# rlog58/dags-vae-search

Hardware: AMD Instinct MI355X
Metric: DAGs/sec VAE+predictor train step, n=12 batch 4096 per GPU, at 1 MI355X (higher is better)
Workload: dtype f32 (fwd bf16x6, bwd bf16x3 split products, fp32 accumulate); 1 GPU; synthetic_v12 DAGs (n=12, card=12, N=15 tokens), PACE-VAE train step: pack + fwd + bwd + clip_grad_norm_(1.0) + Adam(1e-4), train mode dropout 0.15; per_gpu_batch=4096, global_batch=4096, waves_per_workgroup=8, parallelism=single

## Files before the change

### dags_vae_search_amd/csrc/dvs_api.hip

```cpp
#include <math.h>
#include <stdarg.h>
#include <stdio.h>
#include <stdlib.h>
#include <string.h>

#include "dvs_kernels.h"
#include "dvs_backward.h"
#include "dvs_wide.h"
#include "dvs_wimg.h"
#include "dvs_decode.h"
#include "dvs_search_args.h"

static thread_local char g_err[256] = "";

#include <map>
#include <mutex>
#include <string>
#include <utility>
#include <vector>
namespace {
struct ProfRec {
    const char* name;
#ifndef DVS_EMU
    hipEvent_t a, b;
// ... 114 lines not shown
struct LayoutBuilder {
    int64_t off = 0;
    dvs_param_entry* table;
    int cap, count = 0;
    int64_t add(int rows, int cols, const char* fmt, ...) {
        const int64_t o = off;
        if (table && count < cap) {
            dvs_param_entry& e = table[count];
            memset(&e, 0, sizeof(e));
            va_list ap;
            va_start(ap, fmt);
            vsnprintf(e.name, sizeof(e.name), fmt, ap);
            va_end(ap);
            e.offset = o;
            e.rows = rows;
            e.cols = cols;
        }
        ++count;
        const int64_t n = (int64_t)rows * (cols ? cols : 1);
        off += (n + 3) & ~(int64_t)3;
        return o;
    }
};
}

DvsLayout dvs_make_layout(int N, int C, dvs_param_entry* table, int cap, int* count) {
    LayoutBuilder b;
    b.table = table;
    b.cap = cap;
    DvsLayout l;
    auto attn = [&](const char* stack, int i, const char* which, DvsAttnP& p) {
        p.in_w = b.add(192, 64, "%s.layers.%d.%s.in_proj_weight", stack, i, which);
        p.in_b = b.add(192, 0, "%s.layers.%d.%s.in_proj_bias", stack, i, which);
        p.out_w = b.add(64, 64, "%s.layers.%d.%s.out_proj.weight", stack, i, which);
        p.out_b = b.add(64, 0, "%s.layers.%d.%s.out_proj.bias", stack, i, which);
    };
    auto ffn = [&](const char* stack, int i, DvsFfnP& p) {
        p.l1_w = b.add(64, 64, "%s.layers.%d.linear1.weight", stack, i);
        p.l1_b = b.add(64, 0, "%s.layers.%d.linear1.bias", stack, i);
        p.l2_w = b.add(64, 64, "%s.layers.%d.linear2.weight", stack, i);
        p.l2_b = b.add(64, 0, "%s.layers.%d.linear2.bias", stack, i);
    };
    auto norm = [&](const char* stack, int i, int k, DvsNormP& p) {
        p.w = b.add(64, 0, "%s.layers.%d.norm%d.weight", stack, i, k);
        p.b = b.add(64, 0, "%s.layers.%d.norm%d.bias", stack, i, k);
    };
    l.W1 = b.add(2 * N, 64, "vertex_position_embed.W1");
    l.W2 = b.add(64, 32, "vertex_position_embed.W2");
    l.lab_w = b.add(32, C, "vertex_label_embed.0.weight");
    l.lab_b = b.add(32, 0, "vertex_label_embed.0.bias");
    for (int i = 0; i < DVS_LAYERS; ++i) {
        attn("encoder", i, "self_attn", l.enc[i].sa);
        ffn("encoder", i, l.enc[i].ff);
        norm("encoder", i, 1, l.enc[i].n1);
        norm("encoder", i, 2, l.enc[i].n2);
    }
    l.fc1_w = b.add(32, N * 64, "fc1.weight");
    l.fc1_b = b.add(32, 0, "fc1.bias");
    l.fc2_w = b.add(32, N * 64, "fc2.weight");
    l.fc2_b = b.add(32, 0, "fc2.bias");
    for (int i = 0; i < DVS_LAYERS; ++i) {
        attn("decoder", i, "self_attn", l.dec[i].sa);
        attn("decoder", i, "multihead_attn", l.dec[i].ca);
        ffn("decoder", i, l.dec[i].ff);
        norm("decoder", i, 1, l.dec[i].n1);
        norm("decoder", i, 2, l.dec[i].n2);
        norm("decoder", i, 3, l.dec[i].n3);
    }
    l.node0_w = b.add(32, 64, "add_node.0.weight");
    l.node0_b = b.add(32, 0, "add_node.0.bias");
    l.node2_w = b.add(C, 32, "add_node.2.weight");
    l.node2_b = b.add(C, 0, "add_node.2.bias");
    l.edge0_w = b.add(64, 128, "add_edge.0.weight");
    l.edge0_b = b.add(64, 0, "add_edge.0.bias");
    l.edge2_w = b.add(1, 64, "add_edge.2.weight");
    l.edge2_b = b.add(1, 0, "add_edge.2.bias");
    l.fc3_w = b.add(N * 64, 32, "fc3.weight");
    l.fc3_b = b.add(N * 64, 0, "fc3.bias");
    l.total = b.off;
    if (count) *count = b.count;
    return l;
}

DvsWorkspace dvs_make_workspace(int B, int NT, int64_t P, int nslab, bool wide) {
    DvsWorkspace w;
    size_t off = 0;
    auto take = [&](size_t n) {
        const size_t o = off;
        off += (n + 63) & ~(size_t)63;
        return o;
    };
    const size_t tile = (size_t)B * NT * 1024;
    for (int s = 0; s < DVS_NSLOTS; ++s) {
        w.act[s] = take(tile);
        w.stats[s] = take((size_t)B * NT * 32);
    }
    w.enc_out = take(tile);
    w.mu = take((size_t)B * 32);
    w.logvar = take((size_t)B * 32);
    w.z = take((size_t)B * 32);
    w.epsv = take((size_t)B * 32);
    w.mem = take(tile);
    w.dag_loss = take((size_t)B * 2);
    w.gA = take(tile);
    w.gB = take(tile);
    w.gq = take(tile);
    w.gk = take(tile);
    w.gv = take(tile);
    w.gmem = take(tile);
    w.genc = take(tile);
    w.gz = take((size_t)B * 64);
    w.nslab = nslab;
    w.slabs = take((size_t)nslab * (size_t)P);
    w.fcpart = take((size_t)DVS_FC_PARTS * (size_t)P);
    w.wimg = take((DVS_WIMG_BF16 + 1) / 2);
    w.limg = take(DvsLatImg::floats(NT));
    for (int blk = 0; blk < 9; ++blk) w.qkv[blk] = take(wide ? (size_t)B * NT * 12 * 256 : 0);
    w.total_floats = off;
    return w;
}

static int check_shape(const dvs_shape* s) {
    if (!s) return fail(1, "dvs: null shape");
    if (s->batch <= 0) return fail(2, "dvs: batch must be > 0");
    if (s->n_tokens < 4 || s->n_tokens > DVS_WTOK)
        return fail(3, "dvs: n_tokens (= max_num_vertices + 3) must be in [4, 48] in this build");
    if (s->n_classes < 4 || s->n_classes > DVS_WTOK)
        return fail(4, "dvs: n_classes (= vertex_label_cardinality + 3) must be in [4, 48] in this build");
    if (!(s->dropout >= 0.f && s->dropout < 1.f)) return fail(5, "dvs: dropout must be in [0, 1)");
    return 0;
}

static bool is_wide(const dvs_shape* s) { return s->n_tokens > DVS_MAXTOK || s->n_classes > 16; }
static int tiles_of(const dvs_shape* s) { return (s->n_tokens + 15) / 16; }
static size_t record_size(bool wide) { return wide ? sizeof(DvsRecordW) : sizeof(DvsRecord); }

static DvsDims make_dims(const dvs_shape* s) {
    DvsDims d;
    d.NT = tiles_of(s);
    d.B = s->batch;
    d.N = s->n_tokens;
    d.C = s->n_classes;
    d.training = s->training ? 1 : 0;
    d.drop.thr16 = (uint32_t)lrintf(s->dropout * 65536.0f);
    d.drop.on = (d.training && d.drop.thr16 > 0) ? 1 : 0;
    d.drop.scale = 1.0f / (1.0f - (float)d.drop.thr16 / 65536.0f);
    d.seed_lo = (uint32_t)(s->seed & 0xFFFFFFFFull);
    d.seed_hi = (uint32_t)(s->seed >> 32);
    d.dag_offset = s->dag_offset;
    d.beta = s->beta;
    d.eps_scale = s->eps_scale;
    d.debug = 0;
    return d;
}

static int num_slabs() {
    const int cus = dvs_device_cus();
    return cus > 0 ? cus : 256;
}
static int grid_for(int units, int per_wg, int cap) {
    const int want = (units + per_wg - 1) / per_wg;
    return want < cap ? want : cap;
}

static int waves_per_wg(const DvsDims& d, bool wide, int nslab) {
    const char* env = getenv("DVS_WAVES_PER_WG");
    const int force = env ? atoi(env) : 0;
    if (wide) return 8;
    if (force == 4 || force == 8) return force;
    return d.B <= 4 * nslab ? 4 : 8;
}
static int active_slabs(const DvsDims& d, bool wide, int nslab) {
    if (wide) return nslab;
    const int want = (d.B + 3) / 4;
    return want < nslab ? want : nslab;
}

static bool env_on(const char* name) {
    const char* v = getenv(name);
    return v && atoi(v) != 0;
}
static bool split_stack() {
    static const bool on = env_on("DVS_SPLIT_STACK");
    return on;
}
static bool latent_kernels_off() {
    static const bool on = env_on("DVS_LATENT_KERNELS");
    return on;
}
static bool latent_in_chain(bool chain, int nw) { return chain && !latent_kernels_off() && nw == 8; }

struct FwdGrids {
    int chain;
    int tiles16;
    int tiles8;
    int tiles4;
    int dags;
    int dags2;
    int dec4;
};

struct Step {
    DvsDims d;
    DvsLayout L;
    DvsWorkspace W;
    bool wide;
    const float* P;
    float* ws;
    const DvsRecord* rec;
    dvs_stream_t st;
    int nw;
    FwdGrids g;
    int slabs;
};
static Step make_step(const dvs_shape* s, const void* records, const float* params, void* workspace, void* stream) {
    Step c;
    c.d = make_dims(s);
    c.L = dvs_make_layout(c.d.N, c.d.C, nullptr, 0, nullptr);
    c.wide = is_wide(s);
    const int nslab = num_slabs();
    c.W = dvs_make_workspace(c.d.B, c.d.NT, c.L.total, nslab, c.wide);
    c.P = params;
    c.ws = (float*)workspace;
    c.rec = (const DvsRecord*)records;
    c.st = (dvs_stream_t)stream;
    c.nw = waves_per_wg(c.d, c.wide, nslab);
    const int tiles = c.d.B * c.d.NT;
    c.g.chain = grid_for(tiles, c.nw, nslab);
    c.g.tiles16 = grid_for(tiles, 16, nslab);
    c.g.tiles8 = grid_for(tiles, 8, nslab);
    c.g.tiles4 = grid_for(tiles, 4, nslab);
    c.g.dags = grid_for(c.d.B, 1, nslab);
    c.g.dags2 = c.d.B < 2 * c.g.dags ? c.d.B : 2 * c.g.dags;
    c.g.dec4 = grid_for(c.d.B, 4, nslab);
    c.slabs = active_slabs(c.d, c.wide, nslab);
    return c;
}

static int check_records(const char* fn, size_t records_bytes, int batch, bool wide) {
    const size_t need = (size_t)batch * record_size(wide);
    if (records_bytes >= need) return 0;
    char msg[240];
    snprintf(msg, sizeof(msg), "%s: records_bytes %zu < batch * dvs_record_bytes = %zu", fn, records_bytes, need);
    return fail(14, msg);
}
static int check_buffers(const Step& c, const char* fn, size_t records_bytes, int64_t n_params, size_t workspace_bytes) {
    if (int e = check_records(fn, records_bytes, c.d.B, c.wide)) return e;
    char msg[240];
    if (n_params < c.L.total) {
        snprintf(msg, sizeof(msg), "%s: n_params %lld < dvs_param_count = %lld", fn, (long long)n_params, (long long)c.L.total);
        return fail(14, msg);
    }
    const size_t need = c.W.total_floats * sizeof(float);
    if (workspace_bytes < need) {
        snprintf(msg, sizeof(msg), "%s: workspace_bytes %zu < dvs_workspace_bytes = %zu", fn, workspace_bytes, need);
        return fail(14, msg);
    }
    return 0;
}

extern "C" int64_t dvs_param_count(const dvs_shape* s) {
    if (check_shape(s)) return -1;
    return dvs_make_layout(s->n_tokens, s->n_classes, nullptr, 0, nullptr).total;
}

extern "C" int dvs_param_table(const dvs_shape* s, dvs_param_entry* out, int cap) {
    if (check_shape(s)) return -1;
    int count = 0;
    dvs_make_layout(s->n_tokens, s->n_classes, out, cap, &count);
    return count;
}

extern "C" size_t dvs_workspace_bytes(const dvs_shape* s) {
    if (check_shape(s)) return 0;
    return make_step(s, nullptr, nullptr, nullptr, nullptr).W.total_floats * sizeof(float);
}

extern "C" size_t dvs_record_bytes(const dvs_shape* s) {
    if (check_shape(s)) return 0;
    return record_size(is_wide(s));
}

extern "C" int dvs_pack_features(const dvs_shape* s, const float* label_onehot, const float* pos_onehot,
                                 const float* adjacency, const uint8_t* target_masks, void* records, size_t records_bytes,
                                 int32_t* status, void* stream) {
    if (int e = check_shape(s)) return e;
    if (!label_onehot || !pos_onehot || !adjacency || !target_masks || !records || !status)
        return fail(10, "dvs_pack_features: null pointer");
    if (int e = check_records("dvs_pack_features", records_bytes, s->batch, is_wide(s))) return e;
    call_begin();
    PackArgs a;
    a.B = s->batch;
    a.N = s->n_tokens;
    a.C = s->n_classes;
    a.lab1h = label_onehot;
    a.pos1h = pos_onehot;
    a.adj = adjacency;
    a.tmask = target_masks;
    a.rec = (DvsRecord*)records;
    a.status = status;
    if (is_wide(s)) dvs_launch_pack_w(a, (dvs_stream_t)stream);
    else dvs_launch_pack(a, (dvs_stream_t)stream);
    return call_end("dvs_pack_features");
}

extern "C" int dvs_build_records(const dvs_shape* s, const uint8_t* labels, const void* preds, void* records,
                                 size_t records_bytes, int32_t* status, void* stream) {
    if (int e = check_shape(s)) return e;
    if (!labels || !preds || !records || !status) return fail(10, "dvs_build_records: null pointer");
    if (int e = check_records("dvs_build_records", records_bytes, s->batch, is_wide(s))) return e;
    call_begin();
    if (is_wide(s)) {
        BuildWArgs a;
        a.B = s->batch;
        a.N = s->n_tokens;
        a.C = s->n_classes;
        a.labels = labels;
        a.preds = (const uint64_t*)preds;
        a.rec = (DvsRecordW*)records;
        a.status = status;
        dvs_launch_build_records_w(a, (dvs_stream_t)stream);
        return call_end("dvs_build_records");
    }
    BuildArgs a;
    a.B = s->batch;
    a.N = s->n_tokens;
    a.C = s->n_classes;
    a.labels = labels;
    a.preds = (const uint16_t*)preds;
    a.rec = (DvsRecord*)records;
    a.status = status;
    dvs_launch_build_records(a, (dvs_stream_t)stream);
    return call_end("dvs_build_records");
}

static inline int slot_enc(int layer, int sub) { return 1 + 2 * layer + sub; }
static inline int slot_dec(int layer, int sub) { return 8 + 3 * layer + sub; }
static inline int site_enc(int layer, int k) { return 4 + 4 * layer + k; }
static inline int site_dec(int layer, int k) { return 16 + 6 * layer + k; }

static inline size_t img_attn(int block) { return (size_t)block * DvsAttnImg::SIZE; }
static inline size_t img_ffn(int block) { return DVS_N_ATTN_BLOCKS * DvsAttnImg::SIZE + (size_t)block * DvsFfnImg::SIZE; }
static inline int blk_enc_attn(int layer) { return layer; }
static inline int blk_dec_self(int layer) { return 3 + 2 * layer; }
static inline int blk_dec_cross(int layer) { return 4 + 2 * layer; }
static inline int blk_enc_ffn(int layer) { return layer; }
static inline int blk_dec_ffn(int layer) { return 3 + layer; }

static inline const void* wimg_attn(const Step& c, int block) { return (const dvs_bf16*)(c.ws + c.W.wimg) + img_attn(block); }
static inline const void* wimg_ffn(const Step& c, int block) { return (const dvs_bf16*)(c.ws + c.W.wimg) + img_ffn(block); }

static DvsLN ln_of(const Step& c, int slot, const DvsNormP* n) {
    if (!n) return DvsLN{nullptr, nullptr, nullptr};
    return DvsLN{c.ws + c.W.stats[slot], c.P + n->w, c.P + n->b};
}

static EmbedArgs embed_args(const Step& c, int site) {
    EmbedArgs e;
    memset(&e, 0, sizeof(e));
    e.dims = c.d;
    e.rec = c.rec;
    e.W1 = c.P + c.L.W1;
    e.W2 = c.P + c.L.W2;
    e.lab_w = c.P + c.L.lab_w;
    e.lab_b = c.P + c.L.lab_b;
    e.embimg = (const float*)((const dvs_bf16*)(c.ws + c.W.wimg) + DVS_WIMG_EMB);
    e.site = site;
    return e;
}

static AttnArgs attn_args(const Step& c, const DvsAttnP& p, int block, int in, const DvsNormP* norm, const float* kv, int out,
                          int site0) {
    AttnArgs a;
    memset(&a, 0, sizeof(a));
    a.dims = c.d;
    a.rec = c.rec;
    a.xin = c.ws + c.W.act[in];
    a.ln = ln_of(c, in, norm);
    a.kv = kv;
    a.in_w = c.P + p.in_w;
    a.in_b = c.P + p.in_b;
    a.out_w = c.P + p.out_w;
    a.out_b = c.P + p.out_b;
    a.wimg = wimg_attn(c, block);
    a.qkv = c.wide ? c.ws + c.W.qkv[block] : nullptr;
    a.out_pre = c.ws + c.W.act[out];
    a.out_stats = c.ws + c.W.stats[out];
    a.site_prob = site0;
    a.site_post = site0 + 1;
    return a;
}

static FfnArgs ffn_args(const Step& c, const DvsFfnP& p, int block, int in, const DvsNormP& norm, int out, int site0) {
    FfnArgs f;
    memset(&f, 0, sizeof(f));
    f.dims = c.d;
    f.xin = c.ws + c.W.act[in];
    f.ln = ln_of(c, in, &norm);
    f.l1_w = c.P + p.l1_w;
    f.l1_b = c.P + p.l1_b;
    f.l2_w = c.P + p.l2_w;
    f.l2_b = c.P + p.l2_b;
    f.wimg = wimg_ffn(c, block);
    f.out_pre = c.ws + c.W.act[out];
    f.out_stats = c.ws + c.W.stats[out];
    f.site_hidden = site0;
    f.site_post = site0 + 1;
    return f;
}

static LatentArgs latent_args(const Step& c, const float* eps, bool with_mem) {
    LatentArgs a;
    memset(&a, 0, sizeof(a));
    a.dims = c.d;
    a.xenc = c.ws + c.W.enc_out;
    a.fc1_w = c.P + c.L.fc1_w;
    a.fc1_b = c.P + c.L.fc1_b;
    a.fc2_w = c.P + c.L.fc2_w;
    a.fc2_b = c.P + c.L.fc2_b;
    a.fc3_w = c.P + c.L.fc3_w;
    a.fc3_b = c.P + c.L.fc3_b;
    a.limg = c.ws + c.W.limg;
    a.eps_in = eps;
    a.mu = c.ws + c.W.mu;
    a.logvar = c.ws + c.W.logvar;
    a.z = c.ws + c.W.z;
    a.epsv = c.ws + c.W.epsv;
    a.mem = with_mem ? c.ws + c.W.mem : nullptr;
    a.dag_loss = c.ws + c.W.dag_loss;
    return a;
}

template <class A>
static void head_params(const Step& c, A& a) {
    a.node0_w = c.P + c.L.node0_w;
    a.node0_b = c.P + c.L.node0_b;
    a.node2_w = c.P + c.L.node2_w;
    a.node2_b = c.P + c.L.node2_b;
    a.edge0_b = c.P + c.L.edge0_b;
    a.edge2_w = c.P + c.L.edge2_w;
    a.edge2_b = c.P + c.L.edge2_b;
}
template <class A>
static void head_input(const Step& c, A& a) {
    const int last = slot_dec(DVS_LAYERS - 1, 2);
    a.xin = c.ws + c.W.act[last];
    a.ln = ln_of(c, last, &c.L.dec[DVS_LAYERS - 1].n3);
    a.edge0_w = c.P + c.L.edge0_w;
    head_params(c, a);
}

static LossArgs loss_args(const Step& c) {
    LossArgs a;
    memset(&a, 0, sizeof(a));
    a.dims = c.d;
    a.rec = c.rec;
    head_input(c, a);
    a.wimg = (const dvs_bf16*)(c.ws + c.W.wimg) + DVS_WIMG_LOSS;
    a.dag_loss = c.ws + c.W.dag_loss;
    return a;
}

static void prepare_images(const Step& c) {
    const DvsLayout& L = c.L;
    const bool wide = c.wide;
    DvsImgJobs J;
    J.count = 0;
    auto add = [&](int64_t src, size_t dst, int rows, int flags) {
        DvsImgJob& j = J.job[J.count++];
        j.src = src;
        j.dst = (int64_t)dst;
        j.rows = rows;
        j.flags = flags;
    };
    auto attn = [&](const DvsAttnP& p, int block) {
        const size_t b = img_attn(block);
        add(p.in_w, b + DvsAttnImg::Win, 192, wide ? 0 : 2);
        add(p.out_w, b + DvsAttnImg::Wout, 64, wide ? 0 : 4);
        add(p.out_w, b + DvsAttnImg::WoutT, 64, 1 | (wide ? 0 : 4));
        add(p.in_w, b + DvsAttnImg::WinB, 192, 16 | (wide ? 0 : 2));
        for (int q = 0; q < 3; ++q)
            add(p.in_w + 4096 * q, b + DvsAttnImg::WinT + (size_t)q * 2 * DVS_IMG64, 64, 1 | (wide ? 0 : 2));
    };
    auto ffn = [&](const DvsFfnP& p, int block) {
        const size_t b = img_ffn(block);
        add(p.l1_w, b + DvsFfnImg::W1, 64, 0);
        add(p.l2_w, b + DvsFfnImg::W2, 64, 0);
        add(p.l2_w, b + DvsFfnImg::W2T, 64, 1);
        add(p.l1_w, b + DvsFfnImg::W1T, 64, 1);
    };
// ... 10 lines not shown
        add(L.edge0_w, DVS_WIMG_LOSS + DvsLossImg::WaT, 64, 8 | 1);
        add(L.edge0_w + 64, DVS_WIMG_LOSS + DvsLossImg::WbT, 64, 8 | 1);
    }
    dvs_bf16* wimg = (dvs_bf16*)(c.ws + c.W.wimg);
    DvsLatImgArgs lat;
    lat.fc1_w = c.P + L.fc1_w;
    lat.fc2_w = c.P + L.fc2_w;
    lat.fc3_w = c.P + L.fc3_w;
    lat.fc3_b = c.P + L.fc3_b;
    lat.img = c.ws + c.W.limg;
    lat.N = c.d.N;
    lat.NT = c.d.NT;
    DvsLossHeadArgs head;
    memset(&head, 0, sizeof(head));
    if (!wide) {
        head_params(c, head);
        head.ln_g = c.P + L.dec[DVS_LAYERS - 1].n3.w;
        head.ln_b = c.P + L.dec[DVS_LAYERS - 1].n3.b;
        head.dst = (float*)(wimg + DVS_WIMG_LOSS + DvsLossImg::Head);
        head.C = c.d.C;
        head.W1 = c.P + L.W1;
        head.W2 = c.P + L.W2;
        head.lab_w = c.P + L.lab_w;
        head.lab_b = c.P + L.lab_b;
        head.dst_emb = (float*)(wimg + DVS_WIMG_EMB);
        head.N = c.d.N;
    }
    dvs_launch_prepare_images(J, c.P, wimg, lat, head, c.st);
}

static void launch_embed_fwd(const Step& c, const EmbedArgs& e) {
    if (c.wide) dvs_launch_embed_fwd_w(e, c.g.tiles4, c.st);
    else if (c.nw == 4) dvs_launch_embed_fwd(e, c.g.chain, 4, c.st);
    else dvs_launch_embed_fwd(e, c.g.tiles16, 16, c.st);
}
static void launch_attn_fwd(const Step& c, const AttnArgs& a) {
    if (c.wide) dvs_launch_attn_fwd_w(a, c.g.dags, c.st);
    else if (c.nw == 4) dvs_launch_attn_fwd(a, c.g.chain, 4, c.st);
    else dvs_launch_attn_fwd(a, c.g.tiles8, 8, c.st);
}
static void launch_ffn_fwd(const Step& c, const FfnArgs& f) {
    if (c.nw == 4) dvs_launch_ffn_fwd(f, c.g.chain, 4, c.st);
    else dvs_launch_ffn_fwd(f, c.g.tiles16, 16, c.st);
}
static void launch_loss_fwd(const Step& c, const LossArgs& a) {
    if (c.wide) dvs_launch_loss_fwd_w(a, c.g.dags2, c.st);
    else if (c.nw == 4) dvs_launch_loss_fwd(a, c.g.chain, 4, c.st);
    else dvs_launch_loss_fwd(a, c.g.tiles8, 8, c.st);
}
struct FwdChain {
    FwdStackArgs stack;
    const Step& c;
    int tag;
    bool chain;
    FwdChain(const Step& step, int tag_) : c(step), tag(tag_), chain(!step.wide && !split_stack()) { memset(&stack, 0, sizeof(stack)); }
    FwdPhase& next(int kind) {
        if (stack.nphase == DVS_FWD_STACK_PHASES) flush();
        FwdPhase& ph = stack.ph[stack.nphase++];
        ph.kind = kind;
        return ph;
    }
    void attn(const AttnArgs& a) {
        if (chain) next(DVS_FPH_ATTN).u.a = a;
        else launch_attn_fwd(c, a);
    }
    void ffn(const FfnArgs& f) {
        if (chain) next(DVS_FPH_FFN).u.f = f;
        else launch_ffn_fwd(c, f);
    }
    bool latent(const LatentArgs& l) {
        if (!latent_in_chain(chain, c.nw) || stack.nphase == 0 || stack.nphase == DVS_FWD_STACK_PHASES) return false;
        next(DVS_FPH_LATENT).u.l = l;
        return true;
    }
    void flush() {
        if (stack.nphase > 0) dvs_launch_fwd_stack(stack, tag, c.g.chain, c.nw, c.st);
        stack.nphase = 0;
    }
};

static void encoder_forward(const Step& c, const LatentArgs& lat, bool dec_embed = false, bool save_qkv = false) {
    EmbedArgs e = embed_args(c, 0);
    e.out = c.ws + c.W.act[0];
    if (dec_embed) {
        e.out2 = c.ws + c.W.act[7];
        e.site2 = 2;
    }
    launch_embed_fwd(c, e);
    FwdChain chain(c, 0);
    const DvsNormP* norm = nullptr;
    int prev = 0;
    for (int i = 0; i < DVS_LAYERS; ++i) {
        const auto& pl = c.L.enc[i];
        const int sa = slot_enc(i, 0), sf = slot_enc(i, 1);
        AttnArgs a = attn_args(c, pl.sa, blk_enc_attn(i), prev, norm, nullptr, sa, site_enc(i, 0));
        if (!save_qkv) a.qkv = nullptr;
        chain.attn(a);
        FfnArgs f = ffn_args(c, pl.ff, blk_enc_ffn(i), sa, pl.n1, sf, site_enc(i, 2));
        if (i == DVS_LAYERS - 1) {
            f.out_norm = c.ws + c.W.enc_out;
            f.ng = c.P + pl.n2.w;
            f.nb = c.P + pl.n2.b;
        }
        chain.ffn(f);
        norm = &pl.n2;
        prev = sf;
    }
    const bool fused = chain.latent(lat);
    chain.flush();
    if (!fused) dvs_launch_latent_fwd(lat, c.st);
}

static void decoder_forward(const Step& c, int dec_in) {
    FwdChain chain(c, 1);
    const DvsNormP* norm = nullptr;
    int prev = dec_in;
    for (int i = 0; i < DVS_LAYERS; ++i) {
        const auto& pl = c.L.dec[i];
        const int s0 = slot_dec(i, 0), s1 = slot_dec(i, 1), s2 = slot_dec(i, 2);
        chain.attn(attn_args(c, pl.sa, blk_dec_self(i), prev, norm, nullptr, s0, site_dec(i, 0)));
        chain.attn(attn_args(c, pl.ca, blk_dec_cross(i), s0, &pl.n1, c.ws + c.W.mem, s1, site_dec(i, 2)));
        chain.ffn(ffn_args(c, pl.ff, blk_dec_ffn(i), s1, pl.n2, s2, site_dec(i, 4)));
        norm = &pl.n3;
        prev = s2;
    }
    chain.flush();
}

extern "C" int dvs_loss_forward(const dvs_shape* s, const void* records, size_t records_bytes, const float* params,
                                int64_t n_params, void* workspace, size_t workspace_bytes, const float* eps,
                                const int32_t* status, float* losses, float* mu, float* logvar, void* stream) {
    return dvs_loss_forward_notify(s, records, records_bytes, params, n_params, workspace, workspace_bytes, eps,
                                   (int32_t*)status, losses, mu, logvar, nullptr, 0u, stream);
}

extern "C" int dvs_loss_forward_notify(const dvs_shape* s, const void* records, size_t records_bytes, const float* params,
                                       int64_t n_params, void* workspace, size_t workspace_bytes, const float* eps,
                                       int32_t* status, float* losses, float* mu, float* logvar, void* host_tail,
                                       uint32_t host_seq, void* stream) {
    if (int e = check_shape(s)) return e;
    if (!records || !params || !workspace || !losses) return fail(10, "dvs_loss_forward: null pointer");
    const Step c = make_step(s, records, params, workspace, stream);
    if (int e = check_buffers(c, "dvs_loss_forward", records_bytes, n_params, workspace_bytes)) return e;
    call_begin();
    prepare_images(c);
    encoder_forward(c, latent_args(c, eps, true), c.d.drop.on, true);
    decoder_forward(c, c.d.drop.on ? 7 : 0);
    launch_loss_fwd(c, loss_args(c));
    FinalizeArgs fa;
    fa.B = c.d.B;
    fa.beta = c.d.beta;
    fa.dag_loss = c.ws + c.W.dag_loss;
    fa.status = status;
    fa.losses = losses;
    fa.host_tail = (float*)host_tail;
    fa.host_seq = host_seq;
    dvs_launch_finalize(fa, c.st);
    const size_t nb = (size_t)c.d.B * 32 * sizeof(float);
    if (mu) copy_out(mu, c.ws + c.W.mu, nb, c.st);
    if (logvar) copy_out(logvar, c.ws + c.W.logvar, nb, c.st);
    return call_end("dvs_loss_forward");
}

extern "C" int dvs_encode(const dvs_shape* s, const void* records, size_t records_bytes, const float* params,
                          int64_t n_params, void* workspace, size_t workspace_bytes, float* mu, float* logvar,
                          void* stream) {
    if (int e = check_shape(s)) return e;
    if (!records || !params || !workspace || !mu || !logvar) return fail(10, "dvs_encode: null pointer");
    const Step c = make_step(s, records, params, workspace, stream);
// ... 77 lines not shown
```

### dags_vae_search_amd/csrc/dvs_api_backward.inc

```

static AttnBwdArgs attn_bwd_args(const Step& c, const DvsAttnP& ap, int block, int in, const DvsNormP* norm, const float* kv,
                                 const float* gpre, int site0) {
    AttnBwdArgs a;
    memset(&a, 0, sizeof(a));
    a.wimg = wimg_attn(c, block);
    a.dims = c.d;
    a.rec = c.rec;
    a.xin = c.ws + c.W.act[in];
    a.ln = ln_of(c, in, norm);
    a.kv = kv;
    a.in_w = c.P + ap.in_w;
    a.in_b = c.P + ap.in_b;
    a.out_w = c.P + ap.out_w;
    a.out_b = c.P + ap.out_b;
    a.gpre = gpre;
    a.gq = c.ws + c.W.gq;
    a.gk = c.ws + c.W.gk;
    a.gv = c.ws + c.W.gv;
    a.site_prob = site0;
    a.site_post = site0 + 1;
    a.slab = c.ws + c.W.slabs;
    a.P = c.L.total;
    a.o_out_w = ap.out_w;
    a.o_out_b = ap.out_b;
    a.qkv = c.wide ? c.ws + c.W.qkv[block] : nullptr;
    return a;
}

static ProjBwdArgs proj_bwd_args(const Step& c, const DvsAttnP& ap, int block, int in, const DvsNormP* norm, const float* gres,
                                 float* gout) {
    ProjBwdArgs a;
    memset(&a, 0, sizeof(a));
    a.dims = c.d;
    a.xin = c.ws + c.W.act[in];
    a.ln = ln_of(c, in, norm);
    a.w = c.P + ap.in_w;
    a.wimg = (const dvs_bf16*)wimg_attn(c, block) + DvsAttnImg::WinT;
    a.gy[0] = c.ws + c.W.gq;
    a.gy[1] = c.ws + c.W.gk;
    a.gy[2] = c.ws + c.W.gv;
    a.gres = gres;
    a.gout = gout;
    a.slot_order = c.wide ? 0 : 1;
    a.slab = c.ws + c.W.slabs;
    a.P = c.L.total;
    a.o_w = ap.in_w;
    a.o_b = ap.in_b;
    a.o_ln_g = norm ? norm->w : -1;
    a.o_ln_b = norm ? norm->b : -1;
    return a;
}

static FfnBwdArgs ffn_bwd_args(const Step& c, const DvsFfnP& fp, int block, int in, const DvsNormP& norm, const float* gpre,
                               float* gout, int site0) {
    FfnBwdArgs a;
    memset(&a, 0, sizeof(a));
    a.dims = c.d;
    a.xin = c.ws + c.W.act[in];
    a.ln = ln_of(c, in, &norm);
    a.l1_w = c.P + fp.l1_w;
    a.l1_b = c.P + fp.l1_b;
    a.l2_w = c.P + fp.l2_w;
    a.l2_b = c.P + fp.l2_b;
    a.wimg = wimg_ffn(c, block);
    a.gpre = gpre;
    a.gout = gout;
    a.site_hidden = site0;
    a.site_post = site0 + 1;
    a.slab = c.ws + c.W.slabs;
    a.P = c.L.total;
    a.o_l1_w = fp.l1_w;
    a.o_l1_b = fp.l1_b;
    a.o_l2_w = fp.l2_w;
    a.o_l2_b = fp.l2_b;
    a.o_ln_g = norm.w;
    a.o_ln_b = norm.b;
    a.o_own_g = -1;
    a.o_own_b = -1;
    return a;
}

extern "C" int dvs_loss_backward(const dvs_shape* s, const void* records, size_t records_bytes, const float* params,
                                 int64_t n_params, void* workspace, size_t workspace_bytes, const float* gcoef,
                                 float* grads, void* stream) {
    return dvs_loss_backward_sq(s, records, records_bytes, params, n_params, workspace, workspace_bytes, gcoef, grads, nullptr,
                                stream);
}

extern "C" int dvs_loss_backward_sq(const dvs_shape* s, const void* records, size_t records_bytes, const float* params,
                                    int64_t n_params, void* workspace, size_t workspace_bytes, const float* gcoef,
                                    float* grads, float* clip_scratch, void* stream) {
    if (int e = check_shape(s)) return e;
    if (!records || !params || !workspace || !gcoef || !grads) return fail(10, "dvs_loss_backward: null pointer");
    const Step c = make_step(s, records, params, workspace, stream);
    if (int e = check_buffers(c, "dvs_loss_backward", records_bytes, n_params, workspace_bytes)) return e;
    if (clip_scratch && 2 + dvs_sq_parts(c.L.total) > DVS_CLIP_SCRATCH_FLOATS)
        return fail(14, "dvs_loss_backward_sq: clip_scratch (DVS_CLIP_SCRATCH_FLOATS) is too small for this parameter count");
    call_begin();
    const DvsLayout& L = c.L;
    const DvsWorkspace& W = c.W;
    float* ws = c.ws;
    dvs_stream_t st = c.st;
    const bool wide = c.wide;
    const int grid = c.slabs;
    const int nw = c.nw;
    const bool chain = !wide && !split_stack();
    const bool chain_local = wide && !split_stack();
    BwdStackArgs stack;
    memset(&stack, 0, sizeof(stack));
    int stack_tag = 0;
    auto flush_stack = [&]() {
        if (stack.nphase > 0) dvs_launch_bwd_stack(stack, stack_tag, grid, nw, st);
        stack.nphase = 0;
        stack.has_latent = 0;
    };
    auto next_phase = [&](int kind) -> BwdPhase& {
        if (stack.nphase == DVS_STACK_PHASES) flush_stack();
        BwdPhase& ph = stack.ph[stack.nphase++];
        ph.kind = kind;
        return ph;
    };
    auto launch_ffn_bwd = [&](const FfnBwdArgs& f) {
        if (chain || chain_local) next_phase(DVS_PH_FFN).u.f = f;
        else dvs_launch_ffn_bwd(f, grid, nw, st);
    };
    auto launch_attn_bwd = [&](const AttnBwdArgs& a) {
        if (chain) {
            next_phase(DVS_PH_ATTN).u.a = a;
        } else if (wide) {
            flush_stack();
            dvs_launch_attn_bwd_w(a, grid, st);
        } else {
            dvs_launch_attn_bwd(a, grid, nw, st);
        }
    };
    auto launch_proj_bwd = [&](const ProjBwdArgs& a) {
        if (chain || chain_local) next_phase(DVS_PH_PROJ1 + 2).u.p = a;
        else dvs_launch_proj_bwd(a, 3, grid, nw, st);
    };

    float* cur = ws + W.gA;
    float* oth = ws + W.gB;
    {
        LossArgs la = loss_args(c);
        la.gcoef = gcoef;
        la.gout = cur;
        la.slab = ws + W.slabs;
        la.P = L.total;
        la.o_node0_w = L.node0_w;
        la.o_node0_b = L.node0_b;
        la.o_node2_w = L.node2_w;
        la.o_node2_b = L.node2_b;
        la.o_edge0_w = L.edge0_w;
        la.o_edge0_b = L.edge0_b;
        la.o_edge2_w = L.edge2_w;
        la.o_edge2_b = L.edge2_b;
        la.o_ln_g = L.dec[DVS_LAYERS - 1].n3.w;
        la.o_ln_b = L.dec[DVS_LAYERS - 1].n3.b;
        if (wide) dvs_launch_loss_bwd_w(la, grid, st);
        else dvs_launch_loss_bwd(la, grid, st);
    }
// ... 9 lines not shown
        pq.gout2 = ws + W.gmem;
        pq.accumulate_out2 = i != DVS_LAYERS - 1;
        launch_proj_bwd(pq);
        std::swap(cur, oth);
        const int sp = i > 0 ? slot_dec(i - 1, 2) : dec_in;
        const DvsNormP* np = i > 0 ? &L.dec[i - 1].n3 : nullptr;
        launch_attn_bwd(attn_bwd_args(c, pl.sa, blk_dec_self(i), sp, np, nullptr, cur, site_dec(i, 0)));
        launch_proj_bwd(proj_bwd_args(c, pl.sa, blk_dec_self(i), sp, np, cur, oth));
        std::swap(cur, oth);
    }
    flush_stack();
    stack_tag = 1;
    float* gdec_emb = cur;
    float* freebuf = oth;

    const bool fc_deferred = latent_in_chain(chain, nw);
    FcDwArgs fcdw;
    {
        LatentBwdArgs a;
        memset(&a, 0, sizeof(a));
        a.dims = c.d;
        a.gmem = ws + W.gmem;
        a.mu = ws + W.mu;
        a.logvar = ws + W.logvar;
        a.epsv = ws + W.epsv;
        a.limg = ws + W.limg;
        a.gcoef = gcoef;
        a.gz = ws + W.gz;
        a.genc = ws + W.genc;
        if (fc_deferred) {
            stack.has_latent = 1;
            stack.lat = a;
        } else {
            dvs_launch_latent_bwd(a, st);
        }
        FcDwArgs& f = fcdw;
        memset(&f, 0, sizeof(f));
        f.dims = c.d;
        f.gz = ws + W.gz;
        f.xenc = ws + W.enc_out;
        f.gmem = ws + W.gmem;
        f.z = ws + W.z;
        f.fcpart = ws + W.fcpart;
        f.P = L.total;
        f.o_fc1_w = L.fc1_w;
        f.o_fc1_b = L.fc1_b;
        f.o_fc2_w = L.fc2_w;
        f.o_fc2_b = L.fc2_b;
        f.o_fc3_w = L.fc3_w;
        f.o_fc3_b = L.fc3_b;
        if (!fc_deferred) dvs_launch_fc_dw(f, st);
    }
    cur = ws + W.genc;
    oth = freebuf;
    for (int i = DVS_LAYERS - 1; i >= 0; --i) {
        const auto& pl = L.enc[i];
        const int s0 = slot_enc(i, 0), s1 = slot_enc(i, 1);
        FfnBwdArgs f = ffn_bwd_args(c, pl.ff, blk_enc_ffn(i), s0, pl.n1, cur, oth, site_enc(i, 2));
        if (i == DVS_LAYERS - 1) {
            f.own_pre = ws + W.act[s1];
            f.own = ln_of(c, s1, &pl.n2);
            f.o_own_g = pl.n2.w;
            f.o_own_b = pl.n2.b;
        }
        launch_ffn_bwd(f);
        std::swap(cur, oth);
        const int sp = i > 0 ? slot_enc(i - 1, 1) : 0;
        const DvsNormP* np = i > 0 ? &L.enc[i - 1].n2 : nullptr;
        launch_attn_bwd(attn_bwd_args(c, pl.sa, blk_enc_attn(i), sp, np, nullptr, cur, site_enc(i, 0)));
        launch_proj_bwd(proj_bwd_args(c, pl.sa, blk_enc_attn(i), sp, np, cur, oth));
        std::swap(cur, oth);
    }
    flush_stack();
    if (fc_deferred) dvs_launch_fc_dw(fcdw, st);
    {
        EmbedArgs e = embed_args(c, 0);
        e.gout = cur;
        e.slab = ws + W.slabs;
        e.P = L.total;
        e.oW1 = L.W1;
        e.oW2 = L.W2;
        e.olab_w = L.lab_w;
        e.olab_b = L.lab_b;
        if (wide) dvs_launch_embed_bwd_w(e, gdec_emb, 2, grid, st);
        else dvs_launch_embed_bwd(e, gdec_emb, 2, grid, nw, st);
    }
    ReduceArgs r;
    r.slab = ws + W.slabs;
    r.fcpart = ws + W.fcpart;
    r.grads = grads;
    r.P = L.total;
    r.nslab = grid;
    r.fc_lo1 = L.fc1_w;
    r.fc_hi1 = L.dec[0].sa.in_w;
    r.fc_lo2 = L.fc3_w;
    r.fc_hi2 = L.total;
    r.sqpart = clip_scratch ? clip_scratch + 2 : nullptr;
    dvs_launch_reduce_slabs(r, st);
    return call_end("dvs_loss_backward");
}

extern "C" int dvs_clip_adam(int64_t n, float* params, float* grads, float* exp_avg, float* exp_avg_sq, float lr,
                             float beta1, float beta2, float adam_eps, int64_t step, float max_norm, float* scratch,
                             const float* guard, void* stream) {
    if (n <= 0 || !params || !grads || !exp_avg || !exp_avg_sq || !scratch) return fail(10, "dvs_clip_adam: bad argument");
    if (step < 1) return fail(12, "dvs_clip_adam: step is 1-based");
    call_begin();
    dvs_launch_clip_adam(n, params, grads, exp_avg, exp_avg_sq, lr, beta1, beta2, adam_eps, step, max_norm, scratch, guard, false,
                         (dvs_stream_t)stream);
    return call_end("dvs_clip_adam");
}

extern "C" int dvs_clip_adam_from_partials(int64_t n, float* params, float* grads, float* exp_avg, float* exp_avg_sq, float lr,
                                           float beta1, float beta2, float adam_eps, int64_t step, float max_norm,
                                           float* scratch, const float* guard, void* stream) {
    if (n <= 0 || !params || !grads || !exp_avg || !exp_avg_sq || !scratch) return fail(10, "dvs_clip_adam_from_partials: bad argument");
    if (step < 1) return fail(12, "dvs_clip_adam_from_partials: step is 1-based");
    if (2 + dvs_sq_parts(n) > DVS_CLIP_SCRATCH_FLOATS) return fail(14, "dvs_clip_adam_from_partials: more partials than the scratch holds");
    call_begin();
    dvs_launch_clip_adam(n, params, grads, exp_avg, exp_avg_sq, lr, beta1, beta2, adam_eps, step, max_norm, scratch, guard, true,
                         (dvs_stream_t)stream);
    return call_end("dvs_clip_adam_from_partials");
}
```

### dags_vae_search_amd/csrc/dvs_backward.h

```cpp
#pragma once
#include "dvs_kernels.h"
#include "dvs_stage.h"

struct FfnBwdArgs {
    DvsDims dims;
    const float* xin;
    DvsLN ln;
    const float *l1_w, *l1_b, *l2_w, *l2_b;
    const void* wimg;
    const float* gpre;
    const float* own_pre;
    DvsLN own;
    float* gout;
    int site_hidden, site_post;
    float* slab;
    int64_t P;
    int64_t o_l1_w, o_l1_b, o_l2_w, o_l2_b, o_ln_g, o_ln_b, o_own_g, o_own_b;
};

struct ProjBwdArgs {
    DvsDims dims;
    const float* xin;
    DvsLN ln;
    const float* w;
    const void* wimg;
    const float* gy[3];
    const float* gres;
    float* gout;
    int accumulate_out;
    int slot_order;
    const float* xin2;
    float* gout2;
    int accumulate_out2;
    float* slab;
    int64_t P;
    int64_t o_w, o_b, o_ln_g, o_ln_b;
};

struct AttnBwdArgs {
    DvsDims dims;
    const DvsRecord* rec;
    const float* xin;
    DvsLN ln;
    const float* kv;
    const float *in_w, *in_b, *out_w, *out_b;
    const void* wimg;
    const float* gpre;
    float *gq, *gk, *gv;
    int site_prob, site_post;
    float* slab;
    int64_t P;
    int64_t o_out_w, o_out_b;
    const float* qkv;
};

struct LatentBwdArgs {
    DvsDims dims;
    const float* gmem;
    const float *mu, *logvar, *epsv;
    const float* limg;
    const float* gcoef;
    float* gz;
    float* genc;
};

struct FcDwArgs {
    DvsDims dims;
    const float* gz;
    const float* xenc;
    const float* gmem;
    const float* z;
    float* fcpart;
    int64_t P;
    int64_t o_fc1_w, o_fc1_b, o_fc2_w, o_fc2_b, o_fc3_w, o_fc3_b;
};

struct ReduceArgs {
    const float* slab;
    const float* fcpart;
    float* grads;
    int64_t P;
    int nslab;
    int64_t fc_lo1, fc_hi1, fc_lo2, fc_hi2;
    float* sqpart;
};

enum { DVS_PH_FFN = 0, DVS_PH_ATTN = 1, DVS_PH_PROJ1 = 2, DVS_PH_PROJ2 = 3, DVS_PH_PROJ3 = 4 };
#define DVS_STACK_PHASES 9
struct BwdPhase {
    int kind, pad;
    union {
        FfnBwdArgs f;
        AttnBwdArgs a;
        ProjBwdArgs p;
    } u;
};
struct BwdStackArgs {
    int nphase;
    int has_latent;
    BwdPhase ph[DVS_STACK_PHASES];
    DvsStagePlan plan[DVS_STACK_PHASES];
    LatentBwdArgs lat;
};
static_assert(sizeof(BwdStackArgs) <= 4096, "kernel argument block limit");
void dvs_launch_bwd_stack(const BwdStackArgs& s, int tag, int grid, int nw, dvs_stream_t st);
void dvs_launch_ffn_bwd(const FfnBwdArgs& a, int grid, int nw, dvs_stream_t st);
void dvs_launch_proj_bwd(const ProjBwdArgs& a, int nproj, int grid, int nw, dvs_stream_t st);
void dvs_launch_attn_bwd(const AttnBwdArgs& a, int grid, int nw, dvs_stream_t st);
void dvs_launch_loss_bwd(const LossArgs& a, int grid, dvs_stream_t st);
void dvs_launch_embed_bwd(const EmbedArgs& a, const float* gout2, int site2, int grid, int nw, dvs_stream_t st);
void dvs_launch_latent_bwd(const LatentBwdArgs& a, dvs_stream_t st);
void dvs_launch_fc_dw(const FcDwArgs& a, dvs_stream_t st);
void dvs_launch_reduce_slabs(const ReduceArgs& a, dvs_stream_t st);
void dvs_launch_clip_adam(int64_t n, float* params, float* grads, float* m, float* v, float lr, float b1, float b2,
                          float eps, int64_t step, float max_norm, float* scratch, const float* guard, bool have_partials,
                          dvs_stream_t st);
inline int dvs_sq_parts(int64_t n) { return (int)(((n + 3) / 4 + 63) / 64); }

template <int OT, int IT>
__device__ __forceinline__ void dvs_stage_dw(float* region, const f4 (&dw)[OT][IT], const Lane& L) {
    constexpr int COLS = 16 * IT;
    float* mine = region + L.wave * (256 * OT * IT);
#pragma unroll
    for (int ot = 0; ot < OT; ++ot)
#pragma unroll
        for (int it = 0; it < IT; ++it)
#pragma unroll
            for (int reg = 0; reg < 4; ++reg) mine[(16 * ot + 4 * L.g + reg) * COLS + 16 * it + L.r] = dw[ot][it][reg];
}
template <int OT, int IT>
__device__ __forceinline__ void dvs_flush_dw(const float* region, float* dst, const Lane& L, int rows = 16 * OT,
                                             int ld_dst = 16 * IT, int cols_used = 16 * IT, bool rperm = false,
                                             bool cperm = false) {
    constexpr int COLS = 16 * IT, SZ = 256 * OT * IT;
    if (cperm) {
        for (int i = dvs_tid(); i < rows * COLS; i += blockDim.x) {
// ... 153 lines not shown
```

### dags_vae_search_amd/csrc/dvs_bwd_phases.h

```cpp
#pragma once
#include "dvs_backward.h"
#include "dvs_wimg.h"

constexpr int DVS_PROJB_SLOT = 6 * DVS_PKB;
static size_t projb_lds_bytes(int nproj) {
    return (size_t)2 * nproj * 64 * DVS_LDB * sizeof(dvs_bf16) + 128 * 4 + (size_t)8 * DVS_PROJB_SLOT * sizeof(dvs_bf16) + 64;
}


#include "dvs_stage.h"

constexpr size_t DVS_BWD_EPI_FLOOR = 80 * 1024;
static_assert(8 * DVS_IMG64 * sizeof(dvs_bf16) + (192 + 64 + 128) * 4 + 16 <= DVS_BWD_EPI_FLOOR, "attention-core plan");
static_assert(7 * DVS_IMG64 * sizeof(dvs_bf16) + 6 * 64 * 4 + 16 <= DVS_BWD_EPI_FLOOR, "FFN plan");
static_assert(6 * DVS_IMG64 * sizeof(dvs_bf16) + 128 * 4 + 16 <= DVS_BWD_EPI_FLOOR, "projection plan");
static_assert(DVS_BWD_EPI_FLOOR + (2 * 4096 + 8 * 6 * 64) * 4 <= 7 * DVS_IMG64 * sizeof(dvs_bf16) + (6 * 64 + 8 * 2 * DVS_SCR) * 4, "FFN");
static_assert(DVS_BWD_EPI_FLOOR + (4096 + 8 * 64) * 4 <= 8 * DVS_IMG64 * sizeof(dvs_bf16) + (384 + 8 * 2 * DVS_SCR) * 4, "attention core");
static_assert(DVS_BWD_EPI_FLOOR + (1 * 4096 + 8 * 3 * 64) * 4 <= 2 * DVS_IMG64 * sizeof(dvs_bf16) + 8 * DVS_PROJB_SLOT * sizeof(dvs_bf16), "1 projection");
static_assert(DVS_BWD_EPI_FLOOR + (3 * 4096 + 8 * 5 * 64) * 4 <= 6 * DVS_IMG64 * sizeof(dvs_bf16) + 8 * DVS_PROJB_SLOT * sizeof(dvs_bf16), "3 projections");
__device__ __forceinline__ float* dvs_bwd_epi(char* smem) { return (float*)(smem + DVS_BWD_EPI_FLOOR); }

#ifdef DVS_STAMPS
DVS_STAMP_DECL(dvs_stamps_bwd);
#endif

struct FfnBLds {
    dvs_bf16 *W2Th, *W2Tl, *W1Th, *W1Tl, *W1x6;
    float *b1, *b2, *lg, *lb, *og, *ob, *slots;
    int* gcount;
};
DVS_HD inline FfnBLds ffnb_lds(char* smem) {
    FfnBLds l;
    l.W2Th = (dvs_bf16*)smem;
    l.W2Tl = l.W2Th + 64 * DVS_LDB;
    l.W1Th = l.W2Tl + 64 * DVS_LDB;
    l.W1Tl = l.W1Th + 64 * DVS_LDB;
    l.W1x6 = l.W1Tl + 64 * DVS_LDB;
    l.b1 = (float*)(l.W1x6 + 3 * 64 * DVS_LDB);
    l.b2 = l.b1 + 64;
    l.lg = l.b2 + 64;
    l.lb = l.lg + 64;
    l.og = l.lb + 64;
    l.ob = l.og + 64;
    l.gcount = (int*)(l.ob + 64);
    l.slots = (float*)(l.gcount + 4);
    return l;
}
static size_t ffnb_lds_bytes() {
    return 7 * 64 * DVS_LDB * sizeof(dvs_bf16) + (6 * 64 + (size_t)8 * 2 * DVS_SCR + 16) * sizeof(float);
}

constexpr int DVS_ATTNB_TLD = 20;
constexpr int DVS_ATTNB_TSCR = 16 * DVS_ATTNB_TLD;
struct AttnBLds {
    float *inb, *outb, *lg, *lb, *slots, *stats;
    dvs_bf16 *Winh, *Winl, *WoTh, *WoTl;
    int* gcount;
};
DVS_HD inline AttnBLds attnb_lds(char* smem) {
    AttnBLds l;
    l.WoTh = (dvs_bf16*)smem;
    l.WoTl = l.WoTh + 64 * DVS_LDB;
    l.Winh = l.WoTl + 64 * DVS_LDB;
    l.Winl = l.Winh + 192 * DVS_LDB;
    l.inb = (float*)(l.Winl + 192 * DVS_LDB);
    l.outb = l.inb + 192;
    l.lg = l.outb + 64;
    l.lb = l.lg + 64;
    l.gcount = (int*)(l.lb + 64);
    l.slots = (float*)(l.gcount + 4);
    l.stats = l.slots + 8 * 2 * DVS_SCR;
    return l;
}
static size_t attnb_lds_floats() {
    return 512 * DVS_LDB / 2 + 192 + 64 + 128 + (size_t)8 * 2 * DVS_SCR + 8 * DVS_ATTNB_TSCR + 16;
}


struct ProjBLds {
    dvs_bf16* WT;
    float *lg, *lb;
    dvs_bf16* slots;
    int* gcount;
};
DVS_HD inline ProjBLds projb_lds(char* smem, int nproj) {
    ProjBLds l;
    l.WT = (dvs_bf16*)smem;
    l.lg = (float*)(l.WT + nproj * 2 * DVS_IMG64);
    l.lb = l.lg + 64;
    l.gcount = (int*)(l.lb + 64);
    l.slots = (dvs_bf16*)(l.gcount + 4);
    return l;
}

inline void ffnb_plan(DvsStagePlan& p, const FfnBwdArgs& a, char* smem) {
    const FfnBLds l = ffnb_lds(smem);
    dvs_plan_clear(p);
    dvs_plan_seg(p, smem, l.W2Th, (const dvs_bf16*)a.wimg + DvsFfnImg::W2T, (int)(7 * DVS_IMG64));
    dvs_plan_vec(p, smem, l.b1, a.l1_b, 64);
    dvs_plan_vec(p, smem, l.b2, a.l2_b, 64);
    dvs_plan_vec(p, smem, l.lg, a.ln.g, a.ln.stats ? 64 : 0);
    dvs_plan_vec(p, smem, l.lb, a.ln.b, a.ln.stats ? 64 : 0);
    dvs_plan_vec(p, smem, l.og, a.own.g, a.own_pre ? 64 : 0);
    dvs_plan_vec(p, smem, l.ob, a.own.b, a.own_pre ? 64 : 0);
    p.zero_int = (int)(((const char*)l.gcount - smem) >> 2);
    dvs_plan_cold(p, a.xin, a.own_pre, a.dims.B * a.dims.NT);
    dvs_plan_seal(p);
}
inline void attnb_plan(DvsStagePlan& p, const AttnBwdArgs& a, char* smem) {
    const AttnBLds l = attnb_lds(smem);
    dvs_plan_clear(p);
    dvs_plan_seg(p, smem, l.WoTh, (const dvs_bf16*)a.wimg + DvsAttnImg::WoutT, (int)(8 * DVS_IMG64));
    dvs_plan_vec(p, smem, l.inb, a.in_b, 192, true);
    dvs_plan_vec(p, smem, l.outb, a.out_b, 64);
    dvs_plan_vec(p, smem, l.lg, a.ln.g, a.ln.stats ? 64 : 0);
    dvs_plan_vec(p, smem, l.lb, a.ln.b, a.ln.stats ? 64 : 0);
    p.zero_int = (int)(((const char*)l.gcount - smem) >> 2);
    dvs_plan_cold(p, a.xin, a.kv, a.dims.B * a.dims.NT);
    dvs_plan_seal(p);
}
inline void projb_plan(DvsStagePlan& p, const ProjBwdArgs& a, int nproj, char* smem) {
    const ProjBLds l = projb_lds(smem, nproj);
    dvs_plan_clear(p);
    dvs_plan_seg(p, smem, l.WT, a.wimg, (int)(nproj * 2 * DVS_IMG64));
    dvs_plan_vec(p, smem, l.lg, a.ln.g, a.ln.stats ? 64 : 0);
    dvs_plan_vec(p, smem, l.lb, a.ln.b, a.ln.stats ? 64 : 0);
    p.zero_int = (int)(((const char*)l.gcount - smem) >> 2);
    dvs_plan_cold(p, a.xin, a.xin2, a.dims.B * a.dims.NT);
    dvs_plan_seal(p);
}
inline void dvs_bwd_plan(DvsStagePlan& p, const BwdPhase& ph, char* smem) {
    switch (ph.kind) {
        case DVS_PH_FFN: ffnb_plan(p, ph.u.f, smem); break;
        case DVS_PH_ATTN: attnb_plan(p, ph.u.a, smem); break;
        case DVS_PH_PROJ1: projb_plan(p, ph.u.p, 1, smem); break;
        case DVS_PH_PROJ2: projb_plan(p, ph.u.p, 2, smem); break;
        default: projb_plan(p, ph.u.p, 3, smem); break;
    }
}
struct DvsBwdTail {
    DvsPrefetch<DVS_PF_BWD_TAIL> pf;
};
template <class PP>
__device__ __forceinline__ void dvs_tail_issue(DvsBwdTail& t, PP next, bool has_next) {
    if (has_next && dvs_tid() < DVS_PF_THREADS) dvs_prefetch_issue<false>(t.pf, next, dvs_tid(), DVS_PF_THREADS);
}
template <class PP>
__device__ __forceinline__ void dvs_tail_commit(const DvsBwdTail& t, PP next, bool has_next, char* smem) {
    if (has_next && dvs_tid() < DVS_PF_THREADS) dvs_prefetch_commit<false>(t.pf, next, smem, dvs_tid(), DVS_PF_THREADS);
}
template <class PP>
__device__ __forceinline__ void dvs_bwd_tail_end(const DvsBwdTail& tail, const DvsTouch& touch, PP mine, PP next, bool has_next,
                                                 char* smem) {
    DVS_STAMP(dvs_stamps_bwd, mine, 5);
    dvs_tail_commit(tail, next, has_next, smem);
    DVS_STAMP(dvs_stamps_bwd, mine, 6);
    dvs_touch_done(touch);
}

template <int NW, class PP>
__device__ __forceinline__ void dvs_ffn_bwd_phase(const FfnBwdArgs& a, char* smem, PP mine, bool stage_mine, PP next,
                                                  bool has_next) {
    const FfnBLds l = ffnb_lds(smem);
    DVS_STAMP(dvs_stamps_bwd, mine, 0);
    if (stage_mine) {
        dvs_stage_now<(NW == 8 ? DVS_PF_BWD : DVS_PF_BWD_TAIL)>(mine, smem);
        __syncthreads();
    }
    DVS_STAMP(dvs_stamps_bwd, mine, 1);
    int* gcount = l.gcount;
    const Lane L = dvs_lane();
    const DvsDrop D = dvs_drop_of(a.dims);
    const int B = a.dims.B * a.dims.NT;
    float* sA = l.slots + L.wave * 2 * DVS_SCR;
    float* sB = sA + DVS_SCR;
    DvsGroup G = {gcount + (L.wave >> 2), 0};
    f4 aW1[4] = {f4_zero(), f4_zero(), f4_zero(), f4_zero()}, aW2[4] = {f4_zero(), f4_zero(), f4_zero(), f4_zero()};
    f4 ab1 = f4_zero(), ab2 = f4_zero();
    float vgam = 0.f, vbet = 0.f, vog = 0.f, vob = 0.f;
    dvs_bf16* const bslots = (dvs_bf16*)l.slots;
    constexpr int BSTRIDE = 2 * 2 * DVS_SCR;
    bool gate = !stage_mine;
    for (int base = dvs_bid() * NW; base < B; base += gridDim.x * NW) {
        const int dag = base + L.wave;
        const bool live = dag < B;
        const size_t dg = live ? dag : 0;
        const DvsTile T = dvs_tile_of((int)dg, a.dims);
        const int N = T.Nl;
        const int Nl = live ? N : 0;
        f4 x[4], xhat[4], gp[4];
        float rstd;
        {
            DvsRawX rx;
            dvs_load_x_issue(rx, a.xin, a.ln, dg, L);
            DVS_PHASE_GATE(gate);
            dvs_load_tile(gp, a.gpre, dg, L);
            dvs_load_x_finish<true>(x, xhat, rstd, rx, a.ln, l.lg, l.lb, Nl, L);
            dvs_zero_rows(gp, Nl, L);
        }
        if (a.own_pre) {
            f4 po[4], pxh[4], t0[4];
            float prstd;
            dvs_load_x<true>(po, pxh, prstd, a.own_pre, a.own, l.og, l.ob, dg, Nl, L);
#pragma unroll
            for (int t = 0; t < 4; ++t) t0[t] = gp[t] * pxh[t];
            dvs_park_T(sA, t0, L);
            dvs_park_T(sB, gp, L);
            dvs_wave_sync();
            vog += dvs_colsum(sA, L);
            vob += dvs_colsum(sB, L);
            dvs_wave_sync();
            dvs_ln_bwd_core(gp, pxh, prstd, l.og, L);
        }
        const uint32_t gdag = a.dims.dag_offset + (uint32_t)T.dag;
        const uint32_t khid = dvs_site_key(a.dims.seed_lo, a.dims.seed_hi, a.site_hidden, gdag);
        const uint32_t kpost = dvs_site_key(a.dims.seed_lo, a.dims.seed_hi, a.site_post, gdag);
        f4 hpre[4], hd[4];
#pragma unroll
        for (int t = 0; t < 4; ++t) hpre[t] = dvs_vecT(l.b1, t, L);
        dvs_matb3<4>(hpre, dvs_split3_T(x), l.W1x6, 64, 0, L);
#pragma unroll
        for (int t = 0; t < 4; ++t)
#pragma unroll
            for (int kk = 0; kk < 4; ++kk) hd[t][kk] = (live && L.r < N) ? fmaxf(hpre[t][kk], 0.f) : 0.f;
        const uint32_t hid_bits = dvs_dropout_bits(khid, D, L, T.tok0);
        dvs_dropout_apply(hd, hid_bits, D);
        f4 dy[4];
#pragma unroll
        for (int t = 0; t < 4; ++t) dy[t] = gp[t];
        dvs_dropout_tile(dy, kpost, D, L, T.tok0);
        dvs_park_bf((dvs_bf16*)sA, dy, L);
        dvs_park_bf((dvs_bf16*)sB, hd, L);
        dvs_group_barrier(G, L);
        dvs_coop_dw_bf(aW2, ab2, bslots, bslots + 2 * DVS_SCR, BSTRIDE, L);
        f4 dh[4] = {f4_zero(), f4_zero(), f4_zero(), f4_zero()};
        dvs_matb_T<4>(dh, dvs_split_T(dy), l.W2Th, l.W2Tl, 0, L);
        dvs_dropout_apply(dh, hid_bits, D);
#pragma unroll
        for (int t = 0; t < 4; ++t)
#pragma unroll
            for (int kk = 0; kk < 4; ++kk) dh[t][kk] = hpre[t][kk] > 0.f ? dh[t][kk] : 0.f;
        dvs_group_barrier(G, L);
        dvs_park_bf((dvs_bf16*)sA, dh, L);
        dvs_park_bf((dvs_bf16*)sB, x, L);
        dvs_group_barrier(G, L);
        dvs_coop_dw_bf(aW1, ab1, bslots, bslots + 2 * DVS_SCR, BSTRIDE, L);
        f4 dx[4];
#pragma unroll
        for (int t = 0; t < 4; ++t) dx[t] = gp[t];
        dvs_matb_T<4>(dx, dvs_split_T(dh), l.W1Th, l.W1Tl, 0, L);
        dvs_group_barrier(G, L);
        if (a.ln.stats) {
            f4 t0[4];
#pragma unroll
            for (int t = 0; t < 4; ++t) t0[t] = dx[t] * xhat[t];
            dvs_park_T(sA, t0, L);
            dvs_park_T(sB, dx, L);
            dvs_wave_sync();
            vgam += dvs_colsum(sA, L);
            vbet += dvs_colsum(sB, L);
            dvs_wave_sync();
            dvs_ln_bwd_core(dx, xhat, rstd, l.lg, L);
        }
        if (live) dvs_store_tile(a.gout, dag, dx, L);
        if (base == dvs_bid() * NW) DVS_STAMP(dvs_stamps_bwd, mine, 7);
    }
    DVS_PHASE_GATE(gate);
    DvsBwdTail tail;
    DVS_STAMP(dvs_stamps_bwd, mine, 2);
    dvs_tail_issue(tail, next, has_next);
    const DvsTouch touch = dvs_touch_first(next, has_next, NW, L.wave, L.lane);
    DVS_STAMP(dvs_stamps_bwd, mine, 3);
    dvs_lds_barrier();
    DVS_STAMP(dvs_stamps_bwd, mine, 4);
    float* slab = a.slab + (size_t)dvs_bid() * a.P;
    float* const buf1 = dvs_bwd_epi(smem);
    float* const buf2 = buf1 + 4096;
    float* red = buf2 + 4096;
    dvs_coop_stage<NW>(buf1, aW1, L);
    dvs_coop_stage<NW>(buf2, aW2, L);
    red[(L.wave * 6 + 0) * 64 + L.lane] = 0.f;
    red[(L.wave * 6 + 1) * 64 + L.lane] = 0.f;
    red[(L.wave * 6 + 2) * 64 + L.lane] = vgam;
    red[(L.wave * 6 + 3) * 64 + L.lane] = vbet;
    red[(L.wave * 6 + 4) * 64 + L.lane] = vog;
    red[(L.wave * 6 + 5) * 64 + L.lane] = vob;
    dvs_wave_sync();
    if (L.r == 0) {
#pragma unroll
        for (int reg = 0; reg < 4; ++reg) {
            red[(L.wave * 6 + 0) * 64 + 16 * (L.wave & 3) + 4 * L.g + reg] = ab1[reg];
            red[(L.wave * 6 + 1) * 64 + 16 * (L.wave & 3) + 4 * L.g + reg] = ab2[reg];
        }
    }
    dvs_lds_barrier();
    dvs_coop_flush<NW>(buf1, slab + a.o_l1_w, aW1, L);
    dvs_coop_flush<NW>(buf2, slab + a.o_l2_w, aW2, L);
    for (int k = dvs_tid() >> 6; k < 6; k += NW) {
        const int f = dvs_tid() & 63;
        float s = 0.f;
        for (int w = 0; w < NW; ++w) s += red[(w * 6 + k) * 64 + f];
        const int64_t off = k == 0 ? a.o_l1_b : k == 1 ? a.o_l2_b : k == 2 ? a.o_ln_g : k == 3 ? a.o_ln_b : k == 4 ? a.o_own_g : a.o_own_b;
        if (off >= 0) slab[off + f] = s;
    }
    dvs_bwd_tail_end(tail, touch, mine, next, has_next, smem);
}

template <int NPROJ, int NW, class PP>
__device__ __forceinline__ void dvs_proj_bwd_phase(const ProjBwdArgs& a, char* smem, PP mine, bool stage_mine, PP next,
                                                   bool has_next) {
    const ProjBLds pl = projb_lds(smem, NPROJ);
    dvs_bf16* WT = pl.WT;
    float* lg = pl.lg;
    float* lb = pl.lb;
    dvs_bf16* slots = pl.slots;
    int* gcount = pl.gcount;
    DVS_STAMP(dvs_stamps_bwd, mine, 0);
    if (stage_mine) {
        dvs_stage_now<(NW == 8 ? DVS_PF_BWD : DVS_PF_BWD_TAIL)>(mine, smem);
        __syncthreads();
    }
    DVS_STAMP(dvs_stamps_bwd, mine, 1);
    const Lane L = dvs_lane();
    const int B = a.dims.B * a.dims.NT;
    dvs_bf16* myA0 = slots + L.wave * DVS_PROJB_SLOT;
    dvs_bf16* myA1 = myA0 + 2 * DVS_PKB;
    dvs_bf16* myB = myA0 + 4 * DVS_PKB;
    DvsGroup G = {gcount + (L.wave >> 2), 0};
    bool gate = !stage_mine;
    f4 aW[NPROJ][4], ab[NPROJ];
    float vgam = 0.f, vbet = 0.f;
#pragma unroll
    for (int p = 0; p < NPROJ; ++p) {
        ab[p] = f4_zero();
#pragma unroll
        for (int i = 0; i < 4; ++i) aW[p][i] = f4_zero();
    }
    for (int base = dvs_bid() * NW; base < B; base += gridDim.x * NW) {
        const int dag = base + L.wave;
        const bool live = dag < B;
        const size_t dg = live ? dag : 0;
        const int Nl = live ? dvs_tile_of((int)dg, a.dims).Nl : 0;
        f4 x[4], xhat[4], dx[4];
        float rstd;
        {
            DvsRawX rx;
            dvs_load_x_issue(rx, a.xin, a.ln, dg, L);
            DVS_PHASE_GATE(gate);
            if (a.gres) {
                dvs_load_tile(dx, a.gres, dg, L);
            } else {
#pragma unroll
                for (int t = 0; t < 4; ++t) dx[t] = f4_zero();
            }
            dvs_load_x_finish<true>(x, xhat, rstd, rx, a.ln, lg, lb, Nl, L);
            dvs_zero_rows(dx, Nl, L);
        }
        dvs_park_bf(myB, x, L);
        const bool split = NPROJ == 3 && a.xin2 != nullptr;
        auto run = [&](int p0, int p1, f4 (&acc_dx)[4]) {
#pragma unroll
            for (int p = 0; p < NPROJ; ++p) {
                if (p < p0 || p >= p1) continue;
                dvs_bf16* mine = (p & 1) ? myA1 : myA0;
                f4 dy[4];
                dvs_load_grad(dy, a.gy[p], dg, Nl, L);
                dvs_park_bf(mine, dy, L);
                dvs_group_barrier(G, L);
                dvs_coop_dw_bf(aW[p], ab[p], slots + (p & 1) * 2 * DVS_PKB, slots + 4 * DVS_PKB, DVS_PROJB_SLOT, L);
                dvs_matb_T<4>(acc_dx, dvs_split_T(dy), WT + p * 2 * DVS_IMG64, WT + p * 2 * DVS_IMG64 + DVS_IMG64, 0, L);
            }
        };
        run(0, split ? 1 : NPROJ, dx);
        dvs_group_barrier(G, L);
        if (a.ln.stats) {
            float* fA = (float*)myA0;
            float* fB = (float*)myB;
            f4 t0[4];
#pragma unroll
            for (int t = 0; t < 4; ++t) t0[t] = dx[t] * xhat[t];
            dvs_park_T(fA, t0, L);
            dvs_park_T(fB, dx, L);
            dvs_wave_sync();
            vgam += dvs_colsum(fA, L);
            vbet += dvs_colsum(fB, L);
            dvs_wave_sync();
            dvs_ln_bwd_core(dx, xhat, rstd, lg, L);
        }
        if (live) {
            if (a.accumulate_out) {
                f4 old[4];
                dvs_load_tile(old, a.gout, dag, L);
#pragma unroll
                for (int t = 0; t < 4; ++t) dx[t] += old[t];
            }
            dvs_store_tile(a.gout, dag, dx, L);
        }
        if (split) {
            f4 x2[4], dx2[4] = {f4_zero(), f4_zero(), f4_zero(), f4_zero()};
            dvs_load_grad(x2, a.xin2, dg, Nl, L);
            dvs_park_bf(myB, x2, L);
            run(1, 3, dx2);
            dvs_group_barrier(G, L);
            if (live) {
                if (a.accumulate_out2) {
                    f4 old[4];
                    dvs_load_tile(old, a.gout2, dag, L);
#pragma unroll
                    for (int t = 0; t < 4; ++t) dx2[t] += old[t];
                }
                dvs_store_tile(a.gout2, dag, dx2, L);
            }
        }
        if (base == dvs_bid() * NW) DVS_STAMP(dvs_stamps_bwd, mine, 7);
    }
    DVS_PHASE_GATE(gate);
    DvsBwdTail tail;
    DVS_STAMP(dvs_stamps_bwd, mine, 2);
    dvs_tail_issue(tail, next, has_next);
    const DvsTouch touch = dvs_touch_first(next, has_next, NW, L.wave, L.lane);
    DVS_STAMP(dvs_stamps_bwd, mine, 3);
    dvs_lds_barrier();
    DVS_STAMP(dvs_stamps_bwd, mine, 4);
    float* slab = a.slab + (size_t)dvs_bid() * a.P;
    const bool so = a.slot_order != 0;
    float* const bufs = dvs_bwd_epi(smem);
#pragma unroll
    for (int p = 0; p < NPROJ; ++p) dvs_coop_stage<NW>(bufs + 4096 * p, aW[p], L);
    float* red = bufs + 4096 * NPROJ;
#pragma unroll
    for (int p = 0; p < NPROJ; ++p) red[(L.wave * (NPROJ + 2) + p) * 64 + L.lane] = 0.f;
    red[(L.wave * (NPROJ + 2) + NPROJ) * 64 + L.lane] = vgam;
    red[(L.wave * (NPROJ + 2) + NPROJ + 1) * 64 + L.lane] = vbet;
    dvs_wave_sync();
    if (L.r == 0) {
#pragma unroll
        for (int p = 0; p < NPROJ; ++p)
#pragma unroll
            for (int reg = 0; reg < 4; ++reg) red[(L.wave * (NPROJ + 2) + p) * 64 + 16 * (L.wave & 3) + 4 * L.g + reg] = ab[p][reg];
    }
    dvs_lds_barrier();
#pragma unroll
    for (int p = 0; p < NPROJ; ++p) dvs_coop_flush<NW>(bufs + 4096 * p, slab + a.o_w + 4096 * p, aW[p], L, so, false);
    for (int k = dvs_tid() >> 6; k < NPROJ + 2; k += NW) {
        const int f = dvs_tid() & 63;
        float s = 0.f;
        for (int w = 0; w < NW; ++w) s += red[(w * (NPROJ + 2) + k) * 64 + f];
        if (k < NPROJ) slab[a.o_b + 64 * k + (so ? dvs_pi(f) : f)] = s;
        else if (a.o_ln_g >= 0) slab[(k == NPROJ ? a.o_ln_g : a.o_ln_b) + f] = s;
    }
    dvs_bwd_tail_end(tail, touch, mine, next, has_next, smem);
}


__device__ __forceinline__ float dvs_bit_select(uint32_t bits, int pos, float v) {
#ifndef DVS_EMU
    const uint32_t m = (uint32_t)__builtin_amdgcn_sbfe((int)bits, pos, 1);
#else
    const uint32_t m = ((bits >> pos) & 1u) ? 0xFFFFFFFFu : 0u;
#endif
    return __uint_as_float(__float_as_uint(v) & m);
}
struct ProbMask {
    uint32_t T;
    uint32_t S[4];
};
__device__ __forceinline__ ProbMask dvs_prob_mask(uint32_t key, const DvsDrop& D, const Lane& L) {
    ProbMask m;
    m.T = 0xFFFFFFFFu;
    if (D.on) {
        uint32_t bits = 0;
#pragma unroll
        for (int h = 0; h < 8; ++h) {
            const uint32_t p0 = (uint32_t)((h * 16 + L.r) * 8 + 2 * L.g);
            const uint32_t h0 = dvs_draw(key, p0), h1 = dvs_draw(key, p0 + 1);
            bits |= ((h0 & 0xFFFFu) >= D.thr16 ? 1u : 0u) << (4 * h);
            bits |= ((h0 >> 16) >= D.thr16 ? 1u : 0u) << (4 * h + 1);
            bits |= ((h1 & 0xFFFFu) >= D.thr16 ? 1u : 0u) << (4 * h + 2);
            bits |= ((h1 >> 16) >= D.thr16 ? 1u : 0u) << (4 * h + 3);
        }
        m.T = bits;
    }
#pragma unroll
    for (int reg = 0; reg < 4; ++reg)
        m.S[reg] = D.on ? ((uint32_t)__shfl((int)m.T, 4 * L.g + reg + 16 * (L.r >> 2)) >> (L.r & 3)) : 0xFFFFFFFFu;
    return m;
}
__device__ __forceinline__ f4 mask_T(const ProbMask& m, int h, const DvsDrop& D) {
    if (!D.on) return f4_splat(1.f);
    f4 r;
#pragma unroll
    for (int reg = 0; reg < 4; ++reg) r[reg] = dvs_bit_select(m.T, 4 * h + reg, D.scale);
    return r;
}
__device__ __forceinline__ f4 mask_S(const ProbMask& m, int h, const DvsDrop& D) {
    if (!D.on) return f4_splat(1.f);
    f4 r;
#pragma unroll
    for (int reg = 0; reg < 4; ++reg) r[reg] = dvs_bit_select(m.S[reg], 4 * h, D.scale);
    return r;
}

template <int NW, class PP>
__device__ __forceinline__ void dvs_attn_bwd_phase(const AttnBwdArgs& a, char* smem, PP mine, bool stage_mine, PP next,
                                                   bool has_next) {
    const AttnBLds l = attnb_lds(smem);
    DVS_STAMP(dvs_stamps_bwd, mine, 0);
    if (stage_mine) {
        dvs_stage_now<(NW == 8 ? DVS_PF_BWD : DVS_PF_BWD_TAIL)>(mine, smem);
        __syncthreads();
    }
    DVS_STAMP(dvs_stamps_bwd, mine, 1);
    const Lane L = dvs_lane();
    const DvsDrop D = dvs_drop_of(a.dims);
    const int N = a.dims.N, B = a.dims.B;
    float* sA = l.slots + L.wave * 2 * DVS_SCR;
    float* sB = sA + DVS_SCR;
    float* st = l.stats + L.wave * DVS_ATTNB_TSCR;
    DvsGroup G = {l.gcount + (L.wave >> 2), 0};
    const float scale = 0.35355339059327373f;
    f4 aWo[4] = {f4_zero(), f4_zero(), f4_zero(), f4_zero()};
    f4 abo = f4_zero();
    bool gate = !stage_mine;
    DVS_PHASE_GATE(gate);
    for (int base = dvs_bid() * NW; base < B; base += gridDim.x * NW) {
        const int dag = base + L.wave;
        const bool live = dag < B;
        const size_t dg = live ? dag : 0;
        const int Nl = live ? N : 0;
        const uint32_t gdag = a.dims.dag_offset + (uint32_t)dg;
        const uint32_t kprob = dvs_site_key(a.dims.seed_lo, a.dims.seed_hi, a.site_prob, gdag);
        const unsigned allowed_r = live ? a.rec[dg].allowed[L.r] : (1u << L.r);
        f4 q[4], k[4], v[4];
        {
            f4 x[4], kv[4], dummy[4];
            float rstd;
            {
                dvs_load_x<false>(x, dummy, rstd, a.xin, a.ln, l.lg, l.lb, dg, Nl, L);
                if (a.kv) dvs_load_tile(kv, a.kv, dg, L);
            }
            if (!a.kv) {
#pragma unroll
                for (int t = 0; t < 4; ++t) kv[t] = x[t];
            }
#pragma unroll
            for (int t = 0; t < 4; ++t) {
                q[t] = dvs_vecT(l.inb, t, L);
                k[t] = dvs_vecT(l.inb + 64, t, L);
                v[t] = f4_splat(l.inb[128 + 16 * t + L.r]);
            }
            {
                const SplitT xs = dvs_split_T(x);
                dvs_matb_T<4>(q, xs, l.Winh, l.Winl, 0, L);
                if (a.kv) {
                    const SplitT ks = dvs_split_T(kv);
                    dvs_matb_T<4>(k, ks, l.Winh, l.Winl, 64, L);
                    dvs_matb_N<4>(v, ks, l.Winh, l.Winl, 128, L);
                } else {
                    dvs_matb_T<4>(k, xs, l.Winh, l.Winl, 64, L);
                    dvs_matb_N<4>(v, xs, l.Winh, l.Winl, 128, L);
                }
            }
#pragma unroll
            for (int t = 0; t < 4; ++t) q[t] *= scale;
        }
        f4 qN[4], kN[4], vT[4], dOT[4], dON[4];
        {
            f4 dy[4];
            dvs_load_grad(dy, a.gpre, dg, Nl, L);
            dvs_dropout_tile(dy, dvs_site_key(a.dims.seed_lo, a.dims.seed_hi, a.site_post, gdag), D, L);
            dvs_park_bf((dvs_bf16*)sA, dy, L);
#pragma unroll
            for (int t = 0; t < 4; ++t) dOT[t] = f4_zero();
            dvs_matb_T<4>(dOT, dvs_split_T(dy), l.WoTh, l.WoTl, 0, L);
        }
        dvs_t2n<4>(qN, q, sB, L);
        dvs_t2n<4>(kN, k, sB, L);
        dvs_n2t<4>(vT, v, sB, L);
        dvs_t2n<4>(dON, dOT, sB, L);

        const ProbMask pm = dvs_prob_mask(kprob, D, L);
        const bool hsel = ((L.r & 3) >> 1) != 0;
        bool ok[4];
        unsigned al4[4];
#pragma unroll
        for (int reg = 0; reg < 4; ++reg) {
            ok[reg] = (allowed_r >> (4 * L.g + reg)) & 1u;
            al4[reg] = (unsigned)__shfl((int)allowed_r, 4 * L.g + reg);
        }
#pragma unroll
        for (int t = 0; t < 4; ++t) {
            f4 pT[2], dsT[2], ds[2], pd[2];
            float delta[2];
            {
                f4 sT[2] = {f4_zero(), f4_zero()};
#pragma unroll
                for (int kk = 0; kk < 2; ++kk) {
                    sT[0] = dvs_mfma(k[t][kk], q[t][kk], sT[0]);
                    sT[1] = dvs_mfma(k[t][kk + 2], q[t][kk + 2], sT[1]);
                }
                float m[2], den[2];
#pragma unroll
                for (int u = 0; u < 2; ++u) {
                    float mx = -3.0e38f;
#pragma unroll
                    for (int reg = 0; reg < 4; ++reg) mx = ok[reg] ? fmaxf(mx, sT[u][reg]) : mx;
                    m[u] = mx;
                }
#pragma unroll
                for (int u = 0; u < 2; ++u) m[u] = dvs_max_x16(m[u]);
#pragma unroll
                for (int u = 0; u < 2; ++u) m[u] = dvs_max_x32(m[u]);
#pragma unroll
                for (int u = 0; u < 2; ++u) {
                    float sum = 0.f;
#pragma unroll
                    for (int reg = 0; reg < 4; ++reg) {
                        pT[u][reg] = ok[reg] ? __expf(sT[u][reg] - m[u]) : 0.f;
                        sum += pT[u][reg];
                    }
                    den[u] = sum;
                }
#pragma unroll
                for (int u = 0; u < 2; ++u) den[u] = dvs_add_x16(den[u]);
#pragma unroll
                for (int u = 0; u < 2; ++u) den[u] = dvs_add_x32(den[u]);
#pragma unroll
                for (int u = 0; u < 2; ++u) pT[u] *= dvs_rcp(den[u]);
            }
            {
                f4 mk[2], dpT[2];
#pragma unroll
                for (int u = 0; u < 2; ++u) {
                    mk[u] = mask_T(pm, 2 * t + u, D);
                    dpT[u] = f4_zero();
                }
                {
                    f4 oa = f4_zero(), ob = f4_zero();
#pragma unroll
                    for (int kk = 0; kk < 4; ++kk) {
                        oa = dvs_mfma(pT[0][kk] * mk[0][kk], v[t][kk], oa);
                        ob = dvs_mfma(pT[1][kk] * mk[1][kk], v[t][kk], ob);
                    }
                    dvs_bf16* po = (dvs_bf16*)sB + (4 * L.g) * DVS_PLD + 16 * t + L.r;
#pragma unroll
                    for (int reg = 0; reg < 4; ++reg) {
                        dvs_bf16 oh, ol;
                        dvs_split1(hsel ? ob[reg] : oa[reg], oh, ol);
                        po[reg * DVS_PLD] = oh;
                        po[DVS_PKB + reg * DVS_PLD] = ol;
                    }
                }
#pragma unroll
                for (int kk = 0; kk < 2; ++kk) {
                    dpT[0] = dvs_mfma(vT[t][kk], dOT[t][kk], dpT[0]);
                    dpT[1] = dvs_mfma(vT[t][kk + 2], dOT[t][kk + 2], dpT[1]);
                }
#pragma unroll
                for (int u = 0; u < 2; ++u) {
                    dpT[u] *= mk[u];
                    float dl = 0.f;
#pragma unroll
                    for (int reg = 0; reg < 4; ++reg) dl += pT[u][reg] * dpT[u][reg];
                    delta[u] = dl;
                }
#pragma unroll
                for (int u = 0; u < 2; ++u) delta[u] = dvs_add_x16(delta[u]);
#pragma unroll
                for (int u = 0; u < 2; ++u) delta[u] = dvs_add_x32(delta[u]);
#pragma unroll
                for (int u = 0; u < 2; ++u)
#pragma unroll
                    for (int reg = 0; reg < 4; ++reg) dsT[u][reg] = pT[u][reg] * (dpT[u][reg] - delta[u]);
#pragma unroll
                for (int u = 0; u < 2; ++u) {
                    *(f4*)(st + L.r * DVS_ATTNB_TLD + 4 * L.g) = dsT[u];
                    dvs_wave_sync();
#pragma unroll
                    for (int reg = 0; reg < 4; ++reg) ds[u][reg] = st[(4 * L.g + reg) * DVS_ATTNB_TLD + L.r];
                    dvs_wave_sync();
                    *(f4*)(st + L.r * DVS_ATTNB_TLD + 4 * L.g) = pT[u] * mk[u];
                    dvs_wave_sync();
#pragma unroll
                    for (int reg = 0; reg < 4; ++reg) pd[u][reg] = st[(4 * L.g + reg) * DVS_ATTNB_TLD + L.r];
                    dvs_wave_sync();
                }
            }
            {
                f4 qa = f4_zero(), qb = f4_zero();
#pragma unroll
                for (int kk = 0; kk < 4; ++kk) {
                    qa = dvs_mfma(kN[t][kk], dsT[0][kk], qa);
                    qb = dvs_mfma(kN[t][kk], dsT[1][kk], qb);
                }
                const f4 dq = f4{qa[0], qa[1], qb[2], qb[3]} * scale;
                if (live) ((f4*)(a.gq + dg * DVS_TILE))[t * 64 + L.lane] = dq;
            }
            {
                f4 ka = f4_zero(), kb = f4_zero(), va = f4_zero(), vb = f4_zero();
#pragma unroll
                for (int kk = 0; kk < 4; ++kk) {
                    ka = dvs_mfma(qN[t][kk], ds[0][kk], ka);
                    kb = dvs_mfma(qN[t][kk], ds[1][kk], kb);
                    va = dvs_mfma(dON[t][kk], pd[0][kk], va);
                    vb = dvs_mfma(dON[t][kk], pd[1][kk], vb);
                }
                if (live) {
                    ((f4*)(a.gk + dg * DVS_TILE))[t * 64 + L.lane] = f4{ka[0], ka[1], kb[2], kb[3]};
                    ((f4*)(a.gv + dg * DVS_TILE))[t * 64 + L.lane] = f4{va[0], va[1], vb[2], vb[3]};
                }
            }
            DVS_SCHED_FENCE();
        }
        dvs_group_barrier(G, L);
        dvs_coop_dw_bf(aWo, abo, (const dvs_bf16*)l.slots, (const dvs_bf16*)l.slots + 2 * DVS_SCR, 2 * 2 * DVS_SCR, L);
        dvs_group_barrier(G, L);
        if (base == dvs_bid() * NW) DVS_STAMP(dvs_stamps_bwd, mine, 7);
    }
    DvsBwdTail tail;
    DVS_STAMP(dvs_stamps_bwd, mine, 2);
    dvs_tail_issue(tail, next, has_next);
    const DvsTouch touch = dvs_touch_first(next, has_next, NW, L.wave, L.lane);
    DVS_STAMP(dvs_stamps_bwd, mine, 3);
    dvs_lds_barrier();
    DVS_STAMP(dvs_stamps_bwd, mine, 4);
    float* slab = a.slab + (size_t)dvs_bid() * a.P;
    float* const bufo = dvs_bwd_epi(smem);
    float* red = bufo + 4096;
    dvs_coop_stage<NW>(bufo, aWo, L);
    red[L.wave * 64 + L.lane] = 0.f;
    dvs_wave_sync();
    if (L.r == 0) {
#pragma unroll
        for (int reg = 0; reg < 4; ++reg) red[L.wave * 64 + 16 * (L.wave & 3) + 4 * L.g + reg] = abo[reg];
    }
    dvs_lds_barrier();
    dvs_coop_flush<NW>(bufo, slab + a.o_out_w, aWo, L, false, true);
    if (dvs_tid() < 64) {
        float s = 0.f;
        for (int w = 0; w < NW; ++w) s += red[w * 64 + dvs_tid()];
        slab[a.o_out_b + dvs_tid()] = s;
    }
    dvs_bwd_tail_end(tail, touch, mine, next, has_next, smem);
}
```

### dags_vae_search_amd/csrc/dvs_device.h

```cpp
#pragma once

#ifndef DVS_EMU
#include <hip/hip_runtime.h>
typedef float dvs_f32x4 __attribute__((ext_vector_type(4)));
#define DVS_DYN_LDS(name) extern __shared__ __attribute__((aligned(16))) char name[]
#else
#define DVS_DYN_LDS(name) char* name = emu::g_block->dyn_smem
#endif

#include <stdint.h>

typedef dvs_f32x4 f4;

constexpr int DVS_D = 64;
constexpr int DVS_LD = 68;
constexpr int DVS_TOK = 16;
constexpr int DVS_TILE = DVS_TOK * DVS_D;
constexpr int DVS_SCR = DVS_TOK * DVS_LD;

struct DvsRecord {
    uint8_t label[16];
    uint8_t pos[16];
    uint16_t parents[16];
    uint16_t allowed[16];
// ... 209 lines not shown
#ifndef DVS_EMU
__device__ __forceinline__ void dvs_swap16(float& a, float& b) {
    asm volatile("s_nop 1\n\tv_permlane16_swap_b32 %0, %1" : "+v"(a), "+v"(b));
}
__device__ __forceinline__ void dvs_swap32(float& a, float& b) {
    asm volatile("s_nop 1\n\tv_permlane32_swap_b32 %0, %1" : "+v"(a), "+v"(b));
}
__device__ __forceinline__ float dvs_add_x16(float v) { float a = v, b = v; dvs_swap16(a, b); return a + b; }
__device__ __forceinline__ float dvs_add_x32(float v) { float a = v, b = v; dvs_swap32(a, b); return a + b; }
__device__ __forceinline__ float dvs_max_x16(float v) { float a = v, b = v; dvs_swap16(a, b); return fmaxf(a, b); }
__device__ __forceinline__ float dvs_max_x32(float v) { float a = v, b = v; dvs_swap32(a, b); return fmaxf(a, b); }
#else
__device__ __forceinline__ float dvs_add_x16(float v) { return v + __shfl_xor(v, 16); }
__device__ __forceinline__ float dvs_add_x32(float v) { return v + __shfl_xor(v, 32); }
__device__ __forceinline__ float dvs_max_x16(float v) { return fmaxf(v, __shfl_xor(v, 16)); }
__device__ __forceinline__ float dvs_max_x32(float v) { return fmaxf(v, __shfl_xor(v, 32)); }
#endif
__device__ __forceinline__ float dvs_sum_g(float v) { return dvs_add_x32(dvs_add_x16(v)); }
__device__ __forceinline__ float dvs_max_g(float v) { return dvs_max_x32(dvs_max_x16(v)); }
__device__ __forceinline__ float dvs_sum_r(float v) {
    v += __shfl_xor(v, 1);
    v += __shfl_xor(v, 2);
    v += __shfl_xor(v, 4);
    v += __shfl_xor(v, 8);
    return v;
}
__device__ __forceinline__ float dvs_sum_wave(float v) { return dvs_sum_g(dvs_sum_r(v)); }
__device__ __forceinline__ float dvs_tile_sum(const f4 (&x)[4]) {
    float s = 0.f;
#pragma unroll
    for (int t = 0; t < 4; ++t) s += (x[t][0] + x[t][1]) + (x[t][2] + x[t][3]);
    return dvs_sum_g(s);
}

__device__ __forceinline__ void dvs_ln_stats(const f4 (&x)[4], float& mean, float& rstd) {
    mean = dvs_tile_sum(x) * (1.f / 64.f);
    float s = 0.f;
#pragma unroll
    for (int t = 0; t < 4; ++t)
#pragma unroll
        for (int kk = 0; kk < 4; ++kk) {
            const float d = x[t][kk] - mean;
            s += d * d;
        }
    rstd = 1.0f / sqrtf(dvs_sum_g(s) * (1.f / 64.f) + 1e-5f);
}

constexpr uint32_t DVS_SITE_GEN_EDGES = 300u, DVS_SITE_GEN_LABELS = 301u, DVS_SITE_GEN_COUNTS = 302u;
constexpr uint32_t DVS_SITE_HC_PERTURB = 400u;
__device__ __forceinline__ uint32_t dvs_fmix32(uint32_t x) {
    x ^= x >> 16;
    x *= 0x85EBCA6Bu;
    x ^= x >> 13;
    x *= 0xC2B2AE35u;
    x ^= x >> 16;
    return x;
}
__device__ __forceinline__ uint32_t dvs_site_key(uint32_t seed_lo, uint32_t seed_hi, uint32_t site, uint32_t dag) {
    uint32_t k = dvs_fmix32(seed_lo ^ ((site + 1u) * 0x632BE5ABu));
    k = dvs_fmix32(k ^ seed_hi ^ (dag * 0x9E3779B1u));
    return k;
}
__device__ __forceinline__ uint32_t dvs_draw(uint32_t key, uint32_t pair) { return dvs_fmix32(key ^ (pair * 0x9E3779B1u)); }

struct DvsDrop {
    uint32_t thr16;
    float scale;
    int on;
};
template <int NTILE = 4>
__device__ __forceinline__ void dvs_dropout_tile(f4 (&x)[NTILE], uint32_t key, const DvsDrop& D, const Lane& L, int tok0 = 0) {
    if (!D.on) return;
#pragma unroll
    for (int t = 0; t < NTILE; ++t) {
        const uint32_t p0 = (uint32_t)((tok0 + L.r) * 64 + 16 * t + 4 * L.g) >> 1;
        const uint32_t h0 = dvs_draw(key, p0), h1 = dvs_draw(key, p0 + 1);
        x[t][0] = ((h0 & 0xFFFFu) >= D.thr16) ? x[t][0] * D.scale : 0.f;
        x[t][1] = ((h0 >> 16) >= D.thr16) ? x[t][1] * D.scale : 0.f;
        x[t][2] = ((h1 & 0xFFFFu) >= D.thr16) ? x[t][2] * D.scale : 0.f;
        x[t][3] = ((h1 >> 16) >= D.thr16) ? x[t][3] * D.scale : 0.f;
    }
}
template <int NTILE = 4>
__device__ __forceinline__ uint32_t dvs_dropout_bits(uint32_t key, const DvsDrop& D, const Lane& L, int tok0 = 0) {
    uint32_t bits = 0xFFFFFFFFu;
    if (D.on) {
        bits = 0;
#pragma unroll
        for (int t = 0; t < NTILE; ++t) {
            const uint32_t p0 = (uint32_t)((tok0 + L.r) * 64 + 16 * t + 4 * L.g) >> 1;
            const uint32_t h0 = dvs_draw(key, p0), h1 = dvs_draw(key, p0 + 1);
            bits |= ((h0 & 0xFFFFu) >= D.thr16 ? 1u : 0u) << (4 * t);
            bits |= ((h0 >> 16) >= D.thr16 ? 1u : 0u) << (4 * t + 1);
            bits |= ((h1 & 0xFFFFu) >= D.thr16 ? 1u : 0u) << (4 * t + 2);
            bits |= ((h1 >> 16) >= D.thr16 ? 1u : 0u) << (4 * t + 3);
        }
    }
    return bits;
}
template <int NTILE = 4>
__device__ __forceinline__ void dvs_dropout_apply(f4 (&x)[NTILE], uint32_t bits, const DvsDrop& D) {
    if (!D.on) return;
#pragma unroll
    for (int t = 0; t < NTILE; ++t)
#pragma unroll
        for (int kk = 0; kk < 4; ++kk) x[t][kk] = ((bits >> (4 * t + kk)) & 1u) ? x[t][kk] * D.scale : 0.f;
}
__device__ __forceinline__ float dvs_dropout_elem(float v, uint32_t key, uint32_t e, const DvsDrop& D) {
    const uint32_t h = dvs_draw(key, e >> 1);
    const uint32_t half = (e & 1u) ? (h >> 16) : (h & 0xFFFFu);
    return (half >= D.thr16) ? v * D.scale : 0.f;
}
```

### dags_vae_search_amd/csrc/dvs_host.h

```cpp
#pragma once
#include <stddef.h>
#include <stdint.h>

#include "../../include/dvs.h"

constexpr int DVS_LAYERS = 3;
constexpr int DVS_HEADS = 8;
constexpr int DVS_LATENT = 32;
constexpr int DVS_FCH = 32;
constexpr int DVS_EMB = 32;
constexpr int DVS_MAXTOK = 16;
constexpr int DVS_WTOK = 48;
constexpr int DVS_FC_PARTS = 16;
constexpr int DVS_NSLOTS = 17;

struct DvsAttnP { int64_t in_w, in_b, out_w, out_b; };
struct DvsFfnP { int64_t l1_w, l1_b, l2_w, l2_b; };
struct DvsNormP { int64_t w, b; };

struct DvsLayout {
    int64_t W1, W2, lab_w, lab_b;
    struct { DvsAttnP sa; DvsFfnP ff; DvsNormP n1, n2; } enc[DVS_LAYERS];
    int64_t fc1_w, fc1_b, fc2_w, fc2_b;
    struct { DvsAttnP sa, ca; DvsFfnP ff; DvsNormP n1, n2, n3; } dec[DVS_LAYERS];
    int64_t node0_w, node0_b, node2_w, node2_b, edge0_w, edge0_b, edge2_w, edge2_b, fc3_w, fc3_b;
    int64_t total;
};

DvsLayout dvs_make_layout(int N, int C, dvs_param_entry* table , int cap, int* count);

struct DvsDropH {
    uint32_t thr16;
    float scale;
    int on;
};

struct DvsDims {
    int B, N, C, training;
    int NT;
    DvsDropH drop;
    uint32_t seed_lo, seed_hi, dag_offset;
    float beta, eps_scale;
    int debug;
};

struct DvsWorkspace {
    size_t act[DVS_NSLOTS];
    size_t stats[DVS_NSLOTS];
    size_t enc_out;
    size_t mu, logvar, z, epsv;
    size_t mem;
    size_t dag_loss;
    size_t gA, gB;
    size_t gq, gk, gv;
    size_t gmem;
    size_t genc;
    size_t gz;
    size_t slabs;
    size_t fcpart;
    size_t wimg;
    size_t limg;
    size_t qkv[9];
    size_t total_floats;
    int nslab;
};

DvsWorkspace dvs_make_workspace(int B, int NT, int64_t P, int nslab, bool wide);
```

### dags_vae_search_amd/csrc/dvs_kernels.h

```cpp
#pragma once
#include "dvs_device.h"
#include "dvs_host.h"
#include "dvs_stage.h"

#ifndef DVS_EMU
typedef hipStream_t dvs_stream_t;
#else
typedef void* dvs_stream_t;
#endif

struct DvsLN {
    const float* stats;
    const float* g;
    const float* b;
};

struct PackArgs {
    int B, N, C;
    const float* lab1h;
    const float* pos1h;
    const float* adj;
    const uint8_t* tmask;
    DvsRecord* rec;
    int* status;
};

struct EmbedArgs {
    DvsDims dims;
    const DvsRecord* rec;
    const float *W1, *W2, *lab_w, *lab_b;
    const float* embimg;
    float* out;
    int site;
    float* out2;
    int site2;
    const float* gout;
    float* slab;
    int64_t P;
    int64_t oW1, oW2, olab_w, olab_b;
};

struct AttnArgs {
    DvsDims dims;
    const DvsRecord* rec;
    const float* xin;
    DvsLN ln;
    const float* kv;
    const float *in_w, *in_b, *out_w, *out_b;
    const void* wimg;
    float* out_pre;
    float* out_stats;
    int site_prob, site_post;
    float* qkv;
};

struct FfnArgs {
    DvsDims dims;
    const float* xin;
    DvsLN ln;
    const float *l1_w, *l1_b, *l2_w, *l2_b;
    const void* wimg;
    float* out_pre;
    float* out_stats;
    float* out_norm;
    const float *ng, *nb;
    int site_hidden, site_post;
};

struct LatentArgs {
    DvsDims dims;
    const float* xenc;
    const float *fc1_w, *fc1_b, *fc2_w, *fc2_b, *fc3_w, *fc3_b;
    const float* limg;
    const float* eps_in;
    float *mu, *logvar, *z, *epsv;
    float* mem;
    float* dag_loss;
};

struct LossArgs {
    DvsDims dims;
    const DvsRecord* rec;
    const float* xin;
    DvsLN ln;
    const float *node0_w, *node0_b, *node2_w, *node2_b, *edge0_w, *edge0_b, *edge2_w, *edge2_b;
    const void* wimg;
    float* dag_loss;
    const float* gcoef;
    float* gout;
    float* slab;
    int64_t P;
    int64_t o_node0_w, o_node0_b, o_node2_w, o_node2_b, o_edge0_w, o_edge0_b, o_edge2_w, o_edge2_b, o_ln_g, o_ln_b;
};

struct FinalizeArgs {
    int B;
    float beta;
    const float* dag_loss;
    int* status;
    float* losses;
    float* host_tail;
    uint32_t host_seq;
};

struct BuildArgs {
    int B, N, C;
    const uint8_t* labels;
    const uint16_t* preds;
    DvsRecord* rec;
    int* status;
};
void dvs_launch_build_records(const BuildArgs& a, dvs_stream_t st);
void dvs_launch_pack(const PackArgs& a, dvs_stream_t st);
void dvs_launch_embed_fwd(const EmbedArgs& a, int grid, int nw, dvs_stream_t st);
enum { DVS_FPH_ATTN = 0, DVS_FPH_FFN = 1, DVS_FPH_LATENT = 2 };
#define DVS_FWD_STACK_PHASES 9
struct FwdPhase {
    int kind, pad;
    union {
        AttnArgs a;
        FfnArgs f;
        LatentArgs l;
    } u;
};
struct FwdStackArgs {
    int nphase, pad;
    FwdPhase ph[DVS_FWD_STACK_PHASES];
    DvsStagePlan plan[DVS_FWD_STACK_PHASES];
};
static_assert(sizeof(FwdStackArgs) <= 4096, "kernel argument block limit");
void dvs_launch_fwd_stack(const FwdStackArgs& s, int tag, int grid, int nw, dvs_stream_t st);
void dvs_launch_attn_fwd(const AttnArgs& a, int grid, int nw, dvs_stream_t st);
void dvs_launch_ffn_fwd(const FfnArgs& a, int grid, int nw, dvs_stream_t st);
void dvs_launch_latent_fwd(const LatentArgs& a, dvs_stream_t st);
void dvs_launch_loss_fwd(const LossArgs& a, int grid, int nw, dvs_stream_t st);
void dvs_launch_finalize(const FinalizeArgs& a, dvs_stream_t st);
void dvs_launch_unfrag(const float* frag, float* out, int B, dvs_stream_t st);

void dvs_prof_begin(const char* name, dvs_stream_t st);
void dvs_prof_end(dvs_stream_t st);
void dvs_note_hip_error(const char* what, int hip_error, const char* hip_message);
#define DVS_LAUNCH_AS(name, kernel, grid, block, lds, st, ...)                                 \
    do {                                                                                       \
        dvs_prof_begin(name, st);                                                              \
        hipLaunchKernelGGL(kernel, grid, block, lds, st, __VA_ARGS__);                         \
        const hipError_t dvs_le_ = hipGetLastError();                                          \
        if (dvs_le_ != hipSuccess) dvs_note_hip_error(name, (int)dvs_le_, hipGetErrorString(dvs_le_)); \
        dvs_prof_end(st);                                                                      \
    } while (0)
// ... 151 lines not shown
```

### dags_vae_search_amd/csrc/dvs_stage.h

```cpp
#pragma once
#include "dvs_device.h"

constexpr int DVS_PLAN_VECS = 6;
struct DvsStagePlan {
    const f4* src;
    int dst16;
    int n16;
    const float* vsrc[DVS_PLAN_VECS];
    unsigned short vdst[DVS_PLAN_VECS];
    unsigned short vbase[DVS_PLAN_VECS];
    unsigned short vlen[DVS_PLAN_VECS];
    int vperm;
    int nvec;
    int zero_int;
    int phase;
    const float* cold[2];
    int cold_tiles;
};

#ifdef DVS_STAMPS
constexpr int DVS_STAMP_IDS = 8, DVS_STAMP_PHASES = 32, DVS_STAMP_WAVES = 8, DVS_STAMP_WGS = 256;
#define DVS_STAMP_DECL(name) __device__ unsigned long long name[DVS_STAMP_WGS * DVS_STAMP_WAVES * DVS_STAMP_PHASES * DVS_STAMP_IDS]
#define DVS_STAMP(buf, pp, id)                                                                                              \
    do {                                                                                                                    \
        if ((dvs_tid() & 63) == 0 && dvs_bid() < DVS_STAMP_WGS && (dvs_tid() >> 6) < DVS_STAMP_WAVES)                        \
            buf[(((size_t)dvs_bid() * DVS_STAMP_WAVES + (dvs_tid() >> 6)) * DVS_STAMP_PHASES + ((pp)->phase & 31)) *          \
                    DVS_STAMP_IDS + (id)] = __builtin_amdgcn_s_memtime();                                                    \
    } while (0)
#define DVS_ACC_STAMP_DECL(name) __device__ unsigned long long name[256 * 8 * 8]
#define DVS_ACC_STAMP_AT(buf, last, nw, ids, k)                                                                             \
    do {                                                                                                                    \
        const unsigned long long now_ = __builtin_amdgcn_s_memtime();                                                       \
        if ((dvs_tid() & 63) == 0 && dvs_bid() < 256) buf[(dvs_bid() * (nw) + (dvs_tid() >> 6)) * (ids) + (k)] += now_ - last; \
        last = now_;                                                                                                        \
    } while (0)
#define DVS_ACC_STAMP(buf, last, k) DVS_ACC_STAMP_AT(buf, last, 8, 8, k)
#define DVS_STAMP_READER(name)                                                                                              \
    extern "C" int dvs_debug_read_stamps_##name(void* out, size_t bytes, int clear) {                                       \
        if (bytes > sizeof(dvs_stamps_##name)) bytes = sizeof(dvs_stamps_##name);                                           \
        if (hipMemcpyFromSymbol(out, HIP_SYMBOL(dvs_stamps_##name), bytes) != hipSuccess) return 1;                         \
        void* p = nullptr;                                                                                                  \
        if (clear && (hipGetSymbolAddress(&p, HIP_SYMBOL(dvs_stamps_##name)) != hipSuccess ||                               \
                      hipMemset(p, 0, sizeof(dvs_stamps_##name)) != hipSuccess))                                            \
            return 2;                                                                                                       \
        return 0;                                                                                                           \
    }
#else
#define DVS_STAMP(buf, pp, id) ((void)0)
#define DVS_ACC_STAMP(buf, last, k) ((void)0)
#define DVS_ACC_STAMP_AT(buf, last, nw, ids, k) ((void)0)
#endif

#ifndef DVS_EMU
#define DVS_HD __host__ __device__
#else
#define DVS_HD
#endif
#define DVS_FAKE_LDS ((char*)(uintptr_t)(1u << 20))
DVS_HD inline void dvs_plan_clear(DvsStagePlan& p) {
    p.src = nullptr;
    p.dst16 = 0;
    p.n16 = 0;
    for (int i = 0; i < DVS_PLAN_VECS; ++i) {
        p.vsrc[i] = nullptr;
        p.vdst[i] = 0;
        p.vbase[i] = 0;
        p.vlen[i] = 0;
    }
    p.phase = 0;
    p.nvec = 0;
    p.vperm = 0;
    p.zero_int = -1;
    p.cold[0] = p.cold[1] = nullptr;
    p.cold_tiles = 0;
}
DVS_HD inline void dvs_plan_cold(DvsStagePlan& p, const float* a, const float* b, int tiles) {
    p.cold[0] = a ? a : b;
    p.cold[1] = b ? b : a;
    p.cold_tiles = (a || b) ? tiles : 0;
}
DVS_HD inline void dvs_plan_seg(DvsStagePlan& p, const char* smem, const void* lds_dst, const void* src, int n_bf16) {
    p.src = (const f4*)src;
    p.dst16 = (int)(((const char*)lds_dst - smem) >> 4);
    p.n16 = n_bf16 >> 3;
}
DVS_HD inline void dvs_plan_vec(DvsStagePlan& p, const char* smem, const float* lds_dst, const float* src, int n,
                                bool perm = false) {
    for (int base = 0; base < n; base += 64) {
        if (p.nvec >= DVS_PLAN_VECS) {
            p.nvec = DVS_PLAN_VECS + 1;
            return;
        }
        p.vsrc[p.nvec] = src;
        p.vdst[p.nvec] = (unsigned short)(((const char*)lds_dst - smem) >> 2);
        p.vbase[p.nvec] = (unsigned short)base;
        p.vlen[p.nvec] = (unsigned short)n;
        if (perm) p.vperm |= 1 << p.nvec;
        ++p.nvec;
    }
}

constexpr int DVS_PF_THREADS = 256;
constexpr int DVS_PF_BWD = 9, DVS_PF_FWD = 14, DVS_PF_BWD_TAIL = 18, DVS_PF_FWD_TAIL = 27;
template <int NCH>
struct DvsPrefetch {
    f4 v[NCH];
    float s[2];
};

#ifndef DVS_EMU
typedef const __attribute__((address_space(4))) DvsStagePlan* DvsPlanK;
#else
typedef const DvsStagePlan* DvsPlanK;
#endif

DVS_HD inline bool dvs_plan_ok(const DvsStagePlan& p) { return p.nvec <= DVS_PLAN_VECS; }
void dvs_note_hip_error(const char* what, int hip_error, const char* hip_message);
DVS_HD inline void dvs_plan_seal(DvsStagePlan& p) {
#if !defined(__HIP_DEVICE_COMPILE__)
    if (!dvs_plan_ok(p)) {
        dvs_note_hip_error("staging plan", -1, "more than DVS_PLAN_VECS vector units (launcher bug)");
        p.nvec = DVS_PLAN_VECS;
    }
#endif
    for (int i = 0; i < DVS_PLAN_VECS; ++i)
        if (i >= p.nvec || !p.vsrc[i] || p.vlen[i] <= 0) {
            p.vsrc[i] = (const float*)p.src;
            p.vbase[i] = 0;
            p.vlen[i] = 0;
        }
}

__device__ __forceinline__ int dvs_uniform(int v) {
#ifndef DVS_EMU
    return __builtin_amdgcn_readfirstlane(v);
#else
    return v;
#endif
}
struct DvsPlanHead {
    const char* src;
    int dst, nwc, rot, wave, nw, lane16;
};
template <bool ROT, class PP>
__device__ __forceinline__ DvsPlanHead dvs_plan_head(PP p, int tid, int step) {
    DvsPlanHead h;
    h.src = (const char*)p->src;
    h.dst = p->dst16 * 16;
    h.nwc = p->n16 >> 6;
    h.rot = ROT ? (int)(((unsigned)dvs_bid() * 2654435761u) % (unsigned)(h.nwc > 0 ? h.nwc : 1)) : 0;
    h.wave = dvs_uniform(tid >> 6);
    h.nw = step >> 6;
    h.lane16 = (tid & 63) * 16;
    return h;
}
template <bool ROT>
__device__ __forceinline__ bool dvs_plan_slot(const DvsPlanHead& h, int u, int& byte) {
    int c = u * h.nw + h.wave;
    const bool live = c < h.nwc;
    if (ROT) {
        c += h.rot;
        c = c >= h.nwc ? c - h.nwc : c;
    }
    byte = ((live ? c : 0) << 10) + h.lane16;
    return live;
}

template <bool ROT, int NCH, class PP>
__device__ __forceinline__ void dvs_prefetch_issue(DvsPrefetch<NCH>& pf, PP p, int tid, int step) {
    const DvsPlanHead h = dvs_plan_head<ROT>(p, tid, step);
#pragma unroll
    for (int u = 0; u < NCH; ++u) {
        int byte;
        dvs_plan_slot<ROT>(h, u, byte);
        pf.v[u] = *(const f4*)(h.src + (unsigned)byte);
    }
#pragma unroll
    for (int q = 0; q < 2; ++q) {
        const int j = h.wave + q * h.nw, jc = j < DVS_PLAN_VECS ? j : 0;
        const int idx = p->vbase[jc] + (tid & 63);
        const int ic = (j < DVS_PLAN_VECS && idx < p->vlen[jc]) ? idx : 0;
        pf.s[q] = p->vsrc[jc][((p->vperm >> jc) & 1) ? dvs_pi(ic) : ic];
    }
}
template <bool ROT, int NCH, class PP>
__device__ __forceinline__ void dvs_prefetch_commit(const DvsPrefetch<NCH>& pf, PP p, char* smem, int tid, int step) {
    const DvsPlanHead h = dvs_plan_head<ROT>(p, tid, step);
#pragma unroll
    for (int u = 0; u < NCH; ++u) {
        int byte;
        if (dvs_plan_slot<ROT>(h, u, byte)) *(f4*)(smem + h.dst + byte) = pf.v[u];
    }
    float* ldsf = (float*)smem;
#pragma unroll
    for (int q = 0; q < 2; ++q) {
        const int j = h.wave + q * h.nw, jc = j < DVS_PLAN_VECS ? j : 0;
        const int idx = p->vbase[jc] + (tid & 63);
        if (j < DVS_PLAN_VECS && idx < p->vlen[jc]) ldsf[p->vdst[jc] + idx] = pf.s[q];
    }
    if (p->zero_int >= 0 && tid < 2) ((int*)smem)[p->zero_int + tid] = 0;
}
struct DvsTouch {
    float v[2];
};
template <class PP>
__device__ __forceinline__ DvsTouch dvs_touch_first(PP next, bool has_next, int nw, int wave, int lane) {
    DvsTouch t;
    t.v[0] = t.v[1] = 0.f;
    if (has_next && next->cold_tiles > 0) {
        int tile = dvs_bid() * nw + wave;
        tile = tile < next->cold_tiles ? tile : 0;
        const size_t off = (size_t)tile * 1024 + (size_t)lane * 16;
        t.v[0] = next->cold[0][off];
        t.v[1] = next->cold[1][off];
    }
    return t;
}
__device__ __forceinline__ void dvs_touch_done(const DvsTouch& t) {
#ifndef DVS_EMU
    asm volatile("" ::"v"(t.v[0]), "v"(t.v[1]));
#else
    (void)t;
#endif
}

template <int NCH, class PP>
__device__ __forceinline__ void dvs_stage_now(PP p, char* smem) {
    DvsPrefetch<NCH> pf;
    dvs_prefetch_issue<true>(pf, p, dvs_tid(), (int)blockDim.x);
    dvs_prefetch_commit<true>(pf, p, smem, dvs_tid(), (int)blockDim.x);
}
```

### dags_vae_search_amd/csrc/k_backward.hip

```cpp
#include "dvs_bwd_phases.h"
#include "dvs_latent_bwd.h"

template <int NW>
__global__ __launch_bounds__(64 * NW) void k_ffn_bwd(FfnBwdArgs a, DvsStagePlan plan) {
    DVS_DYN_LDS(smem);
    dvs_ffn_bwd_phase<NW>(a, smem, &plan, true, &plan, false);
}
void dvs_launch_ffn_bwd(const FfnBwdArgs& a, int grid, int nw, dvs_stream_t st) {
    const size_t lds = ffnb_lds_bytes();
    DvsStagePlan plan;
    ffnb_plan(plan, a, DVS_FAKE_LDS);
    if (nw == 4) {
        DVS_SET_LDS(k_ffn_bwd<4>, lds);
        DVS_LAUNCH_AS("k_ffn_bwd", k_ffn_bwd<4>, dim3(grid), dim3(256), lds, st, a, plan);
    } else {
        DVS_SET_LDS(k_ffn_bwd<8>, lds);
        DVS_LAUNCH_AS("k_ffn_bwd", k_ffn_bwd<8>, dim3(grid), dim3(512), lds, st, a, plan);
    }
}

template <int NPROJ, int NW>
__global__ __launch_bounds__(64 * NW) void k_proj_bwd(ProjBwdArgs a, DvsStagePlan plan) {
    DVS_DYN_LDS(smem);
    dvs_proj_bwd_phase<NPROJ, NW>(a, smem, &plan, true, &plan, false);
}

#define DVS_PROJ_LAUNCH(NP, NWV)                                                               \
    do {                                                                                       \
        DVS_SET_LDS((k_proj_bwd<NP, NWV>), bytes);                                             \
        DVS_LAUNCH_AS("k_proj_bwd<" #NP ">", (k_proj_bwd<NP, NWV>), dim3(grid), dim3(64 * NWV), bytes, st, a, plan); \
    } while (0)
void dvs_launch_proj_bwd(const ProjBwdArgs& a, int nproj, int grid, int nw, dvs_stream_t st) {
    const size_t bytes = projb_lds_bytes(nproj);
    DvsStagePlan plan;
    projb_plan(plan, a, nproj, DVS_FAKE_LDS);
    if (nw == 4) {
        if (nproj == 3) DVS_PROJ_LAUNCH(3, 4);
        else if (nproj == 2) DVS_PROJ_LAUNCH(2, 4);
        else DVS_PROJ_LAUNCH(1, 4);
    } else {
        if (nproj == 3) DVS_PROJ_LAUNCH(3, 8);
        else if (nproj == 2) DVS_PROJ_LAUNCH(2, 8);
        else DVS_PROJ_LAUNCH(1, 8);
    }
}

template <int NW>
__global__ __launch_bounds__(64 * NW) void k_attn_bwd(AttnBwdArgs a, DvsStagePlan plan) {
    DVS_DYN_LDS(smem);
    dvs_attn_bwd_phase<NW>(a, smem, &plan, true, &plan, false);
}

void dvs_launch_attn_bwd(const AttnBwdArgs& a, int grid, int nw, dvs_stream_t st) {
    const size_t lds = attnb_lds_floats() * 4;
    DvsStagePlan plan;
    attnb_plan(plan, a, DVS_FAKE_LDS);
    if (nw == 4) {
        DVS_SET_LDS(k_attn_bwd<4>, lds);
        DVS_LAUNCH_AS("k_attn_bwd", k_attn_bwd<4>, dim3(grid), dim3(256), lds, st, a, plan);
    } else {
        DVS_SET_LDS(k_attn_bwd<8>, lds);
        DVS_LAUNCH_AS("k_attn_bwd", k_attn_bwd<8>, dim3(grid), dim3(512), lds, st, a, plan);
    }
}

template <int TAG, int NW>
__global__ __launch_bounds__(64 * NW) void k_bwd_stack(BwdStackArgs s) {
    DVS_DYN_LDS(smem);
#ifndef DVS_EMU
    const DvsPlanK plans =
        ((const __attribute__((address_space(4))) BwdStackArgs*)__builtin_amdgcn_kernarg_segment_ptr())->plan;
#else
    const DvsPlanK plans = s.plan;
#endif
    if (TAG == 1 && NW == 8 && s.has_latent) {
        const int step = (int)gridDim.x * 8, B = s.lat.dims.B;
        for (int base = dvs_bid() * 8; base < B; base += 2 * step) {
            dvs_latent_bwd_group<8>(s.lat, (f4 (*)[2][64])smem, base, base + step);
            __syncthreads();
        }
    }
    for (int i = 0; i < s.nphase; ++i) {
        const BwdPhase& ph = s.ph[i];
        const bool first = i == 0;
        const bool more = i + 1 < s.nphase;
        const DvsPlanK mine = plans + i;
        const DvsPlanK next = plans + (more ? i + 1 : i);
        switch (ph.kind) {
            case DVS_PH_FFN: dvs_ffn_bwd_phase<NW>(ph.u.f, smem, mine, first, next, more); break;
            case DVS_PH_ATTN: dvs_attn_bwd_phase<NW>(ph.u.a, smem, mine, first, next, more); break;
            case DVS_PH_PROJ1: dvs_proj_bwd_phase<1, NW>(ph.u.p, smem, mine, first, next, more); break;
            case DVS_PH_PROJ2: dvs_proj_bwd_phase<2, NW>(ph.u.p, smem, mine, first, next, more); break;
            default: dvs_proj_bwd_phase<3, NW>(ph.u.p, smem, mine, first, next, more); break;
        }
    }
}

void dvs_launch_bwd_stack(const BwdStackArgs& s_in, int tag, int grid, int nw, dvs_stream_t st) {
    BwdStackArgs s = s_in;
    for (int i = 0; i < s.nphase; ++i) {
        dvs_bwd_plan(s.plan[i], s.ph[i], DVS_FAKE_LDS);
        s.plan[i].phase = i;
    }
#ifdef DVS_STAMPS
    static int stamp_seq = 0;
    for (int i = 0; i < s.nphase; ++i) s.plan[i].phase = (stamp_seq % 3) * DVS_STACK_PHASES + i;
    ++stamp_seq;
#endif
    size_t lds = 0;
    for (int i = 0; i < s.nphase; ++i) {
        const int k = s.ph[i].kind;
        const size_t b = k == DVS_PH_FFN ? ffnb_lds_bytes() : k == DVS_PH_ATTN ? attnb_lds_floats() * 4 : projb_lds_bytes(k - DVS_PH_PROJ1 + 1);
        lds = b > lds ? b : lds;
    }
#define DVS_BSTACK_LAUNCH(TG, NWV)                                                             \
    do {                                                                                       \
        DVS_SET_LDS((k_bwd_stack<TG, NWV>), lds);                                              \
        DVS_LAUNCH_AS("k_bwd_stack<" #TG ">", (k_bwd_stack<TG, NWV>), dim3(grid), dim3(64 * NWV), lds, st, s); \
    } while (0)
    if (nw == 4) {
        if (tag == 0) DVS_BSTACK_LAUNCH(0, 4);
        else DVS_BSTACK_LAUNCH(1, 4);
    } else {
        if (tag == 0) DVS_BSTACK_LAUNCH(0, 8);
        else DVS_BSTACK_LAUNCH(1, 8);
    }
}

__global__ __launch_bounds__(256) void k_reduce_slabs(ReduceArgs a) {
    __shared__ f4 part[4][64];
    const int q = threadIdx.x >> 6, c = threadIdx.x & 63;
    const int64_t i4 = ((int64_t)blockIdx.x * 64 + c) * 4;
    const bool in = i4 < a.P;
    f4 s = f4_zero();
    if (in) {
        const bool fc = (i4 >= a.fc_lo1 && i4 < a.fc_hi1) || (i4 >= a.fc_lo2 && i4 < a.fc_hi2);
        const float* src = fc ? a.fcpart : a.slab;
        const int n = fc ? DVS_FC_PARTS : a.nslab;
        const int per = (n + 3) / 4;
        const int k1 = (q + 1) * per < n ? (q + 1) * per : n;
        int k = q * per;
        for (; k + 8 <= k1; k += 8) {
            f4 v[8];
#pragma unroll
            for (int u = 0; u < 8; ++u) v[u] = *(const f4*)(src + (size_t)(k + u) * a.P + i4);
#pragma unroll
            for (int u = 0; u < 8; ++u) s += v[u];
        }
        for (; k < k1; ++k) s += *(const f4*)(src + (size_t)k * a.P + i4);
    }
    part[q][c] = s;
    __syncthreads();
    if (q == 0) {
        const f4 tot = (part[0][c] + part[1][c]) + (part[2][c] + part[3][c]);
        if (in) *(f4*)(a.grads + i4) = tot;
        if (a.sqpart) {
            float ss = 0.f;
#pragma unroll
            for (int e = 0; e < 4; ++e) ss += (in && i4 + e < a.P) ? tot[e] * tot[e] : 0.f;
            ss = dvs_sum_wave(ss);
            if (c == 0) a.sqpart[blockIdx.x] = ss;
        }
    }
}

void dvs_launch_reduce_slabs(const ReduceArgs& a, dvs_stream_t st) {
    const int64_t n4 = (a.P + 3) / 4;
    DVS_LAUNCH(k_reduce_slabs, dim3((unsigned)((n4 + 63) / 64)), dim3(256), 0, st, a);
}

#ifdef DVS_STAMPS
DVS_STAMP_READER(bwd)
#endif
```

### dags_vae_search_amd/csrc/k_backward_heads.hip

```cpp
#include "dvs_backward.h"
#include "dvs_wimg.h"
#include "dvs_latent_bwd.h"
#include "dvs_loss.h"

#ifdef DVS_STAMPS
__device__ unsigned long long dvs_stamps_lossb[256 * 4 * 12];
DVS_STAMP_READER(lossb)
#endif
#define LBSTAMP(k) DVS_ACC_STAMP_AT(dvs_stamps_lossb, lst_, 4, 12, k)
__global__ __launch_bounds__(256) void k_loss_bwd(LossArgs a, DvsStagePlan plan) {
#ifdef DVS_STAMPS
    unsigned long long lst_ = __builtin_amdgcn_s_memtime();
#endif
    DVS_DYN_LDS(smem);
    const LossLds l = loss_lds(smem);
    const int N = a.dims.N, C = a.dims.C;
    dvs_stage_now<(LOSS_CHUNKS + 3) / 4>(&plan, smem);
    __syncthreads();
    const Lane L = dvs_lane();
    float* scrV = l.scr + L.wave * 3 * DVS_SCR;
    float* scrU = scrV + DVS_SCR;
    float* dlm = scrU + DVS_SCR;
    const float b2 = l.b2[0];
    const float gr = a.gcoef[0];
// ... 185 lines not shown
        (void)touch;
#endif
        LBSTAMP(7);
    }
    __syncthreads();
    LBSTAMP(8);
    float* slab = a.slab + (size_t)blockIdx.x * a.P;
    {
        dvs_coop_flush<4>(nullptr, slab + a.o_edge0_w, aWa, L, false, false, 128);
        dvs_coop_flush<4>(nullptr, slab + a.o_edge0_w + 64, aWb, L, false, false, 128);
        if (L.r == 0) {
#pragma unroll
            for (int reg = 0; reg < 4; ++reg) slab[a.o_edge0_b + 16 * L.wave + 4 * L.g + reg] = abV[reg];
        }
        float* rN1 = (float*)smem;
        float* rN2 = rN1 + 4 * 2048;
        float* rv = rN2 + 4 * 512;
        dvs_stage_dw<2, 4>(rN1, dWn1, L);
        dvs_stage_dw<1, 2>(rN2, dWn2, L);
        float* es = rv + 192 + 4 * DVS_RED_VEC + 16 + L.wave * DVS_SCR;
        dvs_stage_vec<2>(rv, dbn1, es, L);
        dvs_stage_vec<1>(rv + 128, dbn2, es, L);
        dvs_stage_vec<4>(rv + 192 + DVS_RED_VEC, dw2, es, L);
        dvs_stage_vec<4>(rv + 192 + 2 * DVS_RED_VEC, dgam, es, L);
        dvs_stage_vec<4>(rv + 192 + 3 * DVS_RED_VEC, dbet, es, L);
        const float sb2 = dvs_sum_wave(L.g == 0 ? db2 : 0.f);
        float* rb2 = rv + 192 + 4 * DVS_RED_VEC;
        if (L.lane == 0) rb2[L.wave] = sb2;
        __syncthreads();
        dvs_flush_dw<2, 4>(rN1, slab + a.o_node0_w, L);
        dvs_flush_dw<1, 2>(rN2, slab + a.o_node2_w, L, C, 32);
        dvs_flush_vec<2>(rv, slab + a.o_node0_b, L);
        dvs_flush_vec<1>(rv + 128, slab + a.o_node2_b, L, C);
        dvs_flush_vec<4>(rv + 192 + DVS_RED_VEC, slab + a.o_edge2_w, L);
        dvs_flush_vec<4>(rv + 192 + 2 * DVS_RED_VEC, slab + a.o_ln_g, L);
        dvs_flush_vec<4>(rv + 192 + 3 * DVS_RED_VEC, slab + a.o_ln_b, L);
        if (threadIdx.x == 0) {
            float s = rb2[0];
            for (int w = 1; w < L.nwaves; ++w) s += rb2[w];
            slab[a.o_edge2_b] = s;
        }
    }
    LBSTAMP(9);
}

void dvs_launch_loss_bwd(const LossArgs& a, int grid, dvs_stream_t st) {
    const size_t lds = loss_lds_bytes(4, 3);
    DvsStagePlan plan;
    loss_plan(plan, a);
    DVS_SET_LDS(k_loss_bwd, lds);
    DVS_LAUNCH(k_loss_bwd, dim3(grid), dim3(256), lds, st, a, plan);
}

__global__ __launch_bounds__(512) void k_embed_bwd(EmbedArgs a, const float* gout2, int site2, DvsStagePlan plan) {
    DVS_DYN_LDS(smem);
    const int N = a.dims.N, C = a.dims.C;
    float* W1 = (float*)smem;
    float* W2 = W1 + 2 * DVS_MAXTOK * DVS_LD;
    float* labw = W2 + 64 * EMB_LDW2;
    float* labb = labw + 32 * 16;
    float* scr0 = labb + 32;
    if (blockDim.x >= 512) dvs_stage_now<3>(&plan, smem);
    else dvs_stage_now<5>(&plan, smem);
    __syncthreads();
    const Lane L = dvs_lane();
    const DvsDrop D = dvs_drop_of(a.dims);
    float* scr = scr0 + L.wave * DVS_SCR;
    f4 dW2[4][2], dlabb[2], dW1a[1][4], dW1b[1][4], dlab[2][1];
#pragma unroll
    for (int i = 0; i < 4; ++i) dW2[i][0] = dW2[i][1] = dW1a[0][i] = dW1b[0][i] = f4_zero();
    dlabb[0] = dlabb[1] = dlab[0][0] = dlab[1][0] = f4_zero();
    for (int dag = blockIdx.x * L.nwaves + L.wave; dag < a.dims.B; dag += gridDim.x * L.nwaves) {
        const DvsRecord* rec = a.rec + dag;
        const bool valid = L.r < N;
        const int label = rec->label[L.r];
        const uint32_t gdag = a.dims.dag_offset + dag;
        const EmbSel sel = dvs_emb_selectors(rec, N, scr, L);
        f4 e1[4];
        dvs_emb_hidden(e1, W1, N, sel, L);
        for (int src = 0; src < 2; ++src) {
            const float* gsrc = src == 0 ? a.gout : gout2;
            if (!gsrc) continue;
            const int site = src == 0 ? a.site : site2;
            f4 gx[4];
            dvs_load_grad(gx, gsrc, dag, N, L);
            f4 dle[2];
#pragma unroll
            for (int t = 0; t < 2; ++t)
#pragma unroll
                for (int kk = 0; kk < 4; ++kk) {
                    const int f = 16 * t + 4 * L.g + kk;
                    const float pre = labw[f * 16 + label] + labb[f];
                    dle[t][kk] = (valid && pre > 0.f) ? gx[t][kk] : 0.f;
                }
            dlabb[0] += dle[0];
            dlabb[1] += dle[1];
            const uint32_t k1 = dvs_site_key(a.dims.seed_lo, a.dims.seed_hi, site, gdag);
            f4 m1[4] = {f4_splat(1.f), f4_splat(1.f), f4_splat(1.f), f4_splat(1.f)};
            dvs_dropout_tile(m1, k1, D, L);
            f4 e1d[4];
#pragma unroll
            for (int t = 0; t < 4; ++t) e1d[t] = e1[t] * m1[t];
            f4 de2[2] = {gx[2], gx[3]};
            dvs_dropout_tile<2>(de2, dvs_site_key(a.dims.seed_lo, a.dims.seed_hi, site + 1, gdag), D, L);
            f4 e1dN[4], de2N[2], dleN[2];
            dvs_t2n<4>(e1dN, e1d, scr, L);
            dvs_t2n<2>(de2N, de2, scr, L);
            dvs_t2n<2>(dleN, dle, scr, L);
            dvs_outer_acc<4, 2>(dW2, e1dN, de2N);
            f4 de1[4] = {f4_zero(), f4_zero(), f4_zero(), f4_zero()};
            dvs_mat_T<4, 2>(de1, de2, W2, EMB_LDW2, 0, L);
#pragma unroll
            for (int t = 0; t < 4; ++t) de1[t] *= m1[t];
#pragma unroll
            for (int t = 0; t < 4; ++t)
#pragma unroll
                for (int kk = 0; kk < 4; ++kk) de1[t][kk] = e1[t][kk] > 0.f ? de1[t][kk] : 0.f;
            f4 de1N[4];
            dvs_t2n<4>(de1N, de1, scr, L);
            f4 selA[1] = {sel.selA}, parA[1] = {sel.parA}, labA[1] = {sel.labA};
            dvs_outer_acc<1, 4>(dW1a, selA, de1N);
            dvs_outer_acc<1, 4>(dW1b, parA, de1N);
            dvs_outer_acc<2, 1>(dlab, dleN, labA);
        }
    }
    __syncthreads();
    float* slab = a.slab + (size_t)blockIdx.x * a.P;
    float* r1a = (float*)smem;
    float* r1b = r1a + 8 * 1024;
    float* rlab = r1b + 8 * 1024;
    float* rv = rlab + 8 * 512;
    dvs_stage_dw<1, 4>(r1a, dW1a, L);
    dvs_stage_dw<1, 4>(r1b, dW1b, L);
    dvs_stage_dw<2, 1>(rlab, dlab, L);
    dvs_stage_vec<2>(rv, dlabb, rv + 8 * 32 + L.wave * DVS_SCR, L);
    __syncthreads();
    dvs_flush_dw<1, 4>(r1a, slab + a.oW1, L, N, 64);
    dvs_flush_dw<1, 4>(r1b, slab + a.oW1 + (size_t)N * 64, L, N, 64);
    dvs_flush_dw<2, 1>(rlab, slab + a.olab_w, L, 32, C, C);
    dvs_flush_vec<2>(rv, slab + a.olab_b, L);
    __syncthreads();
    float* rW2 = (float*)smem;
    dvs_stage_dw<4, 2>(rW2, dW2, L);
    __syncthreads();
    dvs_flush_dw<4, 2>(rW2, slab + a.oW2, L);
}

void dvs_launch_embed_bwd(const EmbedArgs& a, const float* gout2, int site2, int grid, int nw, dvs_stream_t st) {
    size_t lds = (2 * DVS_MAXTOK * DVS_LD + 64 * EMB_LDW2 + 32 * 16 + 32 + 8 * DVS_SCR) * 4;
    const size_t red = (8 * (1024 + 1024 + 512) + 8 * 32 + 8 * DVS_SCR) * 4;
    if (lds < red) lds = red;
    DvsStagePlan plan;
    dvs_plan_clear(plan);
    dvs_plan_seg(plan, DVS_FAKE_LDS, DVS_FAKE_LDS, a.embimg, 2 * DvsEmbImg::FLOATS);
    dvs_plan_seal(plan);
    DVS_SET_LDS(k_embed_bwd, lds);
    DVS_LAUNCH(k_embed_bwd, dim3(grid), dim3(nw == 4 ? 256 : 512), lds, st, a, gout2, site2, plan);
}

constexpr int LATB_WAVES = 8;
__global__ __launch_bounds__(64 * LATB_WAVES) void k_latent_bwd(LatentBwdArgs a) {
    __shared__ f4 part[LATB_WAVES][2][64];
    dvs_latent_bwd_group<LATB_WAVES>(a, part, (int)blockIdx.x * 16, (int)blockIdx.x * 16 + 8);
}

void dvs_launch_latent_bwd(const LatentBwdArgs& a, dvs_stream_t st) {
    const int ngroups = (a.dims.B + 15) / 16;
    DVS_LAUNCH(k_latent_bwd, dim3(ngroups), dim3(64 * LATB_WAVES), 0, st, a);
}

constexpr int FC_MT = 4;
__global__ __launch_bounds__(512) void k_fc_dw(FcDwArgs a) {
    __shared__ f4 red[4][FC_MT * 6 + 2][64];
    const Lane L = dvs_lane();
    const int B = a.dims.B, N = a.dims.N;
    const int ldw = N * 64;
    const int nmg = 16 * a.dims.NT;
    const int mg = blockIdx.x % nmg, q = blockIdx.x / nmg;
    const size_t dstride = (size_t)a.dims.NT * DVS_TILE;
    const int per_q = (B + DVS_FC_PARTS - 1) / DVS_FC_PARTS;
    const int per_w = (per_q + 7) / 8;
    const int d0 = q * per_q + L.wave * per_w;
    int d1 = d0 + per_w;
    if (d1 > (q + 1) * per_q) d1 = (q + 1) * per_q;
    if (d1 > B) d1 = B;
    f4 acc[FC_MT][4], acc3[FC_MT][2];
    f4 bs3 = f4_zero();
// ... 130 lines not shown
```

### dags_vae_search_amd/csrc/k_forward.hip

```cpp
#include "dvs_kernels.h"
#include "dvs_wimg.h"

constexpr int PACK_DAGS = 4;
__device__ __forceinline__ void pack_stream(float* dst, const float* __restrict__ src, size_t nfloats) {
    const size_t n4 = nfloats >> 2;
    size_t i = threadIdx.x;
    for (; i + 3 * blockDim.x < n4; i += 4 * blockDim.x) {
        f4 v[4];
#pragma unroll
        for (int u = 0; u < 4; ++u) v[u] = *(const f4*)(src + 4 * (i + u * blockDim.x));
#pragma unroll
        for (int u = 0; u < 4; ++u) *(f4*)(dst + 4 * (i + u * blockDim.x)) = v[u];
    }
    for (; i < n4; i += blockDim.x) *(f4*)(dst + 4 * i) = *(const f4*)(src + 4 * i);
    for (size_t i = 4 * n4 + threadIdx.x; i < nfloats; i += blockDim.x) dst[i] = src[i];
}
__global__ __launch_bounds__(8 * 16 * PACK_DAGS) void k_pack(PackArgs a) {
    DVS_DYN_LDS(smem);
    const int N = a.N, C = a.C;
    const int dag0 = blockIdx.x * PACK_DAGS;
    const int nd = (a.B - dag0 < PACK_DAGS) ? a.B - dag0 : PACK_DAGS;
    float* s_lab = (float*)smem;
    float* s_pos = s_lab + PACK_DAGS * 16 * 16;
    float* s_adj = s_pos + PACK_DAGS * 16 * 16;
// ... 101 lines not shown
        for (int u = 0; u < v; ++u)
            if ((p >> u) & 1u) s_child[u + 2][tid] |= (unsigned short)(1u << (v + 2));
        if (p & ((1u << v) - 1u)) haspred |= 1u << v;
    }
    for (int v = 0; v < n; ++v)
        if (!((haspred >> v) & 1u)) s_child[1][tid] |= (unsigned short)(1u << (v + 2));
    for (int v = 0; v < N - 1; ++v)
        if (s_child[v][tid] == 0) s_child[v][tid] = (unsigned short)(1u << out_id);
    for (int v = 0; v < 16; ++v) s_indeg[v][tid] = 0;
    for (int u = 0; u < N; ++u) {
        unsigned c = s_child[u][tid];
        while (c) {
            const int v = __ffs((int)c) - 1;
            c &= c - 1;
            s_indeg[v][tid]++;
        }
    }
    int tail = 0;
    for (int v = 0; v < N; ++v)
        if (s_indeg[v][tid] == 0) s_order[tail++][tid] = (unsigned char)v;
    for (int head = 0; head < tail && head < N; ++head) {
        unsigned c = s_child[s_order[head][tid]][tid];
        while (c) {
            const int v = __ffs((int)c) - 1;
            c &= c - 1;
            if (--s_indeg[v][tid] == 0 && tail < 16) s_order[tail++][tid] = (unsigned char)v;
        }
    }
    if (tail != N) bad |= 8;
    for (int v = 0; v < N; ++v) s_reach[v][tid] = (unsigned short)(s_child[v][tid] | (1u << v));
    for (int k = 0; k < N; ++k) {
        const unsigned rk = s_reach[k][tid];
        for (int v = 0; v < N; ++v)
            if ((s_reach[v][tid] >> k) & 1u) s_reach[v][tid] |= (unsigned short)rk;
    }
    DvsRecord* r = a.rec + dag;
    for (int i = 0; i < 16; ++i) {
        int label = 0, pos = 0;
        unsigned parents = 0, allowed = 1u << i;
        if (i < N) {
            if (i == 0) label = 2;
            else if (i == 1) label = 0;
            else if (i == out_id) label = 1;
            else {
                label = a.labels[(size_t)dag * n + (i - 2)] + 3;
                if (label >= a.C) { bad |= 1; label = 0; }
            }
            pos = s_order[i][tid];
            allowed = 0;
            for (int j = 0; j < N; ++j) {
                if ((s_child[j][tid] >> i) & 1u) parents |= 1u << j;
                if ((s_reach[j][tid] >> i) & 1u) allowed |= 1u << j;
            }
        }
        r->label[i] = (uint8_t)label;
        r->pos[i] = (uint8_t)pos;
        r->parents[i] = (uint16_t)parents;
        r->allowed[i] = (uint16_t)allowed;
    }
    if (bad) atomicOr(a.status, bad);
}

void dvs_launch_build_records(const BuildArgs& a, dvs_stream_t st) {
    DVS_LAUNCH(k_build_records, dim3((a.B + 255) / 256), dim3(256), 0, st, a);
}

struct EmbLds {
    float *W1, *W2, *labw, *labb, *scr;
};
__device__ __forceinline__ EmbLds emb_lds(char* smem) {
    EmbLds l;
    l.W1 = (float*)smem;
    l.W2 = l.W1 + 2 * DVS_MAXTOK * DVS_LD;
    l.labw = l.W2 + 64 * EMB_LDW2;
    l.labb = l.labw + 32 * 16;
    l.scr = l.labb + 32;
    return l;
}
static size_t emb_lds_floats(int nwaves) {
    const size_t n = 2 * DVS_MAXTOK * DVS_LD + 64 * EMB_LDW2 + 32 * 16 + 32 + (size_t)nwaves * 16;
    return n > (size_t)DvsEmbImg::FLOATS ? n : (size_t)DvsEmbImg::FLOATS;
}

__global__ __launch_bounds__(1024) void k_embed_fwd(EmbedArgs a, DvsStagePlan plan) {
    DVS_DYN_LDS(smem);
    const int N = a.dims.N, C = a.dims.C;
    const EmbLds l = emb_lds(smem);
    if (blockDim.x >= 1024) dvs_stage_now<2>(&plan, smem);
    else dvs_stage_now<5>(&plan, smem);
    __syncthreads();
    const Lane L = dvs_lane();
    const DvsDrop D = dvs_drop_of(a.dims);
    float* scr = l.scr + L.wave * 16;
    for (int dag = blockIdx.x * L.nwaves + L.wave; dag < a.dims.B; dag += gridDim.x * L.nwaves) {
        const DvsRecord* rec = a.rec + dag;
        const bool valid = L.r < N;
        const EmbSel sel = dvs_emb_selectors(rec, N, scr, L);
        f4 eh[4];
        dvs_emb_hidden(eh, l.W1, N, sel, L);
        const uint32_t gdag = a.dims.dag_offset + dag;
        const int label = rec->label[L.r];
        for (int v = 0; v < (a.out2 ? 2 : 1); ++v) {
            const int site = v ? a.site2 : a.site;
            f4 e1[4];
#pragma unroll
            for (int t = 0; t < 4; ++t) e1[t] = eh[t];
            dvs_dropout_tile(e1, dvs_site_key(a.dims.seed_lo, a.dims.seed_hi, site, gdag), D, L);
            f4 x[4];
            f4 e2[2] = {f4_zero(), f4_zero()};
#pragma unroll
            for (int t = 0; t < 4; ++t) {
                const f4 w0 = dvs_wcol(l.W2, EMB_LDW2, 0, t, L), w1 = dvs_wcol(l.W2, EMB_LDW2, 16, t, L);
#pragma unroll
                for (int kk = 0; kk < 4; ++kk) {
                    e2[0] = dvs_mfma(w0[kk], e1[t][kk], e2[0]);
                    e2[1] = dvs_mfma(w1[kk], e1[t][kk], e2[1]);
                }
            }
            {
                f4 tmp[2] = {e2[0], e2[1]};
                dvs_dropout_tile<2>(tmp, dvs_site_key(a.dims.seed_lo, a.dims.seed_hi, site + 1, gdag), D, L);
                x[2] = tmp[0];
                x[3] = tmp[1];
            }
#pragma unroll
            for (int t = 0; t < 2; ++t)
#pragma unroll
                for (int kk = 0; kk < 4; ++kk) {
                    const int f = 16 * t + 4 * L.g + kk;
                    x[t][kk] = valid ? fmaxf(l.labw[f * 16 + label] + l.labb[f], 0.f) : 0.f;
                }
            if (!valid) { x[2] = f4_zero(); x[3] = f4_zero(); }
            dvs_store_tile(v ? a.out2 : a.out, dag, x, L);
        }
    }
}

void dvs_launch_embed_fwd(const EmbedArgs& a, int grid, int nw, dvs_stream_t st) {
    const size_t lds = emb_lds_floats(16) * 4;
    DvsStagePlan plan;
    dvs_plan_clear(plan);
    dvs_plan_seg(plan, DVS_FAKE_LDS, DVS_FAKE_LDS, a.embimg, 2 * DvsEmbImg::FLOATS);
    dvs_plan_seal(plan);
    DVS_SET_LDS(k_embed_fwd, lds);
    DVS_LAUNCH(k_embed_fwd, dim3(grid), dim3(nw == 4 ? 256 : 1024), lds, st, a, plan);
}

#ifdef DVS_STAMPS
DVS_STAMP_DECL(dvs_stamps_fwd);
struct DvsLatTag { int phase; };
__device__ const DvsLatTag dvs_lat_tag = {6};
#define DVS_LAT_STAMP(id) DVS_STAMP(dvs_stamps_fwd, &dvs_lat_tag, id)
DVS_ACC_STAMP_DECL(dvs_stamps_attn);
#endif
#define ASTAMP(k) DVS_ACC_STAMP(dvs_stamps_attn, ast_, k)
#include "dvs_latent.h"
struct AttnLds {
    dvs_bf16 *Win, *Wout;
    float *inb, *outb, *lg, *lb;
};
DVS_HD inline AttnLds attn_lds(char* smem) {
    AttnLds l;
    l.Win = (dvs_bf16*)smem;
    l.Wout = l.Win + 3 * 192 * DVS_LDB;
    l.inb = (float*)(l.Wout + 3 * 64 * DVS_LDB);
    l.outb = l.inb + 192;
    l.lg = l.outb + 64;
    l.lb = l.lg + 64;
    return l;
}
static size_t attn_lds_bytes() { return 3 * 256 * DVS_LDB * sizeof(dvs_bf16) + (192 + 64 + 128) * sizeof(float); }

inline void attn_plan(DvsStagePlan& p, const AttnArgs& a, char* smem) {
    const AttnLds l = attn_lds(smem);
    dvs_plan_clear(p);
    dvs_plan_seg(p, smem, l.Win, (const dvs_bf16*)a.wimg + DvsAttnImg::Win, (int)(DvsAttnImg::WoutT - DvsAttnImg::Win));
    dvs_plan_vec(p, smem, l.inb, a.in_b, 192, true);
    dvs_plan_vec(p, smem, l.outb, a.out_b, 64);
    dvs_plan_vec(p, smem, l.lg, a.ln.g, a.ln.stats ? 64 : 0);
    dvs_plan_vec(p, smem, l.lb, a.ln.b, a.ln.stats ? 64 : 0);
    dvs_plan_seal(p);
}

__device__ __forceinline__ void attn_qkv(f4 (&q)[4], f4 (&k)[4], f4 (&v)[4], const Split3T& x, const Split3T& kv,
                                         const AttnLds& l, const Lane& L) {
#pragma unroll
    for (int t = 0; t < 4; ++t) {
        q[t] = dvs_vecT(l.inb, t, L);
        k[t] = dvs_vecT(l.inb + 64, t, L);
        v[t] = f4_splat(l.inb[128 + 16 * t + L.r]);
    }
    dvs_matb3<4>(q, x, l.Win, 192, 0, L);
    dvs_matb3<4>(k, kv, l.Win, 192, 64, L);
    dvs_matb3<4, true>(v, kv, l.Win, 192, 128, L);
    const float scale = 0.35355339059327373f;
#pragma unroll
    for (int t = 0; t < 4; ++t) q[t] *= scale;
}

__device__ __forceinline__ void attn_scores_T(f4 (&s)[8], const f4 (&q)[4], const f4 (&k)[4], const Lane& L) {
#pragma unroll
    for (int h = 0; h < 8; ++h) s[h] = f4_zero();
#pragma unroll
    for (int kk = 0; kk < 2; ++kk)
#pragma unroll
        for (int t = 0; t < 4; ++t) {
            s[2 * t] = dvs_mfma(k[t][kk], q[t][kk], s[2 * t]);
            s[2 * t + 1] = dvs_mfma(k[t][kk + 2], q[t][kk + 2], s[2 * t + 1]);
        }
}
__device__ __forceinline__ void attn_softmax_T(f4 (&p)[8], float (&m)[8], float (&den)[8], const f4 (&s)[8],
                                               unsigned allowed_r, const Lane& L) {
    bool ok[4];
#pragma unroll
    for (int reg = 0; reg < 4; ++reg) ok[reg] = (allowed_r >> (4 * L.g + reg)) & 1u;
#pragma unroll
    for (int h = 0; h < 8; ++h) {
        float mx = -3.0e38f;
#pragma unroll
        for (int reg = 0; reg < 4; ++reg) mx = ok[reg] ? fmaxf(mx, s[h][reg]) : mx;
        m[h] = mx;
    }
#pragma unroll
    for (int h = 0; h < 8; ++h) m[h] = dvs_max_x16(m[h]);
#pragma unroll
    for (int h = 0; h < 8; ++h) m[h] = dvs_max_x32(m[h]);
#pragma unroll
    for (int h = 0; h < 8; ++h) {
        float sum = 0.f;
#pragma unroll
        for (int reg = 0; reg < 4; ++reg) {
            p[h][reg] = ok[reg] ? __expf(s[h][reg] - m[h]) : 0.f;
            sum += p[h][reg];
        }
        den[h] = sum;
    }
#pragma unroll
    for (int h = 0; h < 8; ++h) den[h] = dvs_add_x16(den[h]);
#pragma unroll
    for (int h = 0; h < 8; ++h) den[h] = dvs_add_x32(den[h]);
#pragma unroll
    for (int h = 0; h < 8; ++h) p[h] *= (1.0f / den[h]);
}

__device__ __forceinline__ f4 attn_drop_T(f4 p, uint32_t key, int h, const DvsDrop& D, const Lane& L) {
    if (!D.on) return p;
    const uint32_t p0 = (uint32_t)((h * 16 + L.r) * 8 + 2 * L.g);
    const uint32_t h0 = dvs_draw(key, p0), h1 = dvs_draw(key, p0 + 1);
    p[0] = ((h0 & 0xFFFFu) >= D.thr16) ? p[0] * D.scale : 0.f;
    p[1] = ((h0 >> 16) >= D.thr16) ? p[1] * D.scale : 0.f;
    p[2] = ((h1 & 0xFFFFu) >= D.thr16) ? p[2] * D.scale : 0.f;
    p[3] = ((h1 >> 16) >= D.thr16) ? p[3] * D.scale : 0.f;
    return p;
}

template <class PP>
__device__ __forceinline__ void dvs_fwd_tail(PP next, bool has_next, char* smem, PP mine) {
    if (has_next) {
        DvsPrefetch<DVS_PF_FWD_TAIL> pf;
        const bool fetcher = dvs_tid() < DVS_PF_THREADS;
        if (fetcher) dvs_prefetch_issue<false>(pf, next, dvs_tid(), DVS_PF_THREADS);
        DVS_STAMP(dvs_stamps_fwd, mine, 3);
        dvs_lds_barrier();
        DVS_STAMP(dvs_stamps_fwd, mine, 4);
        if (fetcher) dvs_prefetch_commit<false>(pf, next, smem, dvs_tid(), DVS_PF_THREADS);
        DVS_STAMP(dvs_stamps_fwd, mine, 6);
    }
}

template <int NW, class PP>
__device__ __forceinline__ void dvs_attn_fwd_phase(const AttnArgs& a, char* smem, PP mine, bool stage_mine, PP next,
                                                   bool has_next) {
    const AttnLds l = attn_lds(smem);
    DVS_STAMP(dvs_stamps_fwd, mine, 0);
    if (stage_mine) {
        dvs_stage_now<(NW >= 8 ? DVS_PF_FWD : DVS_PF_FWD_TAIL)>(mine, smem);
        __syncthreads();
    }
    DVS_STAMP(dvs_stamps_fwd, mine, 1);
    const Lane L = dvs_lane();
    const DvsDrop D = dvs_drop_of(a.dims);
    const int N = a.dims.N;
#ifdef DVS_STAMPS
    unsigned long long ast_ = __builtin_amdgcn_s_memtime();
#endif
    bool gate = !stage_mine;
    for (int base = dvs_bid() * L.nwaves; base < a.dims.B; base += gridDim.x * L.nwaves) {
        const int dag = base + L.wave;
        if (dag >= a.dims.B) {
            DVS_PHASE_GATE(gate);
            continue;
        }
        ASTAMP(7);
        f4 x[4], dummy[4], kvt[4];
        float rstd;
        {
            DvsRawX rx;
            dvs_load_x_issue(rx, a.xin, a.ln, dag, L);
            if (a.kv) dvs_load_tile(kvt, a.kv, dag, L);
            DVS_PHASE_GATE(gate);
            dvs_load_x_finish<false>(x, dummy, rstd, rx, a.ln, l.lg, l.lb, N, L);
        }
#ifdef DVS_STAMPS
        asm volatile("s_waitcnt vmcnt(0)" ::: "memory");
#endif
        ASTAMP(0);
        f4 q[4], k[4], v[4];
        {
            const Split3T xs = dvs_split3_T(x);
            if (a.kv) {
                attn_qkv(q, k, v, xs, dvs_split3_T(kvt), l, L);
            } else {
                attn_qkv(q, k, v, xs, xs, l, L);
            }
        }
        ASTAMP(1);
        const unsigned allowed_r = a.rec[dag].allowed[L.r];
        const uint32_t gdag = a.dims.dag_offset + dag;
        const uint32_t kprob = dvs_site_key(a.dims.seed_lo, a.dims.seed_hi, a.site_prob, gdag);
        f4 s[8], p[8];
        float m[8], den[8];
        attn_scores_T(s, q, k, L);
        attn_softmax_T(p, m, den, s, allowed_r, L);
        ASTAMP(2);
#pragma unroll
        for (int h = 0; h < 8; ++h) p[h] = attn_drop_T(p[h], kprob, h, D, L);
        ASTAMP(3);
        f4 o[4];
        {
            f4 oa[4], ob[4];
#pragma unroll
            for (int t = 0; t < 4; ++t) oa[t] = ob[t] = f4_zero();
#pragma unroll
            for (int kk = 0; kk < 4; ++kk)
#pragma unroll
                for (int t = 0; t < 4; ++t) {
                    oa[t] = dvs_mfma(v[t][kk], p[2 * t][kk], oa[t]);
                    ob[t] = dvs_mfma(v[t][kk], p[2 * t + 1][kk], ob[t]);
                }
#pragma unroll
            for (int t = 0; t < 4; ++t) o[t] = f4{oa[t][0], oa[t][1], ob[t][2], ob[t][3]};
        }
        ASTAMP(4);
        f4 y[4];
#pragma unroll
        for (int t = 0; t < 4; ++t) y[t] = dvs_vecT(l.outb, t, L);
        dvs_matb3<4>(y, dvs_split3_T(o), l.Wout, 64, 0, L);
        ASTAMP(5);
        dvs_dropout_tile(y, dvs_site_key(a.dims.seed_lo, a.dims.seed_hi, a.site_post, gdag), D, L);
        const bool valid = L.r < N;
#pragma unroll
        for (int t = 0; t < 4; ++t)
#pragma unroll
            for (int kk = 0; kk < 4; ++kk) y[t][kk] = valid ? x[t][kk] + y[t][kk] : 0.f;
        dvs_store_pre(a.out_pre, a.out_stats, dag, y, L);
        ASTAMP(6);
    }
    DVS_PHASE_GATE(gate);
    DVS_STAMP(dvs_stamps_fwd, mine, 2);
    dvs_fwd_tail(next, has_next, smem, mine);
}

template <int NW>
__global__ __launch_bounds__(64 * NW) void k_attn_fwd(AttnArgs a, DvsStagePlan plan) {
    DVS_DYN_LDS(smem);
    dvs_attn_fwd_phase<NW>(a, smem, &plan, true, &plan, false);
}

void dvs_launch_attn_fwd(const AttnArgs& a, int grid, int nw, dvs_stream_t st) {
    const size_t lds = attn_lds_bytes();
    DvsStagePlan plan;
    attn_plan(plan, a, DVS_FAKE_LDS);
    if (nw == 4) {
        DVS_SET_LDS(k_attn_fwd<4>, lds);
        DVS_LAUNCH_AS("k_attn_fwd", k_attn_fwd<4>, dim3(grid), dim3(256), lds, st, a, plan);
    } else {
        DVS_SET_LDS(k_attn_fwd<8>, lds);
        DVS_LAUNCH_AS("k_attn_fwd", k_attn_fwd<8>, dim3(grid), dim3(512), lds, st, a, plan);
    }
}

struct FfnLds {
    dvs_bf16 *W1, *W2;
    float *b1, *b2, *lg, *lb, *ng, *nb;
};
DVS_HD inline FfnLds ffn_lds(char* smem) {
    FfnLds l;
    l.W1 = (dvs_bf16*)smem;
    l.W2 = l.W1 + 3 * 64 * DVS_LDB;
    l.b1 = (float*)(l.W2 + 3 * 64 * DVS_LDB);
    l.b2 = l.b1 + 64;
    l.lg = l.b2 + 64;
    l.lb = l.lg + 64;
    l.ng = l.lb + 64;
    l.nb = l.ng + 64;
    return l;
}
static size_t ffn_lds_bytes() { return 6 * 64 * DVS_LDB * sizeof(dvs_bf16) + 6 * 64 * sizeof(float); }

inline void ffn_plan(DvsStagePlan& p, const FfnArgs& a, char* smem) {
    const FfnLds l = ffn_lds(smem);
    dvs_plan_clear(p);
    dvs_plan_seg(p, smem, l.W1, (const dvs_bf16*)a.wimg + DvsFfnImg::W1, (int)(6 * DVS_IMG64));
    dvs_plan_vec(p, smem, l.b1, a.l1_b, 64);
    dvs_plan_vec(p, smem, l.b2, a.l2_b, 64);
    dvs_plan_vec(p, smem, l.lg, a.ln.g, a.ln.stats ? 64 : 0);
    dvs_plan_vec(p, smem, l.lb, a.ln.b, a.ln.stats ? 64 : 0);
    dvs_plan_vec(p, smem, l.ng, a.ng, a.out_norm ? 64 : 0);
    dvs_plan_vec(p, smem, l.nb, a.nb, a.out_norm ? 64 : 0);
    dvs_plan_seal(p);
}

template <class PP>
__device__ __forceinline__ void dvs_ffn_fwd_phase(const FfnArgs& a, char* smem, PP mine, bool stage_mine, PP next,
                                                  bool has_next) {
    const FfnLds l = ffn_lds(smem);
    DVS_STAMP(dvs_stamps_fwd, mine, 0);
    if (stage_mine) {
        dvs_stage_now<DVS_PF_FWD>(mine, smem);
        __syncthreads();
    }
    DVS_STAMP(dvs_stamps_fwd, mine, 1);
    const Lane L = dvs_lane();
    const DvsDrop D = dvs_drop_of(a.dims);
    const int ntiles = a.dims.B * a.dims.NT;
    bool gate = !stage_mine;
    for (int base = dvs_bid() * L.nwaves; base < ntiles; base += gridDim.x * L.nwaves) {
        const int tile = base + L.wave;
        if (tile >= ntiles) {
            DVS_PHASE_GATE(gate);
            continue;
        }
        const DvsTile T = dvs_tile_of(tile, a.dims);
        f4 x[4], dummy[4];
        float rstd;
        {
            DvsRawX rx;
            dvs_load_x_issue(rx, a.xin, a.ln, tile, L);
            DVS_PHASE_GATE(gate);
            dvs_load_x_finish<false>(x, dummy, rstd, rx, a.ln, l.lg, l.lb, T.Nl, L);
        }
        const uint32_t gdag = a.dims.dag_offset + T.dag;
        f4 h[4];
#pragma unroll
        for (int t = 0; t < 4; ++t) h[t] = dvs_vecT(l.b1, t, L);
        dvs_matb3<4>(h, dvs_split3_T(x), l.W1, 64, 0, L);
#pragma unroll
        for (int t = 0; t < 4; ++t)
#pragma unroll
            for (int kk = 0; kk < 4; ++kk) h[t][kk] = fmaxf(h[t][kk], 0.f);
        dvs_dropout_tile(h, dvs_site_key(a.dims.seed_lo, a.dims.seed_hi, a.site_hidden, gdag), D, L, T.tok0);
        f4 y[4];
#pragma unroll
        for (int t = 0; t < 4; ++t) y[t] = dvs_vecT(l.b2, t, L);
        dvs_matb3<4>(y, dvs_split3_T(h), l.W2, 64, 0, L);
        dvs_dropout_tile(y, dvs_site_key(a.dims.seed_lo, a.dims.seed_hi, a.site_post, gdag), D, L, T.tok0);
        const bool valid = L.r < T.Nl;
#pragma unroll
        for (int t = 0; t < 4; ++t)
#pragma unroll
            for (int kk = 0; kk < 4; ++kk) y[t][kk] = valid ? x[t][kk] + y[t][kk] : 0.f;
        float mean, rs;
        dvs_ln_stats(y, mean, rs);
        dvs_store_tile(a.out_pre, tile, y, L);
        if (L.g == 0) {
            a.out_stats[(size_t)tile * 32 + L.r] = mean;
            a.out_stats[(size_t)tile * 32 + 16 + L.r] = rs;
        }
        if (a.out_norm) {
            f4 xn[4];
#pragma unroll
            for (int t = 0; t < 4; ++t) {
                const f4 g = dvs_vecT(l.ng, t, L), b = dvs_vecT(l.nb, t, L);
#pragma unroll
                for (int kk = 0; kk < 4; ++kk) xn[t][kk] = valid ? (y[t][kk] - mean) * rs * g[kk] + b[kk] : 0.f;
            }
            dvs_store_tile(a.out_norm, tile, xn, L);
        }
    }
    DVS_PHASE_GATE(gate);
    DVS_STAMP(dvs_stamps_fwd, mine, 2);
    dvs_fwd_tail(next, has_next, smem, mine);
}

__global__ __launch_bounds__(1024) void k_ffn_fwd(FfnArgs a, DvsStagePlan plan) {
    DVS_DYN_LDS(smem);
    dvs_ffn_fwd_phase(a, smem, &plan, true, &plan, false);
}

void dvs_launch_ffn_fwd(const FfnArgs& a, int grid, int nw, dvs_stream_t st) {
    const size_t lds = ffn_lds_bytes();
    DvsStagePlan plan;
    ffn_plan(plan, a, DVS_FAKE_LDS);
    DVS_SET_LDS(k_ffn_fwd, lds);
    DVS_LAUNCH(k_ffn_fwd, dim3(grid), dim3(nw == 4 ? 256 : 1024), lds, st, a, plan);
}

template <int TAG, int NW>
__global__ __launch_bounds__(64 * NW) void k_fwd_stack(FwdStackArgs s) {
    DVS_DYN_LDS(smem);
#ifndef DVS_EMU
    const DvsPlanK plans =
        ((const __attribute__((address_space(4))) FwdStackArgs*)__builtin_amdgcn_kernarg_segment_ptr())->plan;
#else
    const DvsPlanK plans = s.plan;
#endif
    for (int i = 0; i < s.nphase; ++i) {
        const FwdPhase& ph = s.ph[i];
        const bool first = i == 0, more = i + 1 < s.nphase;
        const DvsPlanK mine = plans + i;
        if (TAG == 0 && NW == 8 && ph.kind == DVS_FPH_LATENT) {
            const int step = (int)gridDim.x * 8, B = ph.u.l.dims.B;
            for (int base = dvs_bid() * 8; base < B; base += 2 * step) {
                __syncthreads();
                dvs_latent_fwd_group(ph.u.l, smem, base, base + step);
            }
            continue;
        }
        const bool more_img = more && s.ph[i + 1].kind != DVS_FPH_LATENT;
        const DvsPlanK next = plans + (more_img ? i + 1 : i);
        if (ph.kind == DVS_FPH_ATTN) dvs_attn_fwd_phase<NW>(ph.u.a, smem, mine, first, next, more_img);
        else dvs_ffn_fwd_phase(ph.u.f, smem, mine, first, next, more_img);
    }
}

void dvs_launch_fwd_stack(const FwdStackArgs& s_in, int tag, int grid, int nw, dvs_stream_t st) {
    FwdStackArgs s = s_in;
    for (int i = 0; i < s.nphase; ++i) {
        if (s.ph[i].kind == DVS_FPH_ATTN) attn_plan(s.plan[i], s.ph[i].u.a, DVS_FAKE_LDS);
        else if (s.ph[i].kind == DVS_FPH_FFN) ffn_plan(s.plan[i], s.ph[i].u.f, DVS_FAKE_LDS);
        else dvs_plan_clear(s.plan[i]);
        s.plan[i].phase = i;
    }
#ifdef DVS_STAMPS
    for (int i = 0; i < s.nphase; ++i) s.plan[i].phase = tag * DVS_FWD_STACK_PHASES + i;
#endif
    const size_t la = attn_lds_bytes(), lf = ffn_lds_bytes();
    const size_t lds = la > lf ? la : lf;
#define DVS_FSTACK_LAUNCH(TG, NWV)                                                             \
    do {                                                                                       \
        DVS_SET_LDS((k_fwd_stack<TG, NWV>), lds);                                              \
        DVS_LAUNCH_AS("k_fwd_stack<" #TG ">", (k_fwd_stack<TG, NWV>), dim3(grid), dim3(64 * NWV), lds, st, s); \
    } while (0)
    if (nw == 4) {
        if (tag == 0) DVS_FSTACK_LAUNCH(0, 4);
        else DVS_FSTACK_LAUNCH(1, 4);
    } else {
        if (tag == 0) DVS_FSTACK_LAUNCH(0, 8);
        else DVS_FSTACK_LAUNCH(1, 8);
    }
}

__global__ void k_unfrag(const float* frag, float* out, int B) {
    const size_t i = (size_t)blockIdx.x * blockDim.x + threadIdx.x;
    if (i >= (size_t)B * 1024) return;
    const size_t dag = i >> 10;
    const int e = (int)(i & 1023);
    const int t = e >> 8, lane = (e >> 2) & 63, kk = e & 3;
    const int r = lane & 15, g = lane >> 4;
    out[dag * 1024 + r * 64 + 16 * t + 4 * g + kk] = frag[i];
}
void dvs_launch_unfrag(const float* frag, float* out, int B, dvs_stream_t st) {
    const size_t n = (size_t)B * 1024;
    DVS_LAUNCH(k_unfrag, dim3((unsigned)((n + 255) / 256)), dim3(256), 0, st, frag, out, B);
}

#ifdef DVS_STAMPS
DVS_STAMP_READER(attn)
DVS_STAMP_READER(fwd)
#endif
```

### dags_vae_search_amd/engine.py

```python
from __future__ import annotations

import ctypes
from typing import Dict, Optional

import torch

from . import _lib as dl


def _ptr(t: Optional[torch.Tensor]):
    return None if t is None else ctypes.c_void_p(t.data_ptr())


def _nbytes(t: torch.Tensor) -> int:
    return t.numel() * t.element_size()


def _stream():
    return ctypes.c_void_p(torch.cuda.current_stream().cuda_stream)


def _require_cuda(t: torch.Tensor, what: str):
    if not t.is_cuda:
        raise RuntimeError(f"dags_vae_search_amd: {what} must live on the GPU (got device {t.device}); "
                           f"this package has no CPU path")


class PaceEngine:

    def __init__(self, n_tokens: int, n_classes: int):
        self.lib = dl.load()
        self.n_tokens = int(n_tokens)
        self.n_classes = int(n_classes)
        shape = dl.make_shape(1, n_tokens, n_classes)
        if self.lib.dvs_param_count(ctypes.byref(shape)) < 0:
            dl.check(self.lib, 1, "dvs_param_count")
        self.table, self.param_floats = dl.param_table(self.lib, shape)
        self.record_bytes = dl.record_bytes(self.lib, shape)
        self.wide = dl.is_wide(self.n_tokens, self.n_classes)
        self.tiles = (self.n_tokens + dl.TILE_TOKENS - 1) // dl.TILE_TOKENS
        self._ws: Optional[torch.Tensor] = None
        self._ws_batch = 0
        self._records: Optional[torch.Tensor] = None
        self._status: Optional[torch.Tensor] = None
        self._status_external = False

    def shape(self, batch, training=False, dropout=0.15, beta=0.005, eps_scale=0.01, dag_offset=0, seed=0):
        return dl.make_shape(batch, self.n_tokens, self.n_classes, training, dropout, beta, eps_scale, dag_offset, seed)

    def workspace(self, batch: int, device) -> torch.Tensor:
        if self._ws is None or self._ws_batch != batch or self._ws.device != device:
            shape = self.shape(batch)
            nbytes = self.lib.dvs_workspace_bytes(ctypes.byref(shape))
            if nbytes == 0:
                dl.check(self.lib, 1, "dvs_workspace_bytes")
            self._ws = torch.zeros((nbytes + 3) // 4, dtype=torch.float32, device=device)
            self._ws_batch = batch
            self._records = torch.empty(batch * self.record_bytes, dtype=torch.uint8, device=device)
            if not self._status_external or self._status.device != device:
                self._status = torch.zeros(1, dtype=torch.int32, device=device)
                self._status_external = False
        return self._ws

    def use_status(self, status: torch.Tensor):
        self._status = status
        self._status_external = True

    def _read_status(self) -> int:
        st = int(self._status.item())
        if st:
            self._status.zero_()
        return st

    def pack(self, features: Dict, check: bool = True, zero_status: bool = True) -> torch.Tensor:
        lab = features["vertex_label_features"]
        pos = features["vertex_position_features"]
        adj = features["adjacency_matrices"]
        tm = features["target_masks"]
        for name, t in (("vertex_label_features", lab), ("vertex_position_features", pos),
                        ("adjacency_matrices", adj), ("target_masks", tm)):
            _require_cuda(t, name)
        B, N, C = lab.shape
        if N != self.n_tokens or C != self.n_classes:
            raise AssertionError(f"Expected [B,{self.n_tokens},{self.n_classes}] label features, got {tuple(lab.shape)}")
        if tuple(pos.shape) != (B, N, N) or tuple(adj.shape) != (B, N, N) or tuple(tm.shape) != (8 * B, N, N):
            raise AssertionError("feature tensors have inconsistent shapes")
        def aligned(t, dtype):
            if t.dtype != dtype:
                t = t.to(dtype)
            if not t.is_contiguous():
                t = t.contiguous()
            return t if t.data_ptr() % 16 == 0 else t.clone()
        lab = aligned(lab, torch.float32)
        pos = aligned(pos, torch.float32)
        adj = aligned(adj, torch.float32)
        tm = aligned(tm, tm.dtype)
        tm = tm.view(torch.uint8) if tm.dtype == torch.bool else aligned(tm, torch.uint8)
        self.workspace(B, lab.device)
        if zero_status:
            self._status.zero_()
        shape = self.shape(B)
        dl.check(self.lib, self.lib.dvs_pack_features(ctypes.byref(shape), _ptr(lab), _ptr(pos), _ptr(adj), _ptr(tm),
                                                      _ptr(self._records), _nbytes(self._records), _ptr(self._status),
                                                      _stream()),
                 "dvs_pack_features")
        if check:
            st = self._read_status()
            if st:
                raise ValueError(f"features violate the prepare_features invariants (status bits {st:#x}: "
                                 f"1 = label/position row not one-hot, 2 = per-head masks differ, 4 = self masked)")
        return self._records

    def build_records(self, labels: torch.Tensor, preds: torch.Tensor, check: bool = True,
                      zero_status: bool = True) -> torch.Tensor:
        _require_cuda(labels, "labels")
        _require_cuda(preds, "preds")
        B, n = labels.shape
        if n != self.n_tokens - 3 or tuple(preds.shape) != (B, n):
            raise AssertionError(f"Expected {self.n_tokens - 3}, got instead {n}")
        labels = labels.contiguous().to(torch.uint8)
        preds = preds.contiguous().to(torch.int64 if self.wide else torch.int16)
        self.workspace(B, labels.device)
        if zero_status:
            self._status.zero_()
        shape = self.shape(B)
        dl.check(self.lib, self.lib.dvs_build_records(ctypes.byref(shape), _ptr(labels), _ptr(preds), _ptr(self._records),
                                                      _nbytes(self._records), _ptr(self._status), _stream()),
                 "dvs_build_records")
        if check:
            st = self._read_status()
            if st:
                raise ValueError(f"invalid compact DAG batch (status bits {st:#x}: 1 = label out of range, "
                                 f"8 = edge not from a lower to a higher vertex id)")
        return self._records

# ... 83 lines not shown
```

Before: 3.462 million DAGs/s.

## Save dropout masks as bitmasks in forward and reuse them in backward

The forward attention, FFN and embed kernels now write their dropout keep-bits to a per-DAG workspace buffer. The backward kernels load those bits instead of regenerating them with hash draws, and the cold-touch prefetch plan covers the bit buffers. This trades RNG recomputation in the backward pass for extra global stores and loads plus a larger training workspace. An environment variable restores the old redraw path.

```diff
diff --git a/dags_vae_search_amd/csrc/dvs_api.hip b/dags_vae_search_amd/csrc/dvs_api.hip
--- a/dags_vae_search_amd/csrc/dvs_api.hip
+++ b/dags_vae_search_amd/csrc/dvs_api.hip
@@ -220,7 +220,7 @@
     return l;
 }
 
-DvsWorkspace dvs_make_workspace(int B, int NT, int64_t P, int nslab, bool wide) {
+DvsWorkspace dvs_make_workspace(int B, int NT, int64_t P, int nslab, bool wide, bool training) {
     DvsWorkspace w;
     size_t off = 0;
     auto take = [&](size_t n) {
@@ -254,6 +254,7 @@
     w.wimg = take((DVS_WIMG_BF16 + 1) / 2);
     w.limg = take(DvsLatImg::floats(NT));
     for (int blk = 0; blk < 9; ++blk) w.qkv[blk] = take(wide ? (size_t)B * NT * 12 * 256 : 0);
+    w.dropbits = take(!wide && training ? DvsDropBits::PER_DAG * (size_t)B : 0);
     w.total_floats = off;
     return w;
 }
@@ -322,6 +323,7 @@
     static const bool on = env_on("DVS_SPLIT_STACK");
     return on;
 }
+static bool dropout_redraw() { return env_on("DVS_DROPOUT_REDRAW"); }
 static bool latent_kernels_off() {
     static const bool on = env_on("DVS_LATENT_KERNELS");
     return on;
@@ -350,6 +352,7 @@
     int nw;
     FwdGrids g;
     int slabs;
+    bool save_bits;
 };
 static Step make_step(const dvs_shape* s, const void* records, const float* params, void* workspace, void* stream) {
     Step c;
@@ -357,7 +360,7 @@
     c.L = dvs_make_layout(c.d.N, c.d.C, nullptr, 0, nullptr);
     c.wide = is_wide(s);
     const int nslab = num_slabs();
-    c.W = dvs_make_workspace(c.d.B, c.d.NT, c.L.total, nslab, c.wide);
+    c.W = dvs_make_workspace(c.d.B, c.d.NT, c.L.total, nslab, c.wide, c.d.training != 0);
     c.P = params;
     c.ws = (float*)workspace;
     c.rec = (const DvsRecord*)records;
@@ -372,6 +375,7 @@
     c.g.dags2 = c.d.B < 2 * c.g.dags ? c.d.B : 2 * c.g.dags;
     c.g.dec4 = grid_for(c.d.B, 4, nslab);
     c.slabs = active_slabs(c.d, c.wide, nslab);
+    c.save_bits = !c.wide && c.d.drop.on && !dropout_redraw();
     return c;
 }
 
@@ -488,6 +492,9 @@
 static inline const void* wimg_attn(const Step& c, int block) { return (const dvs_bf16*)(c.ws + c.W.wimg) + img_attn(block); }
 static inline const void* wimg_ffn(const Step& c, int block) { return (const dvs_bf16*)(c.ws + c.W.wimg) + img_ffn(block); }
 
+static uint32_t* dropbits_at(const Step& c, bool on, size_t off) {
+    return on ? (uint32_t*)(c.ws + c.W.dropbits) + off : nullptr;
+}
 static DvsLN ln_of(const Step& c, int slot, const DvsNormP* n) {
     if (!n) return DvsLN{nullptr, nullptr, nullptr};
     return DvsLN{c.ws + c.W.stats[slot], c.P + n->w, c.P + n->b};
@@ -526,6 +533,7 @@
     a.out_stats = c.ws + c.W.stats[out];
     a.site_prob = site0;
     a.site_post = site0 + 1;
+    a.dropbits = dropbits_at(c, c.save_bits, DvsDropBits::attn(block, c.d.B));
     return a;
 }
 
@@ -544,6 +552,7 @@
     f.out_stats = c.ws + c.W.stats[out];
     f.site_hidden = site0;
     f.site_post = site0 + 1;
+    f.dropbits = dropbits_at(c, c.save_bits, DvsDropBits::ffn(block, c.d.B));
     return f;
 }
 
@@ -720,9 +729,11 @@
 static void encoder_forward(const Step& c, const LatentArgs& lat, bool dec_embed = false, bool save_qkv = false) {
     EmbedArgs e = embed_args(c, 0);
     e.out = c.ws + c.W.act[0];
+    e.dropbits = dropbits_at(c, c.save_bits, DvsDropBits::emb(0, c.d.B));
     if (dec_embed) {
         e.out2 = c.ws + c.W.act[7];
         e.site2 = 2;
+        e.dropbits2 = dropbits_at(c, c.save_bits, DvsDropBits::emb(1, c.d.B));
     }
     launch_embed_fwd(c, e);
     FwdChain chain(c, 0);
diff --git a/dags_vae_search_amd/csrc/dvs_api_backward.inc b/dags_vae_search_amd/csrc/dvs_api_backward.inc
--- a/dags_vae_search_amd/csrc/dvs_api_backward.inc
+++ b/dags_vae_search_amd/csrc/dvs_api_backward.inc
@@ -24,6 +24,7 @@
     a.o_out_w = ap.out_w;
     a.o_out_b = ap.out_b;
     a.qkv = c.wide ? c.ws + c.W.qkv[block] : nullptr;
+    a.dropbits = dropbits_at(c, c.save_bits, DvsDropBits::attn(block, c.d.B));
     return a;
 }
 
@@ -77,6 +78,7 @@
     a.o_ln_b = norm.b;
     a.o_own_g = -1;
     a.o_own_b = -1;
+    a.dropbits = dropbits_at(c, c.save_bits, DvsDropBits::ffn(block, c.d.B));
     return a;
 }
 
@@ -252,6 +254,8 @@
         e.oW2 = L.W2;
         e.olab_w = L.lab_w;
         e.olab_b = L.lab_b;
+        e.dropbits = dropbits_at(c, c.save_bits, DvsDropBits::emb(0, c.d.B));
+        e.dropbits2 = dropbits_at(c, c.save_bits, DvsDropBits::emb(1, c.d.B));
         if (wide) dvs_launch_embed_bwd_w(e, gdec_emb, 2, grid, st);
         else dvs_launch_embed_bwd(e, gdec_emb, 2, grid, nw, st);
     }
diff --git a/dags_vae_search_amd/csrc/dvs_backward.h b/dags_vae_search_amd/csrc/dvs_backward.h
--- a/dags_vae_search_amd/csrc/dvs_backward.h
+++ b/dags_vae_search_amd/csrc/dvs_backward.h
@@ -16,6 +16,7 @@
     float* slab;
     int64_t P;
     int64_t o_l1_w, o_l1_b, o_l2_w, o_l2_b, o_ln_g, o_ln_b, o_own_g, o_own_b;
+    const uint32_t* dropbits;
 };
 
 struct ProjBwdArgs {
@@ -52,6 +53,7 @@
     int64_t P;
     int64_t o_out_w, o_out_b;
     const float* qkv;
+    const uint32_t* dropbits;
 };
 
 struct LatentBwdArgs {
diff --git a/dags_vae_search_amd/csrc/dvs_bwd_phases.h b/dags_vae_search_amd/csrc/dvs_bwd_phases.h
--- a/dags_vae_search_amd/csrc/dvs_bwd_phases.h
+++ b/dags_vae_search_amd/csrc/dvs_bwd_phases.h
@@ -105,6 +105,7 @@
     dvs_plan_vec(p, smem, l.ob, a.own.b, a.own_pre ? 64 : 0);
     p.zero_int = (int)(((const char*)l.gcount - smem) >> 2);
     dvs_plan_cold(p, a.xin, a.own_pre, a.dims.B * a.dims.NT);
+    dvs_plan_cold_bits(p, a.dims.drop.on ? a.dropbits : nullptr, (int)DvsDropBits::FFN);
     dvs_plan_seal(p);
 }
 inline void attnb_plan(DvsStagePlan& p, const AttnBwdArgs& a, char* smem) {
@@ -117,6 +118,7 @@
     dvs_plan_vec(p, smem, l.lb, a.ln.b, a.ln.stats ? 64 : 0);
     p.zero_int = (int)(((const char*)l.gcount - smem) >> 2);
     dvs_plan_cold(p, a.xin, a.kv, a.dims.B * a.dims.NT);
+    dvs_plan_cold_bits(p, a.dims.drop.on ? a.dropbits : nullptr, (int)DvsDropBits::ATTN);
     dvs_plan_seal(p);
 }
 inline void projb_plan(DvsStagePlan& p, const ProjBwdArgs& a, int nproj, char* smem) {
@@ -158,7 +160,7 @@
     dvs_touch_done(touch);
 }
 
-template <int NW, class PP>
+template <int NW, bool SAVED, class PP>
 __device__ __forceinline__ void dvs_ffn_bwd_phase(const FfnBwdArgs& a, char* smem, PP mine, bool stage_mine, PP next,
                                                   bool has_next) {
     const FfnBLds l = ffnb_lds(smem);
@@ -190,9 +192,11 @@
         const int Nl = live ? N : 0;
         f4 x[4], xhat[4], gp[4];
         float rstd;
+        uint32_t saved_bits = 0;
         {
             DvsRawX rx;
             dvs_load_x_issue(rx, a.xin, a.ln, dg, L);
+            if (SAVED) saved_bits = a.dropbits[dg * 64 + L.lane];
             DVS_PHASE_GATE(gate);
             dvs_load_tile(gp, a.gpre, dg, L);
             dvs_load_x_finish<true>(x, xhat, rstd, rx, a.ln, l.lg, l.lb, Nl, L);
@@ -213,8 +217,8 @@
             dvs_ln_bwd_core(gp, pxh, prstd, l.og, L);
         }
         const uint32_t gdag = a.dims.dag_offset + (uint32_t)T.dag;
-        const uint32_t khid = dvs_site_key(a.dims.seed_lo, a.dims.seed_hi, a.site_hidden, gdag);
-        const uint32_t kpost = dvs_site_key(a.dims.seed_lo, a.dims.seed_hi, a.site_post, gdag);
+        const uint32_t hid_bits = SAVED ? (saved_bits & 0xFFFFu)
+                                        : dvs_dropout_bits(dvs_site_key(a.dims.seed_lo, a.dims.seed_hi, a.site_hidden, gdag), D, L, T.tok0);
         f4 hpre[4], hd[4];
 #pragma unroll
         for (int t = 0; t < 4; ++t) hpre[t] = dvs_vecT(l.b1, t, L);
@@ -223,12 +227,12 @@
         for (int t = 0; t < 4; ++t)
 #pragma unroll
             for (int kk = 0; kk < 4; ++kk) hd[t][kk] = (live && L.r < N) ? fmaxf(hpre[t][kk], 0.f) : 0.f;
-        const uint32_t hid_bits = dvs_dropout_bits(khid, D, L, T.tok0);
         dvs_dropout_apply(hd, hid_bits, D);
         f4 dy[4];
 #pragma unroll
         for (int t = 0; t < 4; ++t) dy[t] = gp[t];
-        dvs_dropout_tile(dy, kpost, D, L, T.tok0);
+        if (SAVED) dvs_dropout_apply(dy, saved_bits >> 16, D);
+        else dvs_dropout_tile(dy, dvs_site_key(a.dims.seed_lo, a.dims.seed_hi, a.site_post, gdag), D, L, T.tok0);
         dvs_park_bf((dvs_bf16*)sA, dy, L);
         dvs_park_bf((dvs_bf16*)sB, hd, L);
         dvs_group_barrier(G, L);
@@ -269,7 +273,7 @@
     DvsBwdTail tail;
     DVS_STAMP(dvs_stamps_bwd, mine, 2);
     dvs_tail_issue(tail, next, has_next);
-    const DvsTouch touch = dvs_touch_first(next, has_next, NW, L.wave, L.lane);
+    const DvsTouch touch = dvs_touch_first<SAVED>(next, has_next, NW, L.wave, L.lane);
     DVS_STAMP(dvs_stamps_bwd, mine, 3);
     dvs_lds_barrier();
     DVS_STAMP(dvs_stamps_bwd, mine, 4);
@@ -306,7 +310,7 @@
     dvs_bwd_tail_end(tail, touch, mine, next, has_next, smem);
 }
 
-template <int NPROJ, int NW, class PP>
+template <int NPROJ, int NW, bool SAVED, class PP>
 __device__ __forceinline__ void dvs_proj_bwd_phase(const ProjBwdArgs& a, char* smem, PP mine, bool stage_mine, PP next,
                                                    bool has_next) {
     const ProjBLds pl = projb_lds(smem, NPROJ);
@@ -418,7 +422,7 @@
     DvsBwdTail tail;
     DVS_STAMP(dvs_stamps_bwd, mine, 2);
     dvs_tail_issue(tail, next, has_next);
-    const DvsTouch touch = dvs_touch_first(next, has_next, NW, L.wave, L.lane);
+    const DvsTouch touch = dvs_touch_first<SAVED>(next, has_next, NW, L.wave, L.lane);
     DVS_STAMP(dvs_stamps_bwd, mine, 3);
     dvs_lds_barrier();
     DVS_STAMP(dvs_stamps_bwd, mine, 4);
@@ -465,22 +469,9 @@
     uint32_t T;
     uint32_t S[4];
 };
-__device__ __forceinline__ ProbMask dvs_prob_mask(uint32_t key, const DvsDrop& D, const Lane& L) {
+__device__ __forceinline__ ProbMask dvs_prob_mask(uint32_t bitsT, const DvsDrop& D, const Lane& L) {
     ProbMask m;
-    m.T = 0xFFFFFFFFu;
-    if (D.on) {
-        uint32_t bits = 0;
-#pragma unroll
-        for (int h = 0; h < 8; ++h) {
-            const uint32_t p0 = (uint32_t)((h * 16 + L.r) * 8 + 2 * L.g);
-            const uint32_t h0 = dvs_draw(key, p0), h1 = dvs_draw(key, p0 + 1);
-            bits |= ((h0 & 0xFFFFu) >= D.thr16 ? 1u : 0u) << (4 * h);
-            bits |= ((h0 >> 16) >= D.thr16 ? 1u : 0u) << (4 * h + 1);
-            bits |= ((h1 & 0xFFFFu) >= D.thr16 ? 1u : 0u) << (4 * h + 2);
-            bits |= ((h1 >> 16) >= D.thr16 ? 1u : 0u) << (4 * h + 3);
-        }
-        m.T = bits;
-    }
+    m.T = bitsT;
 #pragma unroll
     for (int reg = 0; reg < 4; ++reg)
         m.S[reg] = D.on ? ((uint32_t)__shfl((int)m.T, 4 * L.g + reg + 16 * (L.r >> 2)) >> (L.r & 3)) : 0xFFFFFFFFu;
@@ -501,7 +492,7 @@
     return r;
 }
 
-template <int NW, class PP>
+template <int NW, bool SAVED, class PP>
 __device__ __forceinline__ void dvs_attn_bwd_phase(const AttnBwdArgs& a, char* smem, PP mine, bool stage_mine, PP next,
                                                    bool has_next) {
     const AttnBLds l = attnb_lds(smem);
@@ -529,8 +520,9 @@
         const size_t dg = live ? dag : 0;
         const int Nl = live ? N : 0;
         const uint32_t gdag = a.dims.dag_offset + (uint32_t)dg;
-        const uint32_t kprob = dvs_site_key(a.dims.seed_lo, a.dims.seed_hi, a.site_prob, gdag);
         const unsigned allowed_r = live ? a.rec[dg].allowed[L.r] : (1u << L.r);
+        uint32_t prob_bits = 0xFFFFFFFFu, post_bits = 0xFFFFFFFFu;
+        if (SAVED) dvs_bits_load2(prob_bits, post_bits, a.dropbits, dg, L);
         f4 q[4], k[4], v[4];
         {
             f4 x[4], kv[4], dummy[4];
@@ -568,7 +560,8 @@
         {
             f4 dy[4];
             dvs_load_grad(dy, a.gpre, dg, Nl, L);
-            dvs_dropout_tile(dy, dvs_site_key(a.dims.seed_lo, a.dims.seed_hi, a.site_post, gdag), D, L);
+            if (SAVED) dvs_dropout_apply(dy, post_bits, D);
+            else dvs_dropout_tile(dy, dvs_site_key(a.dims.seed_lo, a.dims.seed_hi, a.site_post, gdag), D, L);
             dvs_park_bf((dvs_bf16*)sA, dy, L);
 #pragma unroll
             for (int t = 0; t < 4; ++t) dOT[t] = f4_zero();
@@ -579,7 +572,8 @@
         dvs_n2t<4>(vT, v, sB, L);
         dvs_t2n<4>(dON, dOT, sB, L);
 
-        const ProbMask pm = dvs_prob_mask(kprob, D, L);
+        if (!SAVED) prob_bits = dvs_prob_bits(dvs_site_key(a.dims.seed_lo, a.dims.seed_hi, a.site_prob, gdag), D, L);
+        const ProbMask pm = dvs_prob_mask(prob_bits, D, L);
         const bool hsel = ((L.r & 3) >> 1) != 0;
         bool ok[4];
         unsigned al4[4];
@@ -720,7 +714,7 @@
     DvsBwdTail tail;
     DVS_STAMP(dvs_stamps_bwd, mine, 2);
     dvs_tail_issue(tail, next, has_next);
-    const DvsTouch touch = dvs_touch_first(next, has_next, NW, L.wave, L.lane);
+    const DvsTouch touch = dvs_touch_first<SAVED>(next, has_next, NW, L.wave, L.lane);
     DVS_STAMP(dvs_stamps_bwd, mine, 3);
     dvs_lds_barrier();
     DVS_STAMP(dvs_stamps_bwd, mine, 4);
diff --git a/dags_vae_search_amd/csrc/dvs_device.h b/dags_vae_search_amd/csrc/dvs_device.h
--- a/dags_vae_search_amd/csrc/dvs_device.h
+++ b/dags_vae_search_amd/csrc/dvs_device.h
@@ -315,6 +315,23 @@
     }
 }
 template <int NTILE = 4>
+__device__ __forceinline__ uint32_t dvs_dropout_tile_bits(f4 (&x)[NTILE], uint32_t key, const DvsDrop& D, const Lane& L, int tok0 = 0) {
+    if (!D.on) return 0xFFFFFFFFu;
+    uint32_t bits = 0;
+#pragma unroll
+    for (int t = 0; t < NTILE; ++t) {
+        const uint32_t p0 = (uint32_t)((tok0 + L.r) * 64 + 16 * t + 4 * L.g) >> 1;
+        const uint32_t h0 = dvs_draw(key, p0), h1 = dvs_draw(key, p0 + 1);
+        const bool k0 = (h0 & 0xFFFFu) >= D.thr16, k1 = (h0 >> 16) >= D.thr16, k2 = (h1 & 0xFFFFu) >= D.thr16, k3 = (h1 >> 16) >= D.thr16;
+        x[t][0] = k0 ? x[t][0] * D.scale : 0.f;
+        x[t][1] = k1 ? x[t][1] * D.scale : 0.f;
+        x[t][2] = k2 ? x[t][2] * D.scale : 0.f;
+        x[t][3] = k3 ? x[t][3] * D.scale : 0.f;
+        bits |= (k0 ? 1u << (4 * t) : 0u) | (k1 ? 2u << (4 * t) : 0u) | (k2 ? 4u << (4 * t) : 0u) | (k3 ? 8u << (4 * t) : 0u);
+    }
+    return bits;
+}
+template <int NTILE = 4>
 __device__ __forceinline__ uint32_t dvs_dropout_bits(uint32_t key, const DvsDrop& D, const Lane& L, int tok0 = 0) {
     uint32_t bits = 0xFFFFFFFFu;
     if (D.on) {
@@ -339,6 +356,27 @@
 #pragma unroll
         for (int kk = 0; kk < 4; ++kk) x[t][kk] = ((bits >> (4 * t + kk)) & 1u) ? x[t][kk] * D.scale : 0.f;
 }
+__device__ __forceinline__ uint32_t dvs_prob_bits(uint32_t key, const DvsDrop& D, const Lane& L) {
+    uint32_t bits = 0xFFFFFFFFu;
+    if (D.on) {
+        bits = 0;
+#pragma unroll
+        for (int h = 0; h < 8; ++h) {
+            const uint32_t p0 = (uint32_t)((h * 16 + L.r) * 8 + 2 * L.g);
+            const uint32_t h0 = dvs_draw(key, p0), h1 = dvs_draw(key, p0 + 1);
+            bits |= ((h0 & 0xFFFFu) >= D.thr16 ? 1u : 0u) << (4 * h);
+            bits |= ((h0 >> 16) >= D.thr16 ? 1u : 0u) << (4 * h + 1);
+            bits |= ((h1 & 0xFFFFu) >= D.thr16 ? 1u : 0u) << (4 * h + 2);
+            bits |= ((h1 >> 16) >= D.thr16 ? 1u : 0u) << (4 * h + 3);
+        }
+    }
+    return bits;
+}
+__device__ __forceinline__ void dvs_bits_load2(uint32_t& w0, uint32_t& w1, const uint32_t* base, size_t dag, const Lane& L) {
+    const uint64_t w = ((const uint64_t*)base)[dag * 64 + L.lane];
+    w0 = (uint32_t)w;
+    w1 = (uint32_t)(w >> 32);
+}
 __device__ __forceinline__ float dvs_dropout_elem(float v, uint32_t key, uint32_t e, const DvsDrop& D) {
     const uint32_t h = dvs_draw(key, e >> 1);
     const uint32_t half = (e & 1u) ? (h >> 16) : (h & 0xFFFFu);
diff --git a/dags_vae_search_amd/csrc/dvs_host.h b/dags_vae_search_amd/csrc/dvs_host.h
--- a/dags_vae_search_amd/csrc/dvs_host.h
+++ b/dags_vae_search_amd/csrc/dvs_host.h
@@ -61,8 +61,17 @@
     size_t wimg;
     size_t limg;
     size_t qkv[9];
+    size_t dropbits;
     size_t total_floats;
     int nslab;
 };
 
-DvsWorkspace dvs_make_workspace(int B, int NT, int64_t P, int nslab, bool wide);
+struct DvsDropBits {
+    static constexpr size_t ATTN = 128, FFN = 64, EMB = 64;
+    static constexpr size_t PER_DAG = 9 * ATTN + 6 * FFN + 2 * EMB;
+    static size_t attn(int block, size_t B) { return (size_t)block * ATTN * B; }
+    static size_t ffn(int block, size_t B) { return (9 * ATTN + (size_t)block * FFN) * B; }
+    static size_t emb(int src, size_t B) { return (9 * ATTN + 6 * FFN + (size_t)src * EMB) * B; }
+};
+
+DvsWorkspace dvs_make_workspace(int B, int NT, int64_t P, int nslab, bool wide, bool training);
diff --git a/dags_vae_search_amd/csrc/dvs_kernels.h b/dags_vae_search_amd/csrc/dvs_kernels.h
--- a/dags_vae_search_amd/csrc/dvs_kernels.h
+++ b/dags_vae_search_amd/csrc/dvs_kernels.h
@@ -38,6 +38,7 @@
     float* slab;
     int64_t P;
     int64_t oW1, oW2, olab_w, olab_b;
+    uint32_t *dropbits, *dropbits2;
 };
 
 struct AttnArgs {
@@ -52,6 +53,7 @@
     float* out_stats;
     int site_prob, site_post;
     float* qkv;
+    uint32_t* dropbits;
 };
 
 struct FfnArgs {
@@ -65,6 +67,7 @@
     float* out_norm;
     const float *ng, *nb;
     int site_hidden, site_post;
+    uint32_t* dropbits;
 };
 
 struct LatentArgs {
diff --git a/dags_vae_search_amd/csrc/dvs_stage.h b/dags_vae_search_amd/csrc/dvs_stage.h
--- a/dags_vae_search_amd/csrc/dvs_stage.h
+++ b/dags_vae_search_amd/csrc/dvs_stage.h
@@ -16,6 +16,8 @@
     int phase;
     const float* cold[2];
     int cold_tiles;
+    int cold_bits_words;
+    const uint32_t* cold_bits;
 };
 
 #ifdef DVS_STAMPS
@@ -73,11 +75,17 @@
     p.zero_int = -1;
     p.cold[0] = p.cold[1] = nullptr;
     p.cold_tiles = 0;
+    p.cold_bits = nullptr;
+    p.cold_bits_words = 0;
 }
 DVS_HD inline void dvs_plan_cold(DvsStagePlan& p, const float* a, const float* b, int tiles) {
     p.cold[0] = a ? a : b;
     p.cold[1] = b ? b : a;
     p.cold_tiles = (a || b) ? tiles : 0;
+}
+DVS_HD inline void dvs_plan_cold_bits(DvsStagePlan& p, const uint32_t* bits, int words_per_tile) {
+    p.cold_bits = bits;
+    p.cold_bits_words = bits ? words_per_tile : 0;
 }
 DVS_HD inline void dvs_plan_seg(DvsStagePlan& p, const char* smem, const void* lds_dst, const void* src, int n_bf16) {
     p.src = (const f4*)src;
@@ -202,23 +210,27 @@
 }
 struct DvsTouch {
     float v[2];
-};
-template <class PP>
+    uint32_t bits;
+};
+template <bool BITS = false, class PP>
 __device__ __forceinline__ DvsTouch dvs_touch_first(PP next, bool has_next, int nw, int wave, int lane) {
     DvsTouch t;
     t.v[0] = t.v[1] = 0.f;
+    t.bits = 0;
     if (has_next && next->cold_tiles > 0) {
         int tile = dvs_bid() * nw + wave;
         tile = tile < next->cold_tiles ? tile : 0;
         const size_t off = (size_t)tile * 1024 + (size_t)lane * 16;
         t.v[0] = next->cold[0][off];
         t.v[1] = next->cold[1][off];
+        const int bw = next->cold_bits_words;
+        if (BITS && bw > 0) t.bits = next->cold_bits[(size_t)tile * bw + (size_t)lane * (bw >> 6)];
     }
     return t;
 }
 __device__ __forceinline__ void dvs_touch_done(const DvsTouch& t) {
 #ifndef DVS_EMU
-    asm volatile("" ::"v"(t.v[0]), "v"(t.v[1]));
+    asm volatile("" ::"v"(t.v[0]), "v"(t.v[1]), "v"(t.bits));
 #else
     (void)t;
 #endif
diff --git a/dags_vae_search_amd/csrc/k_backward.hip b/dags_vae_search_amd/csrc/k_backward.hip
--- a/dags_vae_search_amd/csrc/k_backward.hip
+++ b/dags_vae_search_amd/csrc/k_backward.hip
@@ -1,28 +1,34 @@
 #include "dvs_bwd_phases.h"
 #include "dvs_latent_bwd.h"
 
-template <int NW>
+template <int NW, bool SAVED>
 __global__ __launch_bounds__(64 * NW) void k_ffn_bwd(FfnBwdArgs a, DvsStagePlan plan) {
     DVS_DYN_LDS(smem);
-    dvs_ffn_bwd_phase<NW>(a, smem, &plan, true, &plan, false);
+    dvs_ffn_bwd_phase<NW, SAVED>(a, smem, &plan, true, &plan, false);
 }
 void dvs_launch_ffn_bwd(const FfnBwdArgs& a, int grid, int nw, dvs_stream_t st) {
     const size_t lds = ffnb_lds_bytes();
     DvsStagePlan plan;
     ffnb_plan(plan, a, DVS_FAKE_LDS);
+#define DVS_PHASE_LAUNCH(name, kernel, NWV, SV)                                                \
+    do {                                                                                       \
+        DVS_SET_LDS((kernel<NWV, SV>), lds);                                                   \
+        DVS_LAUNCH_AS(name, (kernel<NWV, SV>), dim3(grid), dim3(64 * NWV), lds, st, a, plan);  \
+    } while (0)
+    const bool saved = a.dims.drop.on && a.dropbits;
     if (nw == 4) {
-        DVS_SET_LDS(k_ffn_bwd<4>, lds);
-        DVS_LAUNCH_AS("k_ffn_bwd", k_ffn_bwd<4>, dim3(grid), dim3(256), lds, st, a, plan);
+        if (saved) DVS_PHASE_LAUNCH("k_ffn_bwd", k_ffn_bwd, 4, true);
+        else DVS_PHASE_LAUNCH("k_ffn_bwd", k_ffn_bwd, 4, false);
     } else {
-        DVS_SET_LDS(k_ffn_bwd<8>, lds);
-        DVS_LAUNCH_AS("k_ffn_bwd", k_ffn_bwd<8>, dim3(grid), dim3(512), lds, st, a, plan);
+        if (saved) DVS_PHASE_LAUNCH("k_ffn_bwd", k_ffn_bwd, 8, true);
+        else DVS_PHASE_LAUNCH("k_ffn_bwd", k_ffn_bwd, 8, false);
     }
 }
 
 template <int NPROJ, int NW>
 __global__ __launch_bounds__(64 * NW) void k_proj_bwd(ProjBwdArgs a, DvsStagePlan plan) {
     DVS_DYN_LDS(smem);
-    dvs_proj_bwd_phase<NPROJ, NW>(a, smem, &plan, true, &plan, false);
+    dvs_proj_bwd_phase<NPROJ, NW, false>(a, smem, &plan, true, &plan, false);
 }
 
 #define DVS_PROJ_LAUNCH(NP, NWV)                                                               \
@@ -45,26 +51,27 @@
     }
 }
 
-template <int NW>
+template <int NW, bool SAVED>
 __global__ __launch_bounds__(64 * NW) void k_attn_bwd(AttnBwdArgs a, DvsStagePlan plan) {
     DVS_DYN_LDS(smem);
-    dvs_attn_bwd_phase<NW>(a, smem, &plan, true, &plan, false);
+    dvs_attn_bwd_phase<NW, SAVED>(a, smem, &plan, true, &plan, false);
 }
 
 void dvs_launch_attn_bwd(const AttnBwdArgs& a, int grid, int nw, dvs_stream_t st) {
     const size_t lds = attnb_lds_floats() * 4;
     DvsStagePlan plan;
     attnb_plan(plan, a, DVS_FAKE_LDS);
+    const bool saved = a.dims.drop.on && a.dropbits;
     if (nw == 4) {
-        DVS_SET_LDS(k_attn_bwd<4>, lds);
-        DVS_LAUNCH_AS("k_attn_bwd", k_attn_bwd<4>, dim3(grid), dim3(256), lds, st, a, plan);
+        if (saved) DVS_PHASE_LAUNCH("k_attn_bwd", k_attn_bwd, 4, true);
+        else DVS_PHASE_LAUNCH("k_attn_bwd", k_attn_bwd, 4, false);
     } else {
-        DVS_SET_LDS(k_attn_bwd<8>, lds);
-        DVS_LAUNCH_AS("k_attn_bwd", k_attn_bwd<8>, dim3(grid), dim3(512), lds, st, a, plan);
+        if (saved) DVS_PHASE_LAUNCH("k_attn_bwd", k_attn_bwd, 8, true);
+        else DVS_PHASE_LAUNCH("k_attn_bwd", k_attn_bwd, 8, false);
     }
 }
 
-template <int TAG, int NW>
+template <int TAG, int NW, bool SAVED>
 __global__ __launch_bounds__(64 * NW) void k_bwd_stack(BwdStackArgs s) {
     DVS_DYN_LDS(smem);
 #ifndef DVS_EMU
@@ -87,11 +94,11 @@
         const DvsPlanK mine = plans + i;
         const DvsPlanK next = plans + (more ? i + 1 : i);
         switch (ph.kind) {
-            case DVS_PH_FFN: dvs_ffn_bwd_phase<NW>(ph.u.f, smem, mine, first, next, more); break;
-            case DVS_PH_ATTN: dvs_attn_bwd_phase<NW>(ph.u.a, smem, mine, first, next, more); break;
-            case DVS_PH_PROJ1: dvs_proj_bwd_phase<1, NW>(ph.u.p, smem, mine, first, next, more); break;
-            case DVS_PH_PROJ2: dvs_proj_bwd_phase<2, NW>(ph.u.p, smem, mine, first, next, more); break;
-            default: dvs_proj_bwd_phase<3, NW>(ph.u.p, smem, mine, first, next, more); break;
+            case DVS_PH_FFN: dvs_ffn_bwd_phase<NW, SAVED>(ph.u.f, smem, mine, first, next, more); break;
+            case DVS_PH_ATTN: dvs_attn_bwd_phase<NW, SAVED>(ph.u.a, smem, mine, first, next, more); break;
+            case DVS_PH_PROJ1: dvs_proj_bwd_phase<1, NW, SAVED>(ph.u.p, smem, mine, first, next, more); break;
+            case DVS_PH_PROJ2: dvs_proj_bwd_phase<2, NW, SAVED>(ph.u.p, smem, mine, first, next, more); break;
+            default: dvs_proj_bwd_phase<3, NW, SAVED>(ph.u.p, smem, mine, first, next, more); break;
         }
     }
 }
@@ -113,10 +120,20 @@
         const size_t b = k == DVS_PH_FFN ? ffnb_lds_bytes() : k == DVS_PH_ATTN ? attnb_lds_floats() * 4 : projb_lds_bytes(k - DVS_PH_PROJ1 + 1);
         lds = b > lds ? b : lds;
     }
+    bool saved = false;
+    for (int i = 0; i < s.nphase; ++i) {
+        if (s.ph[i].kind == DVS_PH_FFN) saved = saved || (s.ph[i].u.f.dims.drop.on && s.ph[i].u.f.dropbits);
+        if (s.ph[i].kind == DVS_PH_ATTN) saved = saved || (s.ph[i].u.a.dims.drop.on && s.ph[i].u.a.dropbits);
+    }
 #define DVS_BSTACK_LAUNCH(TG, NWV)                                                             \
     do {                                                                                       \
-        DVS_SET_LDS((k_bwd_stack<TG, NWV>), lds);                                              \
-        DVS_LAUNCH_AS("k_bwd_stack<" #TG ">", (k_bwd_stack<TG, NWV>), dim3(grid), dim3(64 * NWV), lds, st, s); \
+        if (saved) {                                                                           \
+            DVS_SET_LDS((k_bwd_stack<TG, NWV, true>), lds);                                    \
+            DVS_LAUNCH_AS("k_bwd_stack<" #TG ">", (k_bwd_stack<TG, NWV, true>), dim3(grid), dim3(64 * NWV), lds, st, s); \
+        } else {                                                                               \
+            DVS_SET_LDS((k_bwd_stack<TG, NWV, false>), lds);                                   \
+            DVS_LAUNCH_AS("k_bwd_stack<" #TG ">", (k_bwd_stack<TG, NWV, false>), dim3(grid), dim3(64 * NWV), lds, st, s); \
+        }                                                                                      \
     } while (0)
     if (nw == 4) {
         if (tag == 0) DVS_BSTACK_LAUNCH(0, 4);
diff --git a/dags_vae_search_amd/csrc/k_backward_heads.hip b/dags_vae_search_amd/csrc/k_backward_heads.hip
--- a/dags_vae_search_amd/csrc/k_backward_heads.hip
+++ b/dags_vae_search_amd/csrc/k_backward_heads.hip
@@ -291,8 +291,13 @@
             const float* gsrc = src == 0 ? a.gout : gout2;
             if (!gsrc) continue;
             const int site = src == 0 ? a.site : site2;
+            const uint32_t* const bsrc = src == 0 ? a.dropbits : a.dropbits2;
+            const bool saved = D.on && bsrc;
             f4 gx[4];
-            dvs_load_grad(gx, gsrc, dag, N, L);
+            uint32_t saved_bits = 0;
+            dvs_load_tile(gx, gsrc, dag, L);
+            if (saved) saved_bits = bsrc[(size_t)dag * 64 + L.lane];
+            dvs_zero_rows(gx, N, L);
             f4 dle[2];
 #pragma unroll
             for (int t = 0; t < 2; ++t)
@@ -304,14 +309,15 @@
                 }
             dlabb[0] += dle[0];
             dlabb[1] += dle[1];
-            const uint32_t k1 = dvs_site_key(a.dims.seed_lo, a.dims.seed_hi, site, gdag);
             f4 m1[4] = {f4_splat(1.f), f4_splat(1.f), f4_splat(1.f), f4_splat(1.f)};
-            dvs_dropout_tile(m1, k1, D, L);
+            if (saved) dvs_dropout_apply(m1, saved_bits & 0xFFFFu, D);
+            else dvs_dropout_tile(m1, dvs_site_key(a.dims.seed_lo, a.dims.seed_hi, site, gdag), D, L);
             f4 e1d[4];
 #pragma unroll
             for (int t = 0; t < 4; ++t) e1d[t] = e1[t] * m1[t];
             f4 de2[2] = {gx[2], gx[3]};
-            dvs_dropout_tile<2>(de2, dvs_site_key(a.dims.seed_lo, a.dims.seed_hi, site + 1, gdag), D, L);
+            if (saved) dvs_dropout_apply<2>(de2, saved_bits >> 16, D);
+            else dvs_dropout_tile<2>(de2, dvs_site_key(a.dims.seed_lo, a.dims.seed_hi, site + 1, gdag), D, L);
             f4 e1dN[4], de2N[2], dleN[2];
             dvs_t2n<4>(e1dN, e1d, scr, L);
             dvs_t2n<2>(de2N, de2, scr, L);
diff --git a/dags_vae_search_amd/csrc/k_forward.hip b/dags_vae_search_amd/csrc/k_forward.hip
--- a/dags_vae_search_amd/csrc/k_forward.hip
+++ b/dags_vae_search_amd/csrc/k_forward.hip
@@ -207,6 +207,7 @@
     return n > (size_t)DvsEmbImg::FLOATS ? n : (size_t)DvsEmbImg::FLOATS;
 }
 
+template <bool SAVED>
 __global__ __launch_bounds__(1024) void k_embed_fwd(EmbedArgs a, DvsStagePlan plan) {
     DVS_DYN_LDS(smem);
     const int N = a.dims.N, C = a.dims.C;
@@ -230,7 +231,9 @@
             f4 e1[4];
 #pragma unroll
             for (int t = 0; t < 4; ++t) e1[t] = eh[t];
-            dvs_dropout_tile(e1, dvs_site_key(a.dims.seed_lo, a.dims.seed_hi, site, gdag), D, L);
+            uint32_t bits1 = 0;
+            if (SAVED) bits1 = dvs_dropout_tile_bits(e1, dvs_site_key(a.dims.seed_lo, a.dims.seed_hi, site, gdag), D, L);
+            else dvs_dropout_tile(e1, dvs_site_key(a.dims.seed_lo, a.dims.seed_hi, site, gdag), D, L);
             f4 x[4];
             f4 e2[2] = {f4_zero(), f4_zero()};
 #pragma unroll
@@ -244,7 +247,12 @@
             }
             {
                 f4 tmp[2] = {e2[0], e2[1]};
-                dvs_dropout_tile<2>(tmp, dvs_site_key(a.dims.seed_lo, a.dims.seed_hi, site + 1, gdag), D, L);
+                if (SAVED) {
+                    const uint32_t bits2 = dvs_dropout_tile_bits<2>(tmp, dvs_site_key(a.dims.seed_lo, a.dims.seed_hi, site + 1, gdag), D, L);
+                    (v ? a.dropbits2 : a.dropbits)[(size_t)dag * 64 + L.lane] = (bits1 & 0xFFFFu) | (bits2 << 16);
+                } else {
+                    dvs_dropout_tile<2>(tmp, dvs_site_key(a.dims.seed_lo, a.dims.seed_hi, site + 1, gdag), D, L);
+                }
                 x[2] = tmp[0];
                 x[3] = tmp[1];
             }
@@ -267,8 +275,13 @@
     dvs_plan_clear(plan);
     dvs_plan_seg(plan, DVS_FAKE_LDS, DVS_FAKE_LDS, a.embimg, 2 * DvsEmbImg::FLOATS);
     dvs_plan_seal(plan);
-    DVS_SET_LDS(k_embed_fwd, lds);
-    DVS_LAUNCH(k_embed_fwd, dim3(grid), dim3(nw == 4 ? 256 : 1024), lds, st, a, plan);
+    if (a.dropbits) {
+        DVS_SET_LDS(k_embed_fwd<true>, lds);
+        DVS_LAUNCH_AS("k_embed_fwd", k_embed_fwd<true>, dim3(grid), dim3(nw == 4 ? 256 : 1024), lds, st, a, plan);
+    } else {
+        DVS_SET_LDS(k_embed_fwd<false>, lds);
+        DVS_LAUNCH_AS("k_embed_fwd", k_embed_fwd<false>, dim3(grid), dim3(nw == 4 ? 256 : 1024), lds, st, a, plan);
+    }
 }
 
 #ifdef DVS_STAMPS
@@ -378,6 +391,18 @@
     p[3] = ((h1 >> 16) >= D.thr16) ? p[3] * D.scale : 0.f;
     return p;
 }
+__device__ __forceinline__ f4 attn_drop_T_bits(f4 p, uint32_t key, int h, const DvsDrop& D, const Lane& L, uint32_t& bits) {
+    if (!D.on) return p;
+    const uint32_t p0 = (uint32_t)((h * 16 + L.r) * 8 + 2 * L.g);
+    const uint32_t h0 = dvs_draw(key, p0), h1 = dvs_draw(key, p0 + 1);
+    const bool k0 = (h0 & 0xFFFFu) >= D.thr16, k1 = (h0 >> 16) >= D.thr16, k2 = (h1 & 0xFFFFu) >= D.thr16, k3 = (h1 >> 16) >= D.thr16;
+    p[0] = k0 ? p[0] * D.scale : 0.f;
+    p[1] = k1 ? p[1] * D.scale : 0.f;
+    p[2] = k2 ? p[2] * D.scale : 0.f;
+    p[3] = k3 ? p[3] * D.scale : 0.f;
+    bits |= (k0 ? 1u << (4 * h) : 0u) | (k1 ? 2u << (4 * h) : 0u) | (k2 ? 4u << (4 * h) : 0u) | (k3 ? 8u << (4 * h) : 0u);
+    return p;
+}
 
 template <class PP>
 __device__ __forceinline__ void dvs_fwd_tail(PP next, bool has_next, char* smem, PP mine) {
@@ -393,7 +418,7 @@
     }
 }
 
-template <int NW, class PP>
+template <int NW, bool SAVED, class PP>
 __device__ __forceinline__ void dvs_attn_fwd_phase(const AttnArgs& a, char* smem, PP mine, bool stage_mine, PP next,
                                                    bool has_next) {
     const AttnLds l = attn_lds(smem);
@@ -448,8 +473,15 @@
         attn_scores_T(s, q, k, L);
         attn_softmax_T(p, m, den, s, allowed_r, L);
         ASTAMP(2);
-#pragma unroll
-        for (int h = 0; h < 8; ++h) p[h] = attn_drop_T(p[h], kprob, h, D, L);
+        uint32_t pbits = 0;
+        if (SAVED) {
+#pragma unroll
+            for (int h = 0; h < 8; ++h) p[h] = attn_drop_T_bits(p[h], kprob, h, D, L, pbits);
+            a.dropbits[((size_t)dag * 64 + L.lane) * 2] = pbits;
+        } else {
+#pragma unroll
+            for (int h = 0; h < 8; ++h) p[h] = attn_drop_T(p[h], kprob, h, D, L);
+        }
         ASTAMP(3);
         f4 o[4];
         {
@@ -472,7 +504,12 @@
         for (int t = 0; t < 4; ++t) y[t] = dvs_vecT(l.outb, t, L);
         dvs_matb3<4>(y, dvs_split3_T(o), l.Wout, 64, 0, L);
         ASTAMP(5);
-        dvs_dropout_tile(y, dvs_site_key(a.dims.seed_lo, a.dims.seed_hi, a.site_post, gdag), D, L);
+        if (SAVED) {
+            const uint32_t ybits = dvs_dropout_tile_bits(y, dvs_site_key(a.dims.seed_lo, a.dims.seed_hi, a.site_post, gdag), D, L);
+            a.dropbits[((size_t)dag * 64 + L.lane) * 2 + 1] = ybits;
+        } else {
+            dvs_dropout_tile(y, dvs_site_key(a.dims.seed_lo, a.dims.seed_hi, a.site_post, gdag), D, L);
+        }
         const bool valid = L.r < N;
 #pragma unroll
         for (int t = 0; t < 4; ++t)
@@ -486,22 +523,27 @@
     dvs_fwd_tail(next, has_next, smem, mine);
 }
 
-template <int NW>
+template <int NW, bool SAVED>
 __global__ __launch_bounds__(64 * NW) void k_attn_fwd(AttnArgs a, DvsStagePlan plan) {
     DVS_DYN_LDS(smem);
-    dvs_attn_fwd_phase<NW>(a, smem, &plan, true, &plan, false);
+    dvs_attn_fwd_phase<NW, SAVED>(a, smem, &plan, true, &plan, false);
 }
 
 void dvs_launch_attn_fwd(const AttnArgs& a, int grid, int nw, dvs_stream_t st) {
     const size_t lds = attn_lds_bytes();
     DvsStagePlan plan;
     attn_plan(plan, a, DVS_FAKE_LDS);
+#define DVS_ATTNF_LAUNCH(NWV, SV)                                                              \
+    do {                                                                                       \
+        DVS_SET_LDS((k_attn_fwd<NWV, SV>), lds);                                               \
+        DVS_LAUNCH_AS("k_attn_fwd", (k_attn_fwd<NWV, SV>), dim3(grid), dim3(64 * NWV), lds, st, a, plan); \
+    } while (0)
     if (nw == 4) {
-        DVS_SET_LDS(k_attn_fwd<4>, lds);
-        DVS_LAUNCH_AS("k_attn_fwd", k_attn_fwd<4>, dim3(grid), dim3(256), lds, st, a, plan);
+        if (a.dropbits) DVS_ATTNF_LAUNCH(4, true);
+        else DVS_ATTNF_LAUNCH(4, false);
     } else {
-        DVS_SET_LDS(k_attn_fwd<8>, lds);
-        DVS_LAUNCH_AS("k_attn_fwd", k_attn_fwd<8>, dim3(grid), dim3(512), lds, st, a, plan);
+        if (a.dropbits) DVS_ATTNF_LAUNCH(8, true);
+        else DVS_ATTNF_LAUNCH(8, false);
     }
 }
 
@@ -536,7 +578,7 @@
     dvs_plan_seal(p);
 }
 
-template <class PP>
+template <bool SAVED, class PP>
 __device__ __forceinline__ void dvs_ffn_fwd_phase(const FfnArgs& a, char* smem, PP mine, bool stage_mine, PP next,
                                                   bool has_next) {
     const FfnLds l = ffn_lds(smem);
@@ -574,12 +616,19 @@
         for (int t = 0; t < 4; ++t)
 #pragma unroll
             for (int kk = 0; kk < 4; ++kk) h[t][kk] = fmaxf(h[t][kk], 0.f);
-        dvs_dropout_tile(h, dvs_site_key(a.dims.seed_lo, a.dims.seed_hi, a.site_hidden, gdag), D, L, T.tok0);
+        uint32_t hbits = 0, ybits = 0;
+        if (SAVED) hbits = dvs_dropout_tile_bits(h, dvs_site_key(a.dims.seed_lo, a.dims.seed_hi, a.site_hidden, gdag), D, L, T.tok0);
+        else dvs_dropout_tile(h, dvs_site_key(a.dims.seed_lo, a.dims.seed_hi, a.site_hidden, gdag), D, L, T.tok0);
         f4 y[4];
 #pragma unroll
         for (int t = 0; t < 4; ++t) y[t] = dvs_vecT(l.b2, t, L);
         dvs_matb3<4>(y, dvs_split3_T(h), l.W2, 64, 0, L);
-        dvs_dropout_tile(y, dvs_site_key(a.dims.seed_lo, a.dims.seed_hi, a.site_post, gdag), D, L, T.tok0);
+        if (SAVED) {
+            ybits = dvs_dropout_tile_bits(y, dvs_site_key(a.dims.seed_lo, a.dims.seed_hi, a.site_post, gdag), D, L, T.tok0);
+            a.dropbits[(size_t)tile * 64 + L.lane] = (hbits & 0xFFFFu) | (ybits << 16);
+        } else {
+            dvs_dropout_tile(y, dvs_site_key(a.dims.seed_lo, a.dims.seed_hi, a.site_post, gdag), D, L, T.tok0);
+        }
         const bool valid = L.r < T.Nl;
 #pragma unroll
         for (int t = 0; t < 4; ++t)
@@ -608,20 +657,26 @@
     dvs_fwd_tail(next, has_next, smem, mine);
 }
 
+template <bool SAVED>
 __global__ __launch_bounds__(1024) void k_ffn_fwd(FfnArgs a, DvsStagePlan plan) {
     DVS_DYN_LDS(smem);
-    dvs_ffn_fwd_phase(a, smem, &plan, true, &plan, false);
+    dvs_ffn_fwd_phase<SAVED>(a, smem, &plan, true, &plan, false);
 }
 
 void dvs_launch_ffn_fwd(const FfnArgs& a, int grid, int nw, dvs_stream_t st) {
     const size_t lds = ffn_lds_bytes();
     DvsStagePlan plan;
     ffn_plan(plan, a, DVS_FAKE_LDS);
-    DVS_SET_LDS(k_ffn_fwd, lds);
-    DVS_LAUNCH(k_ffn_fwd, dim3(grid), dim3(nw == 4 ? 256 : 1024), lds, st, a, plan);
-}
-
-template <int TAG, int NW>
+    if (a.dropbits) {
+        DVS_SET_LDS(k_ffn_fwd<true>, lds);
+        DVS_LAUNCH_AS("k_ffn_fwd", k_ffn_fwd<true>, dim3(grid), dim3(nw == 4 ? 256 : 1024), lds, st, a, plan);
+    } else {
+        DVS_SET_LDS(k_ffn_fwd<false>, lds);
+        DVS_LAUNCH_AS("k_ffn_fwd", k_ffn_fwd<false>, dim3(grid), dim3(nw == 4 ? 256 : 1024), lds, st, a, plan);
+    }
+}
+
+template <int TAG, int NW, bool SAVED>
 __global__ __launch_bounds__(64 * NW) void k_fwd_stack(FwdStackArgs s) {
     DVS_DYN_LDS(smem);
 #ifndef DVS_EMU
@@ -644,8 +699,8 @@
         }
         const bool more_img = more && s.ph[i + 1].kind != DVS_FPH_LATENT;
         const DvsPlanK next = plans + (more_img ? i + 1 : i);
-        if (ph.kind == DVS_FPH_ATTN) dvs_attn_fwd_phase<NW>(ph.u.a, smem, mine, first, next, more_img);
-        else dvs_ffn_fwd_phase(ph.u.f, smem, mine, first, next, more_img);
+        if (ph.kind == DVS_FPH_ATTN) dvs_attn_fwd_phase<NW, SAVED>(ph.u.a, smem, mine, first, next, more_img);
+        else dvs_ffn_fwd_phase<SAVED>(ph.u.f, smem, mine, first, next, more_img);
     }
 }
 
@@ -662,10 +717,17 @@
 #endif
     const size_t la = attn_lds_bytes(), lf = ffn_lds_bytes();
     const size_t lds = la > lf ? la : lf;
+    const bool saved = s.nphase > 0 && (s.ph[0].kind == DVS_FPH_ATTN ? s.ph[0].u.a.dropbits != nullptr
+                                        : s.ph[0].kind == DVS_FPH_FFN && s.ph[0].u.f.dropbits != nullptr);
 #define DVS_FSTACK_LAUNCH(TG, NWV)                                                             \
     do {                                                                                       \
-        DVS_SET_LDS((k_fwd_stack<TG, NWV>), lds);                                              \
-        DVS_LAUNCH_AS("k_fwd_stack<" #TG ">", (k_fwd_stack<TG, NWV>), dim3(grid), dim3(64 * NWV), lds, st, s); \
+        if (saved) {                                                                           \
+            DVS_SET_LDS((k_fwd_stack<TG, NWV, true>), lds);                                    \
+            DVS_LAUNCH_AS("k_fwd_stack<" #TG ">", (k_fwd_stack<TG, NWV, true>), dim3(grid), dim3(64 * NWV), lds, st, s); \
+        } else {                                                                               \
+            DVS_SET_LDS((k_fwd_stack<TG, NWV, false>), lds);                                   \
+            DVS_LAUNCH_AS("k_fwd_stack<" #TG ">", (k_fwd_stack<TG, NWV, false>), dim3(grid), dim3(64 * NWV), lds, st, s); \
+        }                                                                                      \
     } while (0)
     if (nw == 4) {
         if (tag == 0) DVS_FSTACK_LAUNCH(0, 4);
diff --git a/dags_vae_search_amd/engine.py b/dags_vae_search_amd/engine.py
--- a/dags_vae_search_amd/engine.py
+++ b/dags_vae_search_amd/engine.py
@@ -50,7 +50,7 @@
 
     def workspace(self, batch: int, device) -> torch.Tensor:
         if self._ws is None or self._ws_batch != batch or self._ws.device != device:
-            shape = self.shape(batch)
+            shape = self.shape(batch, training=True)
             nbytes = self.lib.dvs_workspace_bytes(ctypes.byref(shape))
             if nbytes == 0:
                 dl.check(self.lib, 1, "dvs_workspace_bytes")
```

New measurement: 3.487 million DAGs/s (median of 6 runs). No clear change (+0.7%).
